# olasanni1/ETOL

Hardware: AMD Instinct MI355X
Metric: collocation-node constraint+Jacobian evals/sec, 6-state VGP N=1024 (higher is better)
Workload: dtype f64

## Files before the change

etol_amd/_lib.py:

```python
import ctypes as C
import os

import torch

_HERE = os.path.dirname(os.path.abspath(__file__))
LIB_PATH = os.path.join(_HERE, "lib", "libemi355x.so")

EMI_OK = 0
STATUS = {0: "EMI_OK", 1: "EMI_ERR_ARG", 2: "EMI_ERR_STATE", 3: "EMI_ERR_HIP",
          4: "EMI_ERR_NO_DEVICE", 5: "EMI_ERR_UNSUPPORTED", 6: "EMI_ERR_COMM"}

MODEL_POINTMASS2D, MODEL_QUADROTOR2D, MODEL_FIXEDWING12 = 0, 1, 2
MODEL_SOURCE = 100
PATH_ELLIPSE, PATH_DISC, PATH_TRACK = 0, 1, 2
PATH_REC = 8
EVAL_NODES, EVAL_DEFECT, EVAL_ALL, EVAL_NOJAC = 1, 2, 3, 4
EVAL_KEEP_INVARIANT = 8


class EmiError(RuntimeError):
    pass


class Layout(C.Structure):
    _fields_ = [("model", C.c_int), ("ns", C.c_int), ("nc", C.c_int), ("np", C.c_int),
                ("M", C.c_int), ("B", C.c_int), ("nres", C.c_int), ("nvals", C.c_int),
                ("nhess", C.c_int), ("real_bytes", C.c_int), ("px", C.c_int), ("py", C.c_int),
                ("t0", C.c_double), ("tf", C.c_double)]


class PassPlan(C.Structure):
    _fields_ = [(n, C.c_int) for n in ("one_launch", "sw", "ksplit", "ring_stages", "cpart", "cx", "mfma_workgroups", "store_mode",
                                       "block_order", "tiles16", "piece", "tail", "k_tile", "column_tiles", "k_halves")]


_P = C.c_void_p
_D = C.POINTER(C.c_double)
_I = C.POINTER(C.c_int)


def _ptr_struct(name, fields):
    return type(name, (C.Structure,), {"_fields_": [(f, _P) for f in fields], "FIELDS": tuple(fields)})


IpmPoint = _ptr_struct("IpmPoint", ("X", "U", "S", "E1", "E2"))
IpmDuals = _ptr_struct("IpmDuals", ("LamF", "Y", "ZL", "ZU", "VL", "VU", "W1", "W2"))
IpmStep = _ptr_struct("IpmStep", ("DZLam", "DS", "DY", "DE1", "DE2", "DZL", "DZU", "DVL", "DVU", "DW1", "DW2"))
IpmElim = _ptr_struct("IpmElim", ("Sigma", "SigT", "SigS", "RhatS", "Rt"))


class IpmBounds(C.Structure):
    _fields_ = [("zl", _P), ("zu", _P), ("nsets", C.c_int), ("cl", _D), ("cu", _D), ("cscale", _D)]


class IpmOptions(C.Structure):
    _fields_ = [(n, C.c_double) for n in ("tol", "mu_init", "bound_push", "bound_frac", "rho_init", "acceptable_factor")] + \
               [(n, C.c_int) for n in ("max_iter", "acceptable_iter", "max_futile_escalations", "rules", "crawl_limit")] + \
               [("crawl_frac", C.c_double)]


class IpmResult(C.Structure):
    _fields_ = [(n, C.c_int) for n in ("status", "iterations", "evaluations", "factorisations", "reflected_steps")] + \
               [(n, C.c_double) for n in ("cost", "kkt_error", "constr_viol", "emax", "mu", "rho")] + \
               [(n, C.c_int) for n in ("newton_steps", "restored_steps")]


class IpmRung(C.Structure):
    _fields_ = [("M", C.c_int), ("bd", IpmBounds), ("recs", _D), ("opt", IpmOptions), ("repair", C.c_int)]


class IpmRefine(C.Structure):
    _fields_ = [("ode_tol", C.c_double), ("first_check", C.c_int), ("ul", _D), ("uu", _D)]


class IpmRefineResult(C.Structure):
    _fields_ = [("rung", C.c_int), ("verdict", C.c_int), ("rungs_solved", C.c_int), ("err", C.c_double)]


class Start(C.Structure):
    _fields_ = [("kind", C.c_int), ("nsets", C.c_int), ("xa", _D), ("xb", _D), ("box", _D), ("bend", C.c_double), ("clearance", C.c_double),
                ("grid", C.c_int), ("repair", C.c_int)]


START_LINE, START_BEND, START_PLANNED = range(3)
REFINE_MET, REFINE_NOT_MET, REFINE_FELL_BACK, REFINE_FAILED = range(4)
IPM_RULE_RESIDUAL = 1
IPM_CONVERGED, IPM_ACCEPTABLE, IPM_MAX_ITER, IPM_LINE_SEARCH, IPM_INFEASIBLE, IPM_FACTOR, IPM_NOT_FINITE = range(7)

_PT, _DU, _ST, _EL, _BD = (C.POINTER(t) for t in (IpmPoint, IpmDuals, IpmStep, IpmElim, IpmBounds))

SYMBOLS = {
    "emi_abi_version": (C.c_int, []),
    "emi_status_string": (C.c_char_p, [C.c_int]),
    "emi_device_count": (C.c_int, [_I]),
    "emi_lgl": (C.c_int, [C.c_int, _D, _D, _D]),
    "emi_model_dims": (C.c_int, [C.c_int, _I, _I, _I]),
    "emi_edge_ellipse": (C.c_int, [C.c_double] * 4 + [_D]),
    "emi_track_centres": (C.c_int, [C.c_int, _D, _D, _D, C.c_int, _D, _D, _D]),
    "emi_create": (C.c_int, [C.c_int, C.POINTER(_P)]),
    "emi_create_f32": (C.c_int, [C.c_int, C.POINTER(_P)]),
    "emi_destroy": (C.c_int, [_P]),
    "emi_last_error": (C.c_char_p, [_P]),
    "emi_set_stream": (C.c_int, [_P, _P]),
    "emi_get_stream": (C.c_int, [_P, C.POINTER(_P)]),
    "emi_synchronize": (C.c_int, [_P]),
    "emi_set_mesh": (C.c_int, [_P, C.c_int, _D, _D, _D, C.c_double, C.c_double]),
    "emi_set_model": (C.c_int, [_P, C.c_int, _D, C.c_int, C.c_int]),
    "emi_set_model_source": (C.c_int, [_P, C.c_char_p, C.c_char_p, C.c_int, C.c_int, C.c_int, _I, C.c_int, _D, C.c_int, C.c_int]),
    "emi_check_model_source": (C.c_int, [C.c_char_p, C.c_char_p, C.c_int, C.c_int, C.c_int, C.c_int, C.c_int, C.c_char_p, C.c_size_t]),
    "emi_kkt_factor": (C.c_int, [_P, _D, _D, C.POINTER(C.c_ubyte), C.c_double, C.POINTER(C.c_int)]),
    "emi_kkt_factor_dev": (C.c_int, [_P, _P, _P, _P, C.c_double, C.POINTER(C.c_int)]),
    "emi_kkt_blocks_rows": (C.c_int, [_P, C.c_int, _I, _I, _I]),
    "emi_kkt_blocks_dev": (C.c_int, [_P, _P, _P, _P, _P, _P, C.c_double, _P, _P, C.c_int, _P, _P, _P, _P, _P]),
    "emi_kkt_blocks_host": (C.c_int, [_P, _D, _D, _D, _D, C.POINTER(C.c_ubyte), C.c_double, _D, _D, C.c_int, _I, _I, _D, _D, _D]),
    "emi_kkt_solve": (C.c_int, [_P, _D, C.c_int]),
    "emi_kkt_solve_dev": (C.c_int, [_P, _P, C.c_int]),
    "emi_ipm_reduce_dev": (C.c_int, [_P, _PT, _DU, _P, _P, _P, _BD, _P, _P, _P, _EL, _P]),
    "emi_ipm_expand_dev": (C.c_int, [_P, _PT, _DU, _P, _BD, _P, _EL, _P, _ST, _P]),
    "emi_ipm_trial_dev": (C.c_int, [_P, _PT, _ST, _P, _PT]),
    "emi_ipm_merit_dev": (C.c_int, [_P, _PT, _P, _P, _BD, _P, _P, C.c_int, _P]),
    "emi_ipm_accept_dev": (C.c_int, [_P, _PT, _PT, _DU, _ST, _BD, _P, _P, _P, _P]),
    "emi_ipm_error_dev": (C.c_int, [_P, _PT, _DU, _P, _P, _BD, _P, _P]),
    "emi_ipm_reduce_host": (C.c_int, [_P, _PT, _DU, _P, _P, _P, _BD, _P, _P, _P, _EL, _P]),
    "emi_ipm_expand_host": (C.c_int, [_P, _PT, _DU, _P, _BD, _P, _EL, _P, _ST, _P]),
    "emi_ipm_trial_host": (C.c_int, [_P, _PT, _ST, _P, _PT]),
    "emi_ipm_merit_host": (C.c_int, [_P, _PT, _P, _P, _BD, _P, _P, C.c_int, _P]),
    "emi_ipm_accept_host": (C.c_int, [_P, _PT, _PT, _DU, _ST, _BD, _P, _P, _P, _P]),
    "emi_ipm_error_host": (C.c_int, [_P, _PT, _DU, _P, _P, _BD, _P, _P]),
    "emi_ipm_start_dev": (C.c_int, [_P, C.c_int, _PT, _DU, _P, _BD, _P, C.c_double, C.c_double, _P, _P]),
    "emi_ipm_error_parts_dev": (C.c_int, [_P, _PT, _DU, _P, _P, _BD, _P, _P]),
    "emi_ipm_error_parts_host": (C.c_int, [_P, _PT, _DU, _P, _P, _BD, _P, _P]),
    "emi_ipm_keep_dev": (C.c_int, [_P, _PT, _DU, _PT, _DU, _P, C.c_int]),
    "emi_ipm_keep_host": (C.c_int, [_P, _PT, _DU, _PT, _DU, _P, C.c_int]),
    "emi_ipm_solve_shard_dev": (C.c_int, [_P, _P, _P, _BD, C.POINTER(IpmOptions), _P, _P, C.POINTER(IpmResult)]),
    "emi_ipm_solve_shard_host": (C.c_int, [_P, _P, _P, _BD, C.POINTER(IpmOptions), _P, _P, C.POINTER(IpmResult)]),
    "emi_prolong_matrix": (C.c_int, [C.c_int, _D, _D, C.c_int, _D, _D]),
    "emi_prolong_dev": (C.c_int, [_P, C.c_int, C.c_int, _P, _P, C.c_int, _P]),
    "emi_repair_guess_dev": (C.c_int, [_P, _P]),
    "emi_ipm_solve_ladder_dev": (C.c_int, [_P, C.c_int, C.POINTER(IpmRung), C.c_double, C.c_double, _P, _P, _P, _P, _P, _P, C.POINTER(IpmResult)]),
    "emi_ipm_solve_ladder_host": (C.c_int, [_P, C.c_int, C.POINTER(IpmRung), C.c_double, C.c_double, _P, _P, _P, _P, _P, _P, C.POINTER(IpmResult)]),
    "emi_ode_error_operator": (C.c_int, [C.c_int, _D, _D, _D, _D, _D]),
    "emi_interp_dev": (C.c_int, [_P, C.c_int, C.c_int, C.c_int, _P, _P, C.c_int, C.c_int, _P]),
    "emi_ode_error_dev": (C.c_int, [_P, _P, _P, _D, _D, _P, _P]),
    "emi_ode_error_host": (C.c_int, [_P, _P, _P, _D, _D, _P, _P]),
    "emi_ipm_refine_decide": (C.c_int, [C.c_int, C.c_double, C.c_double, C.c_int, C.c_int, _I]),
    "emi_prolong_rows_dev": (C.c_int, [_P, C.c_int, C.c_int, _P, _P, C.c_int, _P, _P]),
    "emi_shard_move_dev": (C.c_int, [_P, C.c_int, _P, _P, C.c_int, _I, C.POINTER(_P), _I, C.POINTER(_P), _I, C.c_int]),
    "emi_ipm_solve_refine_dev": (C.c_int, [_P, C.c_int, C.POINTER(IpmRung), C.c_double, C.c_double, C.POINTER(IpmRefine), _P, _P, C.c_int,
                                           _P, _P, _P, _P, C.POINTER(IpmResult), _D, C.POINTER(IpmRefineResult)]),
    "emi_ipm_solve_refine_host": (C.c_int, [_P, C.c_int, C.POINTER(IpmRung), C.c_double, C.c_double, C.POINTER(IpmRefine), _P, _P, C.c_int,
                                            _P, _P, _P, _P, C.POINTER(IpmResult), _D, C.POINTER(IpmRefineResult)]),
    "emi_plan_route": (C.c_int, [C.c_int, _D, _D, _D, C.c_double, C.c_int, C.c_int, _D, _D, _D, _I, _D, _I, _I]),
    "emi_start_guess_dev": (C.c_int, [_P, C.POINTER(Start), _P, _P]),
    "emi_start_guess_host": (C.c_int, [_P, C.POINTER(Start), _P, _P]),
    "emi_kkt_last_regularisation": (C.c_int, [_P, _D, _D]),
    "emi_kkt_factor_batch": (C.c_int, [C.c_int, C.POINTER(_P), C.POINTER(_D), C.POINTER(_D), C.POINTER(C.POINTER(C.c_ubyte)), _D, _I]),
    "emi_kkt_solve_batch": (C.c_int, [C.c_int, C.POINTER(_P), C.POINTER(_D)]),
    "emi_kkt_is_schur": (C.c_int, [_P]),
    "emi_kkt_solve_refined": (C.c_int, [_P, _D, C.c_double, C.c_int, _D, _I, _I, _I]),
    "emi_kkt_solve_refined_batch": (C.c_int, [C.c_int, C.POINTER(_P), C.POINTER(_D), _D, C.c_int, _D, _I, _I, _I]),
    "emi_kkt_lowrank": (C.c_int, [_P, C.c_int, C.POINTER(C.c_int), _D, _D, C.POINTER(C.c_int)]),
    "emi_kkt_factor_shard_dev": (C.c_int, [_P, _P, _P, _P, _D, C.POINTER(C.c_ubyte), _I]),
    "emi_kkt_lowrank_shard_dev": (C.c_int, [_P, C.c_int, _P, _P, _P, _P, C.POINTER(C.c_ubyte), _I]),
    "emi_kkt_solve_shard_dev": (C.c_int, [_P, _P, C.POINTER(C.c_ubyte)]),
    "emi_kkt_solve_refined_shard_dev": (C.c_int, [_P, _P, C.POINTER(C.c_ubyte), _D, C.c_int, _D, _I, _I, _I]),
    "emi_set_batch": (C.c_int, [_P, C.c_int]),
    "emi_set_path": (C.c_int, [_P, C.c_int, C.c_int, _D, C.c_int, C.c_int]),
    "emi_set_tracks": (C.c_int, [_P, C.c_int, C.c_int, _D, _D]),
    "emi_set_track_waypoints": (C.c_int, [_P, C.c_int, C.c_int, C.c_int, _I, _D, _D, _D]),
    "emi_tracks_from_waypoints_dev": (C.c_int, [_P, C.c_int, _P]),
    "emi_get_tracks": (C.c_int, [_P, _D, _D]),
    "emi_get_layout": (C.c_int, [_P, C.POINTER(Layout)]),
    "emi_jac_structure": (C.c_int, [_P, _I, _I]),
    "emi_invariant_rows": (C.c_int, [C.c_int, C.c_int, C.POINTER(C.c_ubyte), _I]),
    "emi_dev_alloc": (C.c_int, [_P, C.c_size_t, C.POINTER(_P)]),
    "emi_dev_free": (C.c_int, [_P, _P]),
    "emi_h2d": (C.c_int, [_P, _P, _P, C.c_size_t]),
    "emi_d2h": (C.c_int, [_P, _P, _P, C.c_size_t]),
    "emi_eval_dev": (C.c_int, [_P, _P, _P, _P, _P, _P, C.c_uint]),
    "emi_eval_host": (C.c_int, [_P, _D, _D, _D, _D, _D, C.c_uint]),
    "emi_hess_dev": (C.c_int, [_P, _P, _P, _P, _P, C.c_double, _P]),
    "emi_hess_host": (C.c_int, [_P, _D, _D, _D, _D, C.c_double, _D]),
    "emi_lagr_grad_dev": (C.c_int, [_P, _P, _P, _P, C.c_double, _P]),
    "emi_lagr_grad_host": (C.c_int, [_P, _D, _D, _D, C.c_double, _D]),
    "emi_kkt_certificate_dev": (C.c_int, [_P, _P, _P, _P, _P, _P, _P, C.c_double, _P, _P, C.c_int, _D, _D, _P, _P]),
    "emi_kkt_certificate_host": (C.c_int, [_P, _D, _D, _D, _D, C.c_double, _D, _D, C.c_int, _D, _D, _D, _D]),
    "emi_lagr_grad_total_dev": (C.c_int, [_P, _P, _P, _P, C.c_double, _P, _P]),
    "emi_lagr_grad_total_host": (C.c_int, [_P, _D, _D, _D, C.c_double, _D, _D]),
    "emi_kkt_certificate_total_dev": (C.c_int, [_P, _P, _P, _P, _P, _P, _P, C.c_double, _P, _P, C.c_int, _D, _D, _P, _P, _P]),
    "emi_kkt_certificate_total_host": (C.c_int, [_P, _D, _D, _D, _D, C.c_double, _D, _D, C.c_int, _D, _D, _D, _D, _D]),
    "emi_timer_start": (C.c_int, [_P]),
    "emi_timer_stop": (C.c_int, [_P, C.POINTER(C.c_float)]),
    "emi_profile_enable": (C.c_int, [_P, C.c_int]),
    "emi_profile_read": (C.c_int, [_P, C.POINTER(C.c_float), _I, C.POINTER(C.c_float), _I, C.POINTER(C.c_float), _I]),
    "emi_set_option": (C.c_int, [_P, C.c_char_p, C.c_int]),
    "emi_last_path": (C.c_int, [_P, _I]),
    "emi_plan_pass": (C.c_int, [_P, C.c_int, C.POINTER(PassPlan)]),
    "emi_last_defect_kernel": (C.c_char_p, [_P]),
    "emi_debug_pass_roles": (C.c_int, [C.c_int, C.c_int, C.c_int, C.POINTER(C.c_int), C.c_int]),
    "emi_debug_tile_order": (C.c_int, [C.c_int, C.c_int, C.c_int, C.c_int, C.c_int, C.POINTER(C.c_int), C.c_int, C.POINTER(C.c_int), C.POINTER(C.c_int), C.POINTER(C.c_int)]),
    "emi_set_delays": (C.c_int, [_P, C.c_int, C.c_int, C.c_double]),
    "emi_get_delays": (C.c_int, [_P, _I, _I, _I]),
    "emi_delay_matrix": (C.c_int, [C.c_int, C.POINTER(C.c_double), C.POINTER(C.c_double), C.c_double, C.c_double, C.c_double, C.POINTER(C.c_double)]),
    "emi_debug_tile_order2": (C.c_int, [C.c_int] * 7 + [C.POINTER(C.c_int), C.c_int, C.POINTER(C.c_int), C.POINTER(C.c_int), C.POINTER(C.c_int)]),
    "emi_comm_unique_id": (C.c_int, [_P]),
    "emi_comm_create": (C.c_int, [C.c_int, C.c_int, C.c_int, _P, C.POINTER(_P)]),
    "emi_comm_gather": (C.c_int, [_P, _P, _P, C.c_size_t, C.c_int, _P]),
    "emi_comm_destroy": (C.c_int, [_P]),
    "emi_comm_last_error": (C.c_char_p, [_P]),
}

_lib = None


def load():
    global _lib
    if _lib is not None:
        return _lib
    if not os.path.exists(LIB_PATH):
        raise EmiError(f"{LIB_PATH} is missing: run `python -c 'import __graft_entry__ as g; g.build()'` "
                       "(or `make lib`) first; there is no CPU fallback")
    lib = C.CDLL(LIB_PATH, mode=C.RTLD_GLOBAL)
    for name, (res, args) in SYMBOLS.items():
        fn = getattr(lib, name)
        fn.restype = res
        fn.argtypes = args
    _lib = lib
    return lib


def check(status, ctx=None, what=""):
    if status == EMI_OK:
        return
    lib = load()
    msg = lib.emi_status_string(status).decode()
    if ctx:
        detail = lib.emi_last_error(ctx).decode()
        if detail:
            msg += ": " + detail
    raise EmiError(f"{what or 'libemi355x'}: {STATUS.get(status, status)} ({msg})")
```

etol_amd/csrc/emi_api.hip:

```cpp
#include "emi_ctx.hpp"

using namespace emi_api;

int emi_api::fail(emi_ctx_t c, int code, const char* fmt, ...) {
    char buf[512];
    va_list ap;
    va_start(ap, fmt);
    vsnprintf(buf, sizeof buf, fmt, ap);
    va_end(ap);
    if (c) c->err = buf;
    return code;
}

int emi_api::upload_bytes(emi_ctx_t c, DevBuf& b, const void* src, size_t bytes) {
    EMI_TRY(ensure(c, b, bytes));
    if (bytes == 0) return EMI_OK;
    HIP_TRY(c, hipMemcpyAsync(b.p, src, bytes, hipMemcpyHostToDevice, c->stream));
    HIP_TRY(c, hipStreamSynchronize(c->stream));
    return EMI_OK;
}

int emi_api::upload_real(emi_ctx_t c, DevBuf& b, const double* src, size_t n) {
    if (!c->f32) return upload_bytes(c, b, src, n * 8);
    std::vector<float> tmp(n);
    for (size_t i = 0; i < n; ++i) tmp[i] = (float)src[i];
    return upload_bytes(c, b, tmp.data(), n * 4);
}

int emi_api::download_real(emi_ctx_t c, double* dst, const void* dsrc, size_t n) {
    if (!dst || n == 0) return EMI_OK;
    std::vector<float> tmp(c->f32 ? n : 0);
    HIP_TRY(c, hipMemcpyAsync(c->f32 ? (void*)tmp.data() : (void*)dst, dsrc, n * (c->f32 ? 4 : 8), hipMemcpyDeviceToHost, c->stream));
    HIP_TRY(c, hipStreamSynchronize(c->stream));
    for (size_t i = 0; i < tmp.size(); ++i) dst[i] = tmp[i];
    return EMI_OK;
}

int emi_api::ensure_vals_staging(emi_ctx_t c, size_t bytes) {
    if (c->s_VALS.bytes() < bytes) c->keep.written(c->s_VALS.p);
    return ensure(c, c->s_VALS, bytes);
}

void* emi_api::HostStager::place(const void* host, size_t bytes, bool in, bool out) {
    if (!host || status) return nullptr;
    if (slot == c->host_stage.size()) c->host_stage.emplace_back();
    DevBuf& b = c->host_stage[slot++];
    if (b.reserve(std::max<size_t>(bytes, 8)) != hipSuccess) { status = fail(c, EMI_ERR_HIP, "staging of a host-form call: out of device memory"); return nullptr; }
    if (in && bytes && hipMemcpyAsync(b.p, host, bytes, hipMemcpyHostToDevice, c->stream) != hipSuccess) {
        status = fail(c, EMI_ERR_HIP, "staging of a host-form call: copy failed");
        return nullptr;
    }
    if (out) outs.push_back({const_cast<void*>(host), b.p, bytes});
    return b.p;
}

int emi_api::HostStager::finish() {
    for (const Out& o : outs)
        if (o.bytes) HIP_TRY(c, hipMemcpyAsync(o.host, o.dev, o.bytes, hipMemcpyDeviceToHost, c->stream));
    HIP_TRY(c, hipStreamSynchronize(c->stream));
    return EMI_OK;
}

namespace {

struct OptionRow {
    const char* name;
    int emi_ctx_s::*member;
    bool (*accepts)(int);
    int (*stored)(int);
    const char* message;
};
template <int LO, int HI> bool within(int v) { return v >= LO && v <= HI; }
template <int... VS> bool one_of(int v) { return ((v == VS) || ...); }
bool any_value(int) { return true; }
bool at_least_0(int v) { return v >= 0; }
bool whole_tiles(int v) { return v >= 0 && v % 16 == 0; }
int as_given(int v) { return v; }
int as_flag(int v) { return v != 0; }
int ring_wgs(int v) { return v == 1 ? 1 : 2; }
int block_order(int v) { return v < 0 ? -1 : (v >= 100 ? v : (v != 0)); }

const OptionRow OPTIONS[] = {
    {"overlap", &emi_ctx_s::allow_fused, any_value, as_flag, nullptr},
    {"fused", &emi_ctx_s::allow_fused, any_value, as_flag, nullptr},
    {"sym_ct", &emi_ctx_s::sym_ct, within<0, 8>, as_given,
     "sym_ct must be 0..8 (0/4 = chosen from the batch, 3 = LDS-DMA ring, 5..8 = state-split ring with SW = NS/2/1/3)"},
    {"small_rows", &emi_ctx_s::small_rows, at_least_0, as_given, "small_rows must be >= 0 (0 disables the skinny defect kernel)"},
    {"sym_order", &emi_ctx_s::sym_order, any_value, as_flag, nullptr},
    {"f32_ring", &emi_ctx_s::f32_ring, any_value, as_flag, nullptr},
    {"f32_ring_wgs", &emi_ctx_s::f32_ring_wgs, any_value, ring_wgs, nullptr},
    {"f32_one_launch", &emi_ctx_s::f32_one_launch, any_value, as_flag, nullptr},
    {"slice", &emi_ctx_s::slice, whole_tiles, as_given, "slice must be 0 (never) or a multiple of 16 instances"},
    {"pass_order", &emi_ctx_s::pass_order, any_value, block_order, nullptr},
    {"sym_ablate", &emi_ctx_s::sym_ablate, any_value, as_given, nullptr},
    {"adj_fold_tile", &emi_ctx_s::adj_fold_tile, within<0, 2>, as_given, "adj_fold_tile must be 0 (by size), 1 (48 x 64) or 2 (96 x 128)"},
    {"cost_in_kernel", &emi_ctx_s::cost_in_kernel, any_value, as_flag, nullptr},
    {"sym_nst", &emi_ctx_s::sym_nst, one_of<3, 4>, as_given, "sym_nst must be 3 or 4"},
    {"sym_hs", &emi_ctx_s::sym_hs, within<0, 2>, as_given, "sym_hs must be 0 (by batch size), 1 or 2"},
    {"sym_ctc", &emi_ctx_s::sym_ctc, within<0, 2>, as_given, "sym_ctc must be 0 (by batch size), 1 or 2"},
    {"sym_bk", &emi_ctx_s::sym_bk, one_of<0, 8, 16>, as_given, "sym_bk must be 0 (by batch size), 8 or 16"},
    {"sym_cpart", &emi_ctx_s::sym_cpart, one_of<-1, 0, 1, 2, 4, 8>, as_given, "sym_cpart must be -1 (plain order), 0 (by mesh size), 1, 2, 4 or 8"},
    {"sym_gblk", &emi_ctx_s::sym_gblk, within<0, 64>, as_given, "sym_gblk must be 0 (off) .. 64 instance groups per super-block"},
    {"sym_cx", &emi_ctx_s::sym_cx, within<0, 64>, as_given, "sym_cx must be 0 (default) .. 64 column tiles per block"},
    {"sym_combine", &emi_ctx_s::sym_combine, any_value, as_flag, nullptr},
    {"sym_ksplit", &emi_ctx_s::sym_ksplit, one_of<0, 1, 2, 4, 8>, as_given, "sym_ksplit must be 0 (by batch size), 1, 2, 4 or 8"},
    {"node_store", &emi_ctx_s::node_store, within<-1, 3>, as_given,
     "node_store must be -1 (by size), 0 (plain), 1 (write-through sc1), 2 (non-temporal) or 3 (nt sc1; the one-launch pass only)"},
    {"overlap_mode", &emi_ctx_s::overlap_mode, within<0, 3>, as_given,
     "overlap_mode must be 0 (by batch size), 1 (one stream), 2 (two streams) or 3 (one launch)"},
};

}

extern "C" {

int emi_device_count(int* count) {
    if (!count) return EMI_ERR_ARG;
    int n = 0;
    if (hipGetDeviceCount(&n) != hipSuccess) n = 0;
    *count = n;
    return EMI_OK;
}

static int create_impl(int device_id, bool f32, emi_ctx_t* out) {
    if (!out) return EMI_ERR_ARG;
    *out = nullptr;
    int n = 0;
    if (hipGetDeviceCount(&n) != hipSuccess || n <= 0) return EMI_ERR_NO_DEVICE;
    if (device_id < 0 || device_id >= n) return EMI_ERR_ARG;
    hipDeviceProp_t prop;
    if (hipGetDeviceProperties(&prop, device_id) != hipSuccess) return EMI_ERR_HIP;
    if (strncmp(prop.gcnArchName, "gfx950", 6) != 0) return EMI_ERR_NO_DEVICE;
    if (hipSetDevice(device_id) != hipSuccess) return EMI_ERR_HIP;
    emi_ctx_t c = new emi_ctx_s();
    c->device = device_id;
    c->f32 = f32;
    c->own_stream = true;
    if (hipStreamCreateWithFlags(&c->stream, hipStreamNonBlocking) != hipSuccess ||
        hipEventCreateWithFlags(&c->ev_fork, hipEventDisableTiming) != hipSuccess ||
        hipEventCreateWithFlags(&c->ev_join, hipEventDisableTiming) != hipSuccess ||
        hipEventCreate(&c->t_start) != hipSuccess || hipEventCreate(&c->t_stop) != hipSuccess) {
        delete c;
        return EMI_ERR_HIP;
    }
    *out = c;
    return EMI_OK;
}

int emi_create(int device_id, emi_ctx_t* out) { return create_impl(device_id, false, out); }
int emi_create_f32(int device_id, emi_ctx_t* out) { return create_impl(device_id, true, out); }

int emi_destroy(emi_ctx_t c) {
    if (!c) return EMI_ERR_ARG;
    delete c;
    return EMI_OK;
}

const char* emi_last_error(emi_ctx_t c) { return c ? c->err.c_str() : "null context"; }

int emi_set_stream(emi_ctx_t c, void* s) {
    if (!c) return EMI_ERR_ARG;
    HIP_TRY(c, hipSetDevice(c->device));
    HIP_TRY(c, hipStreamSynchronize(c->stream));
    if (s == nullptr) {
        if (!c->own_stream) {
            HIP_TRY(c, hipStreamCreateWithFlags(&c->stream, hipStreamNonBlocking));
            c->own_stream = true;
        }
        return EMI_OK;
    }
    if (c->own_stream) { HIP_TRY(c, hipStreamDestroy(c->stream)); c->own_stream = false; }
    c->stream = (hipStream_t)s;
    return EMI_OK;
}

int emi_get_stream(emi_ctx_t c, void** s) {
    if (!c || !s) return EMI_ERR_ARG;
    *s = (void*)c->stream;
    return EMI_OK;
}

int emi_synchronize(emi_ctx_t c) {
    if (!c) return EMI_ERR_ARG;
    HIP_TRY(c, hipStreamSynchronize(c->stream));
    return EMI_OK;
}

static int upload_operator(emi_ctx_t c, int M, const double* D) {
    if (c->f32) {
        std::vector<float> Df((size_t)M * M);
        for (int i = 0; i < M; ++i) {
            double rs = 0.0;
            for (int j = 0; j < M; ++j) {
                if (j == i) continue;
                Df[(size_t)i * M + j] = (float)D[(size_t)i * M + j];
                rs += (double)Df[(size_t)i * M + j];
            }
            Df[(size_t)i * M + i] = (float)(-rs);
        }
        return upload_bytes(c, c->d_D, Df.data(), Df.size() * 4);
    }
    EMI_TRY(upload_real(c, c->d_D, D, (size_t)M * M));
    if (M % 2 != 0) return EMI_OK;
    const int N = M - 1, Hh = M / 2;
    for (int i = 0; i < M; ++i)
        for (int j = 0; j < M; ++j)
            if (D[(size_t)i * M + j] != -D[(size_t)(N - i) * M + (N - j)]) return EMI_OK;
    std::vector<double> De((size_t)Hh * Hh), Do((size_t)Hh * Hh);
    for (int i = 0; i < Hh; ++i)
        for (int j = 0; j < Hh; ++j) {
            const double p = D[(size_t)i * M + j], q = D[(size_t)i * M + (N - j)];
            De[(size_t)i * Hh + j] = 0.5 * (p + q);
            Do[(size_t)i * Hh + j] = 0.5 * (p - q);
        }
    EMI_TRY(upload_real(c, c->d_De, De.data(), De.size()));
    EMI_TRY(upload_real(c, c->d_Do, Do.data(), Do.size()));
    c->symmetric = true;
    return EMI_OK;
}

int emi_set_mesh(emi_ctx_t c, int M, const double* tau, const double* w, const double* D, double t0,
                 double tf) {
    if (!c || M < 2 || !tau || !w) return fail(c, EMI_ERR_ARG, "emi_set_mesh: bad argument");
    if (!(tf > t0)) return fail(c, EMI_ERR_ARG, "emi_set_mesh: tf must exceed t0");
    c->keep.bump();
    HIP_TRY(c, hipSetDevice(c->device));
    const double h = (tf - t0) / 2.0;
    std::vector<double> nt(M), dd(M, 0.0);
    for (int k = 0; k < M; ++k) {
        nt[k] = t0 + h * (tau[k] + 1.0);
        if (D) dd[k] = D[(size_t)k * M + k];
    }
    EMI_TRY(upload_real(c, c->d_w, w, M));
    EMI_TRY(upload_real(c, c->d_t, nt.data(), M));
    EMI_TRY(upload_real(c, c->d_Ddiag, dd.data(), M));
    c->symmetric = false;
    if (D) EMI_TRY(upload_operator(c, M, D));
    c->points_only = !D;
    c->h_tau.assign(tau, tau + M);
    c->h_w.assign(w, w + M);
    c->M = M;
    c->t0 = t0;
    c->tf = tf;
    c->adj_dirty = true;
    c->ode_dirty = true;
    c->delay_dirty = true;
    c->adjw_dirty = true;
    emi::kkt_mesh_changed(c->kkt);
    for (emi::KktWorkspace* w : c->kkt_shard) emi::kkt_mesh_changed(w);
    c->ntracks = 0;
    c->track_sets = 0;
    c->wp_nt_dirty = true;
    if (c->B > 0) EMI_TRY(ensure(c, c->d_cost_part, (size_t)c->B * emi::node_chunks(M) * (c->f32 ? 4 : 8)));
    return EMI_OK;
}

static void model_in_force(emi_ctx_t c, int model, int ns, int nc, int npath, const int* path_vars, int n_path_vars,
                           const double* params, int nparams, int maximize) {
    c->keep.bump();
    c->model = model;
    c->ns = ns;
    c->nc = nc;
    c->xh = c->uh = c->nch = 0;
    c->np_model = npath;
    c->pvars.assign(path_vars, path_vars + n_path_vars);
    c->maximize = maximize ? 1 : 0;
    memset(c->params, 0, sizeof c->params);
    for (int i = 0; i < nparams; ++i) c->params[i] = params[i];
    c->np = 0;
    c->path_sets = 0;
    c->path_has_track = false;
}

int emi_set_model(emi_ctx_t c, int model, const double* params, int nparams, int maximize) {
    if (!c) return EMI_ERR_ARG;
    int ns, nc, np_expected;
    if (emi_model_dims(model, &ns, &nc, &np_expected)) return fail(c, EMI_ERR_ARG, "unknown model %d", model);
    if (nparams != np_expected || (nparams > 0 && !params))
        return fail(c, EMI_ERR_ARG, "model %d takes %d parameters, got %d", model, np_expected, nparams);
    if (c->rtc) {
        HIP_TRY(c, hipStreamSynchronize(c->stream));
        emi::rtc_destroy(c->rtc);
        c->rtc = nullptr;
    }
    model_in_force(c, model, ns, nc, 0, nullptr, 0, params, nparams, maximize);
    return EMI_OK;
}

int emi_set_model_source(emi_ctx_t c, const char* struct_name, const char* source, int ns, int nc, int npath,
                         const int* path_vars, int n_path_vars, const double* params, int nparams, int maximize) {
    if (!c) return EMI_ERR_ARG;
    if (npath < 0 || npath > 64) return fail(c, EMI_ERR_ARG, "emi_set_model_source: npath must be in [0, 64]");
    if (npath > 0 && (!path_vars || n_path_vars < 1 || n_path_vars > ns + nc))
        return fail(c, EMI_ERR_ARG, "emi_set_model_source: %d traced rows need the list of variables they depend on", npath);
    for (int q = 0; q < (npath > 0 ? n_path_vars : 0); ++q)
        if (path_vars[q] < 0 || path_vars[q] >= ns + nc || (q > 0 && path_vars[q] <= path_vars[q - 1]))
            return fail(c, EMI_ERR_ARG, "emi_set_model_source: path_vars must be ascending node-variable indices below %d", ns + nc);
    if (nparams < 0 || nparams > EMI_MAX_PARAMS || (nparams > 0 && !params))
        return fail(c, EMI_ERR_ARG, "emi_set_model_source: at most %d parameters", EMI_MAX_PARAMS);
    HIP_TRY(c, hipSetDevice(c->device));
    HIP_TRY(c, hipStreamSynchronize(c->stream));
    emi::RtcModel* m = nullptr;
    std::string log;
    const int st = emi::rtc_build(c->f32, struct_name, source, ns, nc, npath, npath > 0 ? n_path_vars : 0, &m, &log);
    if (st) {
        c->err = log;
        return st;
    }
    emi::rtc_destroy(c->rtc);
    c->rtc = m;
    model_in_force(c, EMI_MODEL_SOURCE, ns, nc, npath, path_vars, npath > 0 ? n_path_vars : 0, params, nparams, maximize);
    return EMI_OK;
}

int emi_check_model_source(const char* struct_name, const char* source, int ns, int nc, int npath, int n_path_vars, int f32,
                           char* log, size_t log_len) {
    std::string l;
    const int st = emi::rtc_check(f32 != 0, struct_name, source, ns, nc, npath, npath > 0 ? n_path_vars : 0, &l);
    if (log && log_len) {
        strncpy(log, l.c_str(), log_len - 1);
        log[log_len - 1] = '\0';
    }
    return st;
}

int emi_set_batch(emi_ctx_t c, int B) {
    if (!c || B < 1) return fail(c, EMI_ERR_ARG, "emi_set_batch: B must be >= 1");
    if (c->M <= 0) return fail(c, EMI_ERR_STATE, "emi_set_mesh must precede emi_set_batch");
    c->keep.bump();
    HIP_TRY(c, hipSetDevice(c->device));
    const size_t rb = c->f32 ? 4 : 8;
    int st = ensure(c, c->d_cost_part, (size_t)B * emi::node_chunks(c->M) * rb);
    if (st) return st;
    c->B = B;
    return EMI_OK;
}

int emi_set_delays(emi_ctx_t c, int x_horizon, int u_horizon, double dt) {
    if (!c || x_horizon < 0 || u_horizon < 0) return fail(c, EMI_ERR_ARG, "emi_set_delays: horizons must be >= 0");
    if (c->model < 0) return fail(c, EMI_ERR_STATE, "emi_set_model / emi_set_model_source must precede emi_set_delays");
    c->keep.bump();
    const int nxd = std::max(x_horizon - 1, 0) * c->ns;
    const int rest = c->nc - nxd;
    if (nxd + u_horizon == 0) { c->xh = x_horizon; c->uh = 0; c->nch = 0; return EMI_OK; }
    if (!(dt > 0)) return fail(c, EMI_ERR_ARG, "emi_set_delays: dt must be positive");
    if (rest < 1 || rest % (1 + u_horizon) != 0)
        return fail(c, EMI_ERR_ARG, "emi_set_delays: the model has %d controls, which is not nc + %d delayed states + %d x nc delayed controls for any nc >= 1",
                    c->nc, nxd, u_horizon);
    if (c->f32) return fail(c, EMI_ERR_UNSUPPORTED, "emi_set_delays: f64 contexts only");
    c->xh = x_horizon;
    c->uh = u_horizon;
    c->nch = c->nc - rest / (1 + u_horizon);
    c->delay_dt = dt;
    c->delay_dirty = true;
    c->adjw_dirty = true;
    return EMI_OK;
}

int emi_get_delays(emi_ctx_t c, int* x_horizon, int* u_horizon, int* n_delayed) {
    if (!c) return EMI_ERR_ARG;
    if (x_horizon) *x_horizon = c->xh;
    if (u_horizon) *u_horizon = c->uh;
    if (n_delayed) *n_delayed = c->nch;
    return EMI_OK;
}

int emi_set_path(emi_ctx_t c, int np, int nsets, const double* recs, int px_state, int py_state) {
    if (!c || np < 0) return fail(c, EMI_ERR_ARG, "emi_set_path: bad argument");
    if (c->model < 0) return fail(c, EMI_ERR_STATE, "emi_set_model must precede emi_set_path");
    c->keep.bump();
    if (np > 0 && (!recs || nsets < 1)) return fail(c, EMI_ERR_ARG, "emi_set_path: null table");
    if (px_state < 0 || px_state >= c->ns || py_state < 0 || py_state >= c->ns || px_state == py_state)
        return fail(c, EMI_ERR_ARG, "emi_set_path: state indices (%d,%d) out of range", px_state, py_state);
    HIP_TRY(c, hipSetDevice(c->device));
    bool has_track = false;
    for (size_t i = 0; i < (size_t)np * nsets; ++i) {
        const int kind = (int)recs[i * EMI_PATH_REC];
        if (kind != EMI_PATH_ELLIPSE && kind != EMI_PATH_DISC && kind != EMI_PATH_TRACK)
            return fail(c, EMI_ERR_ARG, "emi_set_path: record %zu has unknown kind %d", i, kind);
        has_track = has_track || kind == EMI_PATH_TRACK;
    }
    int st = upload_real(c, c->d_path, recs, (size_t)np * nsets * EMI_PATH_REC);
    if (st) return st;
    c->path_has_track = has_track;
    c->np = np;
    c->path_sets = np > 0 ? nsets : 0;
    c->px = px_state;
    c->py = py_state;
    return EMI_OK;
}

int emi_set_tracks(emi_ctx_t c, int ntracks, int nsets, const double* xc, const double* yc) {
    if (!c || ntracks < 0) return fail(c, EMI_ERR_ARG, "emi_set_tracks: bad argument");
    if (c->M <= 0) return fail(c, EMI_ERR_STATE, "emi_set_mesh must precede emi_set_tracks");
    c->keep.bump();
    if (ntracks > 0 && (!xc || !yc || nsets < 1)) return fail(c, EMI_ERR_ARG, "emi_set_tracks: null table");
    HIP_TRY(c, hipSetDevice(c->device));
    const size_t n = (size_t)ntracks * nsets * c->M;
    int st;
    if ((st = upload_real(c, c->d_trkx, xc, n))) return st;
    if ((st = upload_real(c, c->d_trky, yc, n))) return st;
    c->ntracks = ntracks;
    c->track_sets = ntracks > 0 ? nsets : 0;
    return EMI_OK;
}

int emi_set_track_waypoints(emi_ctx_t c, int ntracks, int nsets, int ld, const int* counts, const double* t, const double* x,
                            const double* y) {
    if (!c || ntracks < 0) return fail(c, EMI_ERR_ARG, "emi_set_track_waypoints: bad argument");
    if (ntracks == 0) {
        c->wp_ntracks = c->wp_sets = c->wp_ld = 0;
        return EMI_OK;
    }
    if (!t || !x || !y || nsets < 1) return fail(c, EMI_ERR_ARG, "emi_set_track_waypoints: null table");
    if (ld < 2) return fail(c, EMI_ERR_ARG, "emi_set_track_waypoints: ld %d is below the 2 waypoints a track needs", ld);
    const size_t rows = (size_t)nsets * ntracks, n = rows * ld;
    std::vector<int> cnt(rows, ld);
    for (size_t r = 0; r < rows; ++r) {
        const int set = (int)(r / ntracks), trk = (int)(r % ntracks);
        if (counts) cnt[r] = counts[r];
        if (cnt[r] < 2 || cnt[r] > ld)
            return fail(c, EMI_ERR_ARG, "emi_set_track_waypoints: set %d, track %d has %d waypoints (2 .. ld = %d)", set, trk, cnt[r], ld);
        for (int s = 0; s + 1 < cnt[r]; ++s)
            if (!(t[r * ld + s + 1] > t[r * ld + s]))
                return fail(c, EMI_ERR_ARG, "emi_set_track_waypoints: set %d, track %d: the times of waypoints %d and %d are not ascending", set,
                            trk, s, s + 1);
    }
    HIP_TRY(c, hipSetDevice(c->device));
    HIP_TRY(c, hipStreamSynchronize(c->stream));
    HIP_TRY(c, c->d_wp.reserve(3 * n));
    HIP_TRY(c, c->d_wp_cnt.reserve(rows));
    const double* src[3] = {t, x, y};
    for (int q = 0; q < 3; ++q) HIP_TRY(c, hipMemcpyAsync(c->d_wp.p + q * n, src[q], n * sizeof(double), hipMemcpyHostToDevice, c->stream));
    HIP_TRY(c, hipMemcpyAsync(c->d_wp_cnt.p, cnt.data(), rows * sizeof(int), hipMemcpyHostToDevice, c->stream));
    HIP_TRY(c, hipStreamSynchronize(c->stream));
    c->wp_ntracks = ntracks;
    c->wp_sets = nsets;
    c->wp_ld = ld;
    return EMI_OK;
}

int emi_tracks_from_waypoints_dev(emi_ctx_t c, int n, const void* dSetMap) {
    if (!c) return EMI_ERR_ARG;
    if (c->M <= 0) return fail(c, EMI_ERR_STATE, "emi_set_mesh must precede emi_tracks_from_waypoints_dev");
    if (c->wp_ntracks <= 0) return fail(c, EMI_ERR_STATE, "emi_tracks_from_waypoints_dev: emi_set_track_waypoints has not been called");
    if (n < 0 || (!dSetMap && n != 0 && n != c->wp_sets) || (dSetMap && n == 0))
        return fail(c, EMI_ERR_ARG, "emi_tracks_from_waypoints_dev: n = %d (without a map 0 or the table's %d sets, with one >= 1)", n, c->wp_sets);
    const int sets = dSetMap ? n : c->wp_sets;
    if ((long long)sets * c->wp_ntracks > 0x7fffffffLL) return fail(c, EMI_ERR_ARG, "emi_tracks_from_waypoints_dev: %d sets of %d tracks", sets, c->wp_ntracks);
    c->keep.bump();
    HIP_TRY(c, hipSetDevice(c->device));
    const size_t total = (size_t)sets * c->wp_ntracks * c->M, rb = c->f32 ? 4 : 8, wn = (size_t)c->wp_sets * c->wp_ntracks * c->wp_ld;
    EMI_TRY(ensure(c, c->d_trkx, total * rb));
    EMI_TRY(ensure(c, c->d_trky, total * rb));
    const double* node_t = (const double*)c->d_t.p;
    if (c->f32) {
        if (c->wp_nt_dirty || c->d_wp_nt.cap < (size_t)c->M) {
            const double h = (c->tf - c->t0) / 2.0;
            std::vector<double> nt(c->M);
            for (int k = 0; k < c->M; ++k) nt[k] = c->t0 + h * (c->h_tau[k] + 1.0);
            HIP_TRY(c, hipStreamSynchronize(c->stream));
            HIP_TRY(c, c->d_wp_nt.reserve(nt.size()));
            HIP_TRY(c, hipMemcpyAsync(c->d_wp_nt.p, nt.data(), nt.size() * sizeof(double), hipMemcpyHostToDevice, c->stream));
            HIP_TRY(c, hipStreamSynchronize(c->stream));
            c->wp_nt_dirty = false;
        }
        node_t = c->d_wp_nt.p;
    }
    const emi::TrackWaypointArgs a{c->d_wp.p, c->d_wp.p + wn, c->d_wp.p + 2 * wn, node_t, c->d_wp_cnt.p, (const int*)dSetMap,
                                   c->d_trkx.p, c->d_trky.p, sets, c->wp_ntracks, c->wp_ld, c->M, 0};
    HIP_TRY(c, c->f32 ? emi::launch_track_waypoints<float>(a, c->stream) : emi::launch_track_waypoints<double>(a, c->stream));
    c->ntracks = c->wp_ntracks;
    c->track_sets = sets;
    return EMI_OK;
}

int emi_get_tracks(emi_ctx_t c, double* xc, double* yc) {
    if (!c || !xc || !yc) return fail(c, EMI_ERR_ARG, "emi_get_tracks: null argument");
    if (c->M <= 0 || c->ntracks <= 0 || c->track_sets <= 0)
        return fail(c, EMI_ERR_STATE, "emi_get_tracks: the context holds no centres (emi_set_tracks or emi_tracks_from_waypoints_dev on this mesh)");
    HIP_TRY(c, hipSetDevice(c->device));
    const size_t n = (size_t)c->track_sets * c->ntracks * c->M;
    EMI_TRY(download_real(c, xc, c->d_trkx.p, n));
    return download_real(c, yc, c->d_trky.p, n);
}

int emi_get_layout(emi_ctx_t c, emi_layout_t* o) {
    if (!c || !o) return EMI_ERR_ARG;
    o->model = c->model;
    o->ns = c->ns;
    o->nc = c->nc;
    o->np = np_total(c);
    o->M = c->M;
    o->B = c->B;
    o->nres = nres_of(c);
    o->nvals = nvals_of(c);
    o->nhess = nhess_of(c);
    o->real_bytes = c->f32 ? 4 : 8;
    o->px = c->px;
    o->py = c->py;
    o->t0 = c->t0;
    o->tf = c->tf;
    return EMI_OK;
}

int emi_jac_structure(emi_ctx_t c, int* rows, int* cols) {
    if (!c || !rows || !cols) return EMI_ERR_ARG;
    if (c->M <= 0 || c->model < 0) return fail(c, EMI_ERR_STATE, "mesh and model must be set");
    const int M = c->M, ns = c->ns, nv = c->ns + c->nc;
    size_t e = 0;
    for (int i = 0; i < ns; ++i)
        for (int v = 0; v < nv; ++v)
            for (int k = 0; k < M; ++k, ++e) { rows[e] = i * M + k; cols[e] = v * M + k; }
    for (int j = 0; j < c->np; ++j)
        for (int s = 0; s < 2; ++s)
            for (int k = 0; k < M; ++k, ++e) {
                rows[e] = ns * M + 2 * ns + j * M + k;
                cols[e] = (s == 0 ? c->px : c->py) * M + k;
            }
    for (int j = 0; j < c->np_model; ++j)
        for (size_t q = 0; q < c->pvars.size(); ++q)
            for (int k = 0; k < M; ++k, ++e) {
                rows[e] = ns * M + 2 * ns + (c->np + j) * M + k;
                cols[e] = c->pvars[q] * M + k;
            }
    for (int v = 0; v < nv; ++v)
        for (int k = 0; k < M; ++k, ++e) { rows[e] = -1; cols[e] = v * M + k; }
    return EMI_OK;
}

int emi_invariant_rows(int model, int np, unsigned char* mask, int* nvals) {
    int ns, nc;
    if (np < 0 || emi_model_dims(model, &ns, &nc, nullptr)) return EMI_ERR_ARG;
    if (nvals) *nvals = ns * (ns + nc) + 2 * np + (ns + nc);
    if (mask && !emi::invariant_rows(model, np, mask)) return EMI_ERR_ARG;
    return EMI_OK;
}

int emi_dev_alloc(emi_ctx_t c, size_t bytes, void** dptr) {
// ... 147 lines not shown
```

etol_amd/csrc/emi_api_pass.hip:

```cpp
#include "emi_ctx.hpp"

using namespace emi_api;

namespace {

bool overlapped_path(emi_ctx_t c) {
    if (c->f32 || !c->allow_fused || !c->symmetric || c->M <= 0 || c->model < 0) return false;
    if (c->model == EMI_MODEL_SOURCE) return emi::rtc_has_symdefect(c->rtc) && c->M % 128 == 0;
    return emi::fused_supported(c->model, c->M, c->sym_ct);
}

bool pass_takes_small_batches(emi_ctx_t c, int B) {
    if (!overlapped_path(c) || (c->overlap_mode != 0 && c->overlap_mode != 3) || c->M % 128 != 0) return false;
    if (c->rtc) return emi::rtc_pass_supported(c->rtc, B, c->M, 1, 1, 0);
    const emi::SymPlan p = emi::plan_symdefect(c->ns, B, c->M, 7, 1, c->sym_cpart, c->sym_gblk, c->sym_cx);
    return emi::pass_supported(c->model, c->ns, B, c->M, p);
}

int store_mode_for(emi_ctx_t c, int B) {
    if (c->node_store >= 0) return c->node_store;
    if ((size_t)B * (nvals_of(c) + nres_of(c)) * c->M * (c->f32 ? 4 : 8) > ((size_t)230 << 20)) return 2;
    const int tiles16 = ((B + 15) / 16) * (c->M / 128);
    if (tiles16 > 16 && tiles16 <= 32) return 0;
    return (!c->rtc && !c->f32) ? 1 : 0;
}

struct PassPlan {
    bool one_launch = false;
    emi::SymPlan sym;
    int tiles16 = 0;
    int store_mode = 0;
    int mfma_first = 0;
};

PassPlan plan_pass(emi_ctx_t c, int B, bool jac) {
    PassPlan p;
    p.tiles16 = ((B + 15) / 16) * (c->M / 128);
    p.store_mode = store_mode_for(c, B);
    const bool auto_mode = c->overlap_mode == 0;
    if (!((c->overlap_mode == 3 || auto_mode) && jac) || c->M % 128 != 0) return p;
    const bool auto_ct = auto_mode && (c->sym_ct == 0 || c->sym_ct == 4);
    const int gblk = (c->sym_gblk == 0 && c->sym_cpart == 0 && B > 2048 && B % 256 == 0) ? 2 : c->sym_gblk;
    const int gblk_first = (auto_ct || c->rtc) ? gblk : c->sym_gblk;
    int ct = c->sym_ct;
    const bool deep_base = auto_ct && !c->rtc && c->sym_bk == 0 && c->sym_ksplit == 0 && c->sym_nst == 3;
    const bool deep_mid = deep_base && c->ns % 2 == 0 && c->ns > 2 && p.tiles16 >= 49 && p.tiles16 < 128;
    const bool deep_small = deep_base && c->ns % 2 == 0 && c->ns > 2 && p.tiles16 >= 33 && p.tiles16 < 49;
    if (c->rtc) ct = (p.store_mode == 2 && emi::rtc_pass_sw_large(c->rtc) == 2) ? 6 : 7;
    else if (auto_ct) ct = (p.tiles16 < 128 && !deep_mid) ? 7 : 6;
    emi::SymPlan plan = emi::plan_symdefect(c->ns, B, c->M, ct, 1, c->sym_cpart, gblk_first, c->sym_cx);
    if (plan.ring1) plan = emi::plan_symdefect(c->ns, B, c->M, 5, 1, c->sym_cpart, c->sym_gblk, c->sym_cx);
    int ks_want = c->sym_ksplit;
    if (ks_want == 0 && auto_ct && !deep_mid && !deep_small) ks_want = plan.tiles * 4 <= 256 ? 4 : (plan.tiles * 2 <= 512 ? 2 : 1);
    if (ks_want > 1) {
        const int ct_now = plan.sw == c->ns ? 5 : (plan.sw == 2 ? 6 : (plan.sw == 3 ? 8 : 7));
        plan = emi::plan_symdefect(c->ns, B, c->M, ct_now, ks_want, c->sym_cpart, c->rtc ? gblk : c->sym_gblk, c->sym_cx);
    } else {
        plan.ks = 1;
    }
    plan.nst = c->rtc ? 3 : c->sym_nst;
    const bool deep_large = auto_ct && !c->rtc && c->sym_bk == 0 && c->sym_nst == 3 && c->pass_order < 0 && p.tiles16 >= 208 && p.tiles16 <= 1024;
    const bool deep_band = auto_ct && !c->rtc && c->sym_bk == 0 && c->sym_nst == 3 && c->pass_order < 0 && c->ns % 2 == 0 && c->ns > 2 &&
                           p.tiles16 >= 144 && p.tiles16 < 208;
    const int bk_want = c->sym_bk ? c->sym_bk : ((deep_mid || deep_small || deep_large || deep_band) ? 16 : 8);
    if (bk_want == 16 && !c->rtc && plan.ks == 1 && (plan.sw == 1 || plan.sw == 2) && plan.nst == 3) plan.bk = 16;
    const bool wide_large = auto_ct && c->sym_ctc == 0 && B > 2048 && B % 256 == 0 && c->sym_cpart == 0;
    const int ctc_want = c->sym_ctc ? c->sym_ctc : (wide_large ? 2 : 1);
    if (ctc_want == 2 && !c->rtc && plan.ks == 1 && plan.sw == 2 && plan.nst == 3 && c->M % 256 == 0) {
        const int bk_keep = plan.bk;
        plan = emi::plan_symdefect(c->ns, B, c->M, 6, 1, c->sym_cpart, gblk_first, (wide_large && c->sym_cx == 0) ? 1 : c->sym_cx, bk_keep, 2);
        plan.ks = 1;
        plan.nst = 3;
        plan.bk = bk_keep;
    }
    const int hs_want = c->sym_hs ? c->sym_hs : 1;
    if (hs_want == 2 && !c->rtc && plan.ks == 1 && plan.ct == 1 && (plan.sw == 1 || plan.sw == 2) && plan.nst == 3 &&
        ((c->M / 2) / plan.bk) % 4 == 0)
        plan.hs = 2;
    p.sym = plan;
    p.mfma_first = c->pass_order >= 0 ? c->pass_order
                                      : (deep_band ? 150 : (p.tiles16 < 208 ? 1 : (p.tiles16 < 384 ? 125 : (p.tiles16 < 768 ? 110 : 0))));
    p.one_launch = c->rtc ? emi::rtc_pass_supported(c->rtc, B, c->M, plan.sw, plan.ks, p.store_mode)
                          : emi::pass_supported(c->model, c->ns, B, c->M, plan);
    return p;
}

int plan_piece(emi_ctx_t c, int B) {
    const long long cap = ((0xFFFFFFFFLL / ((long long)c->ns * c->M * 8)) / 256) * 256;
    int piece = 0;
    if (c->slice > 0) { if (B > 2 * c->slice) piece = c->slice; }
    else if (B > 2048) piece = (int)std::min<long long>(cap > 0 ? cap : 256, B - B % 256);
    return piece >= B ? 0 : piece;
}

struct Launch { int first, B; bool keep = false; };
struct PassIO { const void *X, *U; void *RES, *VALS, *COST; };

PassIO io_at(emi_ctx_t c, const PassIO& io, int first) {
    const size_t row = (size_t)first * c->M * (c->f32 ? 4 : 8);
    return PassIO{(const char*)io.X + row * c->ns, (const char*)io.U + row * c->nc, (char*)io.RES + row * nres_of(c),
                  io.VALS ? (char*)io.VALS + row * nvals_of(c) : nullptr, (char*)io.COST + (size_t)first * (c->f32 ? 4 : 8)};
}

template <typename T>
void fill_node_args(emi_ctx_t c, Launch L, emi::NodeArgs<T>& a, const PassIO& io) {
    a.X = (const T*)io.X;
    a.U = (const T*)io.U;
    a.RES = (T*)io.RES;
    a.VALS = (T*)io.VALS;
    a.cost_part = (T*)c->d_cost_part.p + (size_t)L.first * emi::node_chunks(c->M);
    a.cost = (T*)io.COST;
    a.cost_ticket = nullptr;
    a.w = (const T*)c->d_w.p;
    a.node_t = (const T*)c->d_t.p;
    a.Ddiag = (const T*)c->d_Ddiag.p;
    a.path = (const T*)c->d_path.p + (c->path_sets > 1 ? (size_t)L.first * c->np * EMI_PATH_REC : 0);
    a.track_x = (const T*)c->d_trkx.p + (c->track_sets > 1 ? (size_t)L.first * c->ntracks * c->M : 0);
    a.track_y = (const T*)c->d_trky.p + (c->track_sets > 1 ? (size_t)L.first * c->ntracks * c->M : 0);
    a.M = c->M;
    a.B = L.B;
    a.np = np_total(c);
    a.nres = nres_of(c);
    a.nvals = nvals_of(c);
    a.path_sets = c->path_sets;
    a.track_sets = c->track_sets;
    a.ntracks = c->ntracks;
    a.px = c->px;
    a.py = c->py;
    a.store_mode = store_mode_for(c, L.B);
    a.keep = L.keep ? 1 : 0;
    a.h = (T)((c->tf - c->t0) / 2.0);
    a.sgn = c->maximize ? T(-1) : T(1);
    for (int i = 0; i < EMI_MAX_PARAMS; ++i) a.P.p[i] = (T)c->params[i];
}

void delay_matrix(const std::vector<double>& tau, const std::vector<double>& w, double t0, double tf, double delay, double* W) {
    const int M = (int)tau.size();
    std::vector<double> lam(M);
    for (int j = 0; j < M; ++j) lam[j] = ((j & 1) ? -1.0 : 1.0) * std::sqrt(w[j]);
    const double hh = (tf - t0) / 2.0;
    for (int k = 0; k < M; ++k) {
        double ts = t0 + hh * (tau[k] + 1.0) - delay;
        if (ts < t0) ts = t0;
        const double x = (ts - t0) / hh - 1.0;
        double* row = W + (size_t)k * M;
        int hit = -1;
        for (int j = 0; j < M; ++j)
            if (x == tau[j]) hit = j;
        if (ts <= t0) hit = 0;
        if (hit >= 0) {
            for (int j = 0; j < M; ++j) row[j] = j == hit ? 1.0 : 0.0;
            continue;
        }
        double den = 0.0;
        for (int j = 0; j < M; ++j) {
            row[j] = lam[j] / (x - tau[j]);
            den += row[j];
        }
        for (int j = 0; j < M; ++j) row[j] /= den;
    }
}

int extend_controls(emi_ctx_t c, const void* dX, const void* dU_free, const void** dU_ext) {
    if (c->f32) return fail(c, EMI_ERR_UNSUPPORTED, "delayed values: f64 contexts only");
    if (c->points_only) return fail(c, EMI_ERR_STATE, "delayed values need a collocation mesh (this context holds a points-only mesh)");
    const int M = c->M, ncf = c->nc - c->nch;
    HIP_TRY(c, hipSetDevice(c->device));
    if (!c->attr_set) {
        HIP_TRY(c, emi::defect_f64_set_attr());
        c->attr_set = true;
    }
    int st;
    if ((st = ensure_delay_matrices(c))) return st;
    const size_t row = (size_t)M * 8;
    if ((st = ensure(c, c->d_uext, (size_t)c->B * c->nc * row))) return st;
    HIP_TRY(c, hipMemsetAsync(c->d_uext.p, 0, (size_t)c->B * c->nc * row, c->stream));
    HIP_TRY(c, hipMemcpy2DAsync(c->d_uext.p, (size_t)c->nc * row, dU_free, (size_t)ncf * row, (size_t)ncf * row, c->B, hipMemcpyDeviceToDevice, c->stream));
    double* base = (double*)c->d_uext.p + (size_t)ncf * M;
    for (int i = 1; i < c->xh; ++i) {
        emi::DefectArgs a{(const double*)dX, (const double*)c->d_W.p + (size_t)(i - 1) * M * M, base + (size_t)(i - 1) * c->ns * M,
                          c->B * c->ns, M, c->ns, c->nc};
        HIP_TRY(c, emi::launch_defect_f64(a, c->stream));
    }
    base += (size_t)std::max(c->xh - 1, 0) * c->ns * M;
    for (int i = 1; i <= c->uh; ++i) {
        emi::DefectArgs a{(const double*)dU_free, (const double*)c->d_W.p + (size_t)(i - 1) * M * M, base + (size_t)(i - 1) * ncf * M,
                          c->B * ncf, M, ncf, c->nc};
        HIP_TRY(c, emi::launch_defect_f64(a, c->stream));
    }
    *dU_ext = c->d_uext.p;
    return EMI_OK;
}

enum class Form {
    PassF64,
    TwoKernelF64,
    PassF32,
    TwoStreamF32,
    Sequential,
};
struct FormChoice {
    Form form = Form::Sequential;
    bool small = false;
    PassPlan plan;
    bool overlapped() const { return form == Form::PassF64 || form == Form::TwoKernelF64; }
};

FormChoice choose_form(emi_ctx_t c, Launch L, unsigned flags) {
    const bool nodes = flags & EMI_EVAL_NODES, defect = flags & EMI_EVAL_DEFECT, jac = !(flags & EMI_EVAL_NOJAC);
    FormChoice ch;
    ch.small = defect && !c->f32 && L.B > 0 && L.B * c->ns <= c->small_rows && emi::defect_small_supported(L.B * c->ns) &&
               !(nodes && jac && pass_takes_small_batches(c, L.B));
    if (nodes && defect && !ch.small && overlapped_path(c)) {
        ch.plan = plan_pass(c, L.B, jac);
        ch.form = ch.plan.one_launch ? Form::PassF64 : Form::TwoKernelF64;
    } else if (c->f32 && nodes && defect && jac && !c->rtc && c->allow_fused) {
        if ((c->overlap_mode == 3 || (c->overlap_mode == 0 && c->f32_one_launch)) && emi::pass_f32_supported(c->model, L.B * c->ns, c->M, L.B))
            ch.form = Form::PassF32;
        else if (c->overlap_mode == 2 && emi::defect_f32_mfma_supported(c->M))
            ch.form = Form::TwoStreamF32;
    }
    return ch;
}

int next_prof_record(emi_ctx_t c, ProfEvents** out) {
    if (c->prof_used == c->prof.size()) c->prof.emplace_back();
    ProfEvents& pe = c->prof[c->prof_used];
    for (hipEvent_t& e : pe.ev)
        if (!e) HIP_TRY(c, hipEventCreate(&e));
    ++c->prof_used;
    *out = &pe;
    return EMI_OK;
}

constexpr unsigned AT1 = 1u << 1, AT2 = 1u << 2, AT3 = 1u << 3, AT_ANY = AT1 | AT2 | AT3;
int prof_mark(emi_ctx_t c, ProfEvents* pe, ProfMark which, unsigned levels, hipStream_t s) {
    if (pe && pe->level > 0 && ((levels >> pe->level) & 1u)) HIP_TRY(c, hipEventRecord(pe->ev[which], s));
    return EMI_OK;
}

const char* const NAME_PASS_F32 = "emi_pass_f32_kernel (MFMA + node roles, one launch)";
const char* const NAME_RING1_F64 = "emi_symdefect_ring_f64_kernel";
const char* name_defect_f32(emi_ctx_t c, bool mfma) {
    return !mfma ? "emi_defect_f32_kernel" : (c->f32_ring ? "emi_defect_f32_ring_kernel" : "emi_defect_f32_mfma_kernel");
}
const char* name_defect_f64(bool small) { return small ? "emi_defect_small_f64_kernel" : "emi_defect_f64_kernel"; }
std::string name_pass_f64(const emi::SymPlan& plan) {
    return "emi_pass_f64_kernel<SW=" + std::to_string(plan.sw) + "> (MFMA + node roles, one launch" +
           (plan.ks > 1 ? ", " + std::to_string(plan.ks) + " K slices per tile" : "") + ")" +
           (plan.bk == 16 ? " [K tiles of 16]" : "") + (plan.ct == 2 ? " [128-column tiles]" : "") + (plan.hs == 2 ? " [K range in two halves per workgroup]" : "");
}
std::string name_symdefect(emi_ctx_t c, const emi::SymPlan& plan, bool in_kernel_combine) {
    if (plan.ring1) return c->sym_ct == 1 || c->sym_ct == 2 ? "emi_symdefect_f64_kernel" : NAME_RING1_F64;
    return "emi_symdefect_ring2_f64_kernel<SW=" + std::to_string(plan.sw) + ">" +
           (plan.ks > 1 ? " x" + std::to_string(plan.ks) + (in_kernel_combine ? " K slices (in-kernel combine)" : " K slices + emi_symdefect_combine_kernel") : "");
}

emi::SymDefectArgs sym_defect_args(emi_ctx_t c, Launch L, const PassIO& io) {
    emi::SymDefectArgs sa;
    sa.X = (const double*)io.X;
    sa.U = (const double*)io.U;
    sa.RES = (double*)io.RES;
    sa.node_t = (const double*)c->d_t.p;
    sa.De = (const double*)c->d_De.p;
    sa.Do = (const double*)c->d_Do.p;
    sa.M = c->M;
    sa.B = L.B;
    sa.nres = nres_of(c);
    sa.h = (c->tf - c->t0) / 2.0;
    sa.order = c->sym_order;
    sa.ablate = c->sym_ablate;
    sa.ksplit = 1;
    sa.slab = nullptr;
    sa.tile_ticket = nullptr;
    sa.cpart = sa.cx = 0;
    sa.mfma_first = 0;
    for (int i = 0; i < EMI_MAX_PARAMS; ++i) sa.P.p[i] = c->params[i];
    return sa;
}

emi::DefectArgsF32 defect_args_f32(emi_ctx_t c, Launch L, const PassIO& io) {
    return emi::DefectArgsF32{(const float*)io.X, (const float*)c->d_D.p, (float*)io.RES, L.B * c->ns, c->M, c->ns, nres_of(c)};
}

int form_pass_f64(emi_ctx_t c, Launch L, const PassIO& io, const PassPlan& pp, ProfEvents* pe) {
    const emi::SymPlan& plan = pp.sym;
    emi::SymDefectArgs sa = sym_defect_args(c, L, io);
    emi::NodeArgs<double> na;
    fill_node_args(c, L, na, io);
    sa.mfma_first = pp.mfma_first;
    sa.cpart = plan.cpart;
    sa.cx = plan.cx;
    if (plan.ks > 1) {
        EMI_TRY(ensure(c, c->d_slab, plan.slab_bytes));
        EMI_TRY(ensure_zeroed(c, c->d_tile_ticket, (size_t)plan.tiles * 4, c->stream));
        sa.ksplit = plan.ks;
        sa.slab = (double*)c->d_slab.p;
        sa.tile_ticket = (unsigned*)c->d_tile_ticket.p;
    }
    EMI_TRY(ensure_zeroed(c, c->d_ticket, (size_t)L.B * 4, c->stream));
    na.cost_ticket = (unsigned*)c->d_ticket.p;
    EMI_TRY(prof_mark(c, pe, K0, AT_ANY, c->stream));
    if (c->rtc) HIP_TRY(c, emi::rtc_launch_pass(c->rtc, sa, na, plan.sw, c->stream));
    else HIP_TRY(c, emi::launch_pass(c->model, sa, na, c->stream, plan));
    EMI_TRY(prof_mark(c, pe, K1, AT_ANY, c->stream));
    if (pe) pe->level = -1;
    c->last_defect_kernel = name_pass_f64(plan);
    return EMI_OK;
}

int launch_symdefect_f64(emi_ctx_t c, Launch L, emi::SymDefectArgs& sa, hipStream_t s) {
    if (c->rtc) {
        HIP_TRY(c, emi::rtc_launch_symdefect(c->rtc, sa, s));
        c->last_defect_kernel = NAME_RING1_F64;
        return EMI_OK;
    }
    const emi::SymPlan plan = emi::plan_symdefect(c->ns, L.B, c->M, c->sym_ct, c->sym_ksplit, c->sym_cpart, c->sym_gblk, c->sym_cx);
    if (plan.slab_bytes) EMI_TRY(ensure(c, c->d_slab, plan.slab_bytes));
    sa.ksplit = plan.ring1 ? 1 : plan.ks;
    sa.slab = (double*)c->d_slab.p;
    sa.cpart = plan.cpart;
    sa.cx = plan.cx;
    if (sa.ksplit > 1 && c->sym_combine) {
        EMI_TRY(ensure_zeroed(c, c->d_tile_ticket, (size_t)plan.tiles * 4, s));
        sa.tile_ticket = (unsigned*)c->d_tile_ticket.p;
    }
    const unsigned bit = 1u << c->sym_ct;
    HIP_TRY(c, emi::launch_symdefect(c->model, sa, s, !(c->fused_attr_mask & bit), c->sym_ct, plan));
    c->fused_attr_mask |= bit;
    c->last_defect_kernel = name_symdefect(c, plan, sa.tile_ticket != nullptr);
    return EMI_OK;
}

int form_two_kernel_f64(emi_ctx_t c, Launch L, const PassIO& io, bool jac, ProfEvents* pe) {
    emi::SymDefectArgs sa = sym_defect_args(c, L, io);
    emi::NodeArgs<double> na;
    fill_node_args(c, L, na, io);
    const bool two = c->overlap_mode != 1;
    const bool split = two && c->cu_split > 0;
    if (two && !split) EMI_TRY(need_stream2(c));
    hipStream_t s1 = split ? c->s_mfma : c->stream;
    hipStream_t s2 = split ? c->s_node : (two ? c->stream2 : c->stream);
    if (two) {
        HIP_TRY(c, hipEventRecord(c->ev_fork, c->stream));
        HIP_TRY(c, hipStreamWaitEvent(s2, c->ev_fork, 0));
        if (split) HIP_TRY(c, hipStreamWaitEvent(s1, c->ev_fork, 0));
    }
    EMI_TRY(prof_mark(c, pe, K0, AT1 | AT2, s1));
    EMI_TRY(launch_symdefect_f64(c, L, sa, s1));
    EMI_TRY(prof_mark(c, pe, K1, AT1 | AT2, s1));
    if (c->cost_in_kernel) {
        EMI_TRY(ensure_zeroed(c, c->d_ticket, (size_t)L.B * 4, s2));
        na.cost_ticket = (unsigned*)c->d_ticket.p;
    }
    EMI_TRY(prof_mark(c, pe, K2, AT1 | AT3, s2));
    if (c->rtc && jac && na.store_mode == 2 && c->M % 2 == 0) HIP_TRY(c, emi::rtc_launch_nodes_nt(c->rtc, na, s2));
    else if (c->rtc) HIP_TRY(c, emi::rtc_launch_nodes<double>(c->rtc, na, jac, false, s2));
    else HIP_TRY(c, emi::launch_nodes<double>(c->model, na, jac, false, s2));
    EMI_TRY(prof_mark(c, pe, K3, AT1 | AT3, s2));
    if (!c->cost_in_kernel) HIP_TRY(c, emi::launch_cost_finish<double>(na.cost_part, na.cost, L.B, emi::node_chunks(c->M), na.sgn * na.h, s2));
    if (two) {
        HIP_TRY(c, hipEventRecord(c->ev_join, s2));
        HIP_TRY(c, hipStreamWaitEvent(c->stream, c->ev_join, 0));
        if (split) {
            HIP_TRY(c, hipEventRecord(c->ev_join2, s1));
            HIP_TRY(c, hipStreamWaitEvent(c->stream, c->ev_join2, 0));
        }
    }
    EMI_TRY(prof_mark(c, pe, E1, AT1, c->stream));
    EMI_TRY(prof_mark(c, pe, E2, AT1, c->stream));
    return EMI_OK;
}

int form_pass_f32(emi_ctx_t c, Launch L, const PassIO& io, ProfEvents* pe) {
    emi::NodeArgs<float> na;
    fill_node_args(c, L, na, io);
    const size_t rowb = (size_t)c->M * 4;
    HIP_TRY(c, hipMemset2DAsync(io.RES, (size_t)nres_of(c) * rowb, 0, (size_t)c->ns * rowb, L.B, c->stream));
    EMI_TRY(ensure_zeroed(c, c->d_ticket, (size_t)L.B * 4, c->stream));
    na.cost_ticket = (unsigned*)c->d_ticket.p;
    EMI_TRY(prof_mark(c, pe, K0, AT_ANY, c->stream));
    HIP_TRY(c, emi::launch_pass_f32(c->model, defect_args_f32(c, L, io), na, c->pass_order >= 0 ? c->pass_order : 0, c->stream));
    EMI_TRY(prof_mark(c, pe, K1, AT_ANY, c->stream));
    if (pe) { pe->level = -1; pe->fused = true; }
    c->last_defect_kernel = NAME_PASS_F32;
    return EMI_OK;
}

int form_two_stream_f32(emi_ctx_t c, Launch L, const PassIO& io, ProfEvents* pe) {
    emi::NodeArgs<float> pre, full;
    PassIO values_only = io;
    values_only.VALS = nullptr;
    fill_node_args(c, L, pre, values_only);
    fill_node_args(c, L, full, io);
    EMI_TRY(ensure(c, c->d_cost_part2, (size_t)L.B * emi::node_chunks(c->M) * 4));
    EMI_TRY(need_stream2(c));
    pre.cost_part = (float*)c->d_cost_part2.p;
    pre.np = 0;
    const bool fork_late = c->f32_ring_wgs == 1;
    if (!fork_late) {
        HIP_TRY(c, hipEventRecord(c->ev_fork, c->stream));
        HIP_TRY(c, hipStreamWaitEvent(c->stream2, c->ev_fork, 0));
    }
    HIP_TRY(c, emi::launch_nodes<float>(c->model, pre, false, true, c->stream));
    if (fork_late) {
        HIP_TRY(c, hipEventRecord(c->ev_fork, c->stream));
        HIP_TRY(c, hipStreamWaitEvent(c->stream2, c->ev_fork, 0));
    }
    EMI_TRY(prof_mark(c, pe, K0, AT1 | AT2, c->stream));
    HIP_TRY(c, emi::launch_defect_f32_mfma(defect_args_f32(c, L, io), c->stream, c->f32_ring, c->f32_ring_wgs));
    EMI_TRY(prof_mark(c, pe, K1, AT1 | AT2, c->stream));
    c->last_defect_kernel = name_defect_f32(c, true);
    EMI_TRY(prof_mark(c, pe, K2, AT1 | AT3, c->stream2));
    HIP_TRY(c, emi::launch_nodes<float>(c->model, full, true, false, c->stream2));
    EMI_TRY(prof_mark(c, pe, K3, AT1 | AT3, c->stream2));
    HIP_TRY(c, emi::launch_cost_finish<float>(full.cost_part, full.cost, L.B, emi::node_chunks(c->M), full.sgn * full.h, c->stream2));
    HIP_TRY(c, hipEventRecord(c->ev_join, c->stream2));
    HIP_TRY(c, hipStreamWaitEvent(c->stream, c->ev_join, 0));
    if (pe) pe->fused = true;
    EMI_TRY(prof_mark(c, pe, E1, AT1, c->stream));
    EMI_TRY(prof_mark(c, pe, E2, AT1, c->stream));
    return EMI_OK;
}

template <typename T>
int launch_nodes_alone(emi_ctx_t c, Launch L, const PassIO& io, bool jac) {
    emi::NodeArgs<T> a;
    fill_node_args(c, L, a, io);
    if (c->rtc) HIP_TRY(c, emi::rtc_launch_nodes<T>(c->rtc, a, jac, true, c->stream));
    else HIP_TRY(c, emi::launch_nodes<T>(c->model, a, jac, true, c->stream));
    HIP_TRY(c, emi::launch_cost_finish<T>(a.cost_part, a.cost, L.B, emi::node_chunks(c->M), a.sgn * a.h, c->stream));
    return EMI_OK;
}

int form_sequential(emi_ctx_t c, Launch L, const PassIO& io, unsigned flags, bool small, ProfEvents* pe) {
    const bool jac = !(flags & EMI_EVAL_NOJAC);
    if (flags & EMI_EVAL_NODES) EMI_TRY(c->f32 ? launch_nodes_alone<float>(c, L, io, jac) : launch_nodes_alone<double>(c, L, io, jac));
    EMI_TRY(prof_mark(c, pe, E1, AT_ANY, c->stream));
    if ((flags & EMI_EVAL_DEFECT) && c->f32) {
        const bool mfma = emi::defect_f32_mfma_supported(c->M) && c->allow_fused;
        if (mfma) HIP_TRY(c, emi::launch_defect_f32_mfma(defect_args_f32(c, L, io), c->stream, c->f32_ring, c->f32_ring_wgs));
        else HIP_TRY(c, emi::launch_defect_f32(defect_args_f32(c, L, io), c->stream));
        c->last_defect_kernel = name_defect_f32(c, mfma);
    } else if (flags & EMI_EVAL_DEFECT) {
        emi::DefectArgs a{(const double*)io.X, (const double*)c->d_D.p, (double*)io.RES, L.B * c->ns, c->M, c->ns, nres_of(c)};
        if (small) HIP_TRY(c, emi::launch_defect_small_f64(a, c->stream));
        else HIP_TRY(c, emi::launch_defect_f64(a, c->stream));
        c->last_defect_kernel = name_defect_f64(small);
    }
    EMI_TRY(prof_mark(c, pe, E2, AT1 | AT2, c->stream));
    return EMI_OK;
}

int eval_launch(emi_ctx_t c, Launch L, const PassIO& io, unsigned flags) {
    const bool nodes = flags & EMI_EVAL_NODES, defect = flags & EMI_EVAL_DEFECT;
    const bool jac = !(flags & EMI_EVAL_NOJAC);
    if (!nodes && !defect) return fail(c, EMI_ERR_ARG, "emi_eval: empty flags");
    if (defect && c->points_only) return fail(c, EMI_ERR_STATE, "emi_eval: the mesh has no differentiation matrix (points-only mesh): EMI_EVAL_NODES only");
    if (!io.X || !io.RES || (nodes && (!io.U || !io.COST || (jac && !io.VALS))))
        return fail(c, EMI_ERR_ARG, "emi_eval: null device pointer");
    HIP_TRY(c, hipSetDevice(c->device));
    if (!c->attr_set) {
        HIP_TRY(c, emi::defect_f64_set_attr());
        c->attr_set = true;
    }
    const FormChoice ch = choose_form(c, L, flags);
    ProfEvents* pe = nullptr;
    if (c->profile) {
        EMI_TRY(next_prof_record(c, &pe));
        pe->has_node = nodes;
        pe->has_defect = defect;
        pe->fused = ch.overlapped();
        pe->level = c->profile;
        EMI_TRY(prof_mark(c, pe, E0, pe->fused ? AT1 : AT1 | AT3, c->stream));
    }
    switch (ch.form) {
        case Form::PassF64: return form_pass_f64(c, L, io, ch.plan, pe);
        case Form::TwoKernelF64: return form_two_kernel_f64(c, L, io, jac, pe);
        case Form::PassF32: return form_pass_f32(c, L, io, pe);
        case Form::TwoStreamF32: return form_two_stream_f32(c, L, io, pe);
        case Form::Sequential: break;
    }
    return form_sequential(c, L, io, flags, ch.small, pe);
}

}

int emi_api::ensure_delay_matrices(emi_ctx_t c) {
    if (!c->delay_dirty) return EMI_OK;
    const int M = c->M, nd = std::max(c->xh - 1, c->uh);
    std::vector<double> W((size_t)nd * M * M);
    for (int d = 0; d < nd; ++d) delay_matrix(c->h_tau, c->h_w, c->t0, c->tf, (d + 1) * c->delay_dt, W.data() + (size_t)d * M * M);
    EMI_TRY(upload_real(c, c->d_W, W.data(), W.size()));
    c->delay_dirty = false;
    return EMI_OK;
}

int emi_api::need_stream2(emi_ctx_t c) {
    if (c->stream2) return EMI_OK;
    if (hipStreamCreateWithFlags(&c->stream2, hipStreamNonBlocking) != hipSuccess) {
        c->stream2 = nullptr;
        return fail(c, EMI_ERR_HIP, "cannot create the second stream of the two-stream pass");
    }
    return EMI_OK;
}

extern "C" {

int emi_delay_matrix(int M, const double* tau, const double* w, double t0, double tf, double delay, double* W) {
    if (M < 2 || !tau || !w || !W || !(tf > t0) || delay < 0) return EMI_ERR_ARG;
    delay_matrix(std::vector<double>(tau, tau + M), std::vector<double>(w, w + M), t0, tf, delay, W);
    return EMI_OK;
}

int emi_eval_dev(emi_ctx_t c, const void* dX, const void* dU, void* dRES, void* dVALS, void* dCOST,
                 unsigned flags) {
    int st = ready(c);
    if (st) return st;
    if (c->nch > 0 && dX && dU && (st = extend_controls(c, dX, dU, &dU))) return st;
    int piece = 0;
    if (!c->profile && !c->f32 && (flags & EMI_EVAL_ALL) == EMI_EVAL_ALL && overlapped_path(c) && dX && dU && dRES && dCOST &&
        (dVALS || (flags & EMI_EVAL_NOJAC)))
        piece = plan_piece(c, c->B);
    const PassIO io{dX, dU, dRES, dVALS, dCOST};
    const emi::KeepRecord::Pass kp = c->keep.begin_pass((flags & EMI_EVAL_NODES) && !(flags & EMI_EVAL_NOJAC),
                                                        flags & EMI_EVAL_KEEP_INVARIANT, dVALS);
    flags &= ~(unsigned)EMI_EVAL_KEEP_INVARIANT;
    if (piece <= 0) st = eval_launch(c, Launch{0, c->B, kp.keep}, io, flags);
    for (int first = 0; piece > 0 && first < c->B && st == EMI_OK; first += piece)
        st = eval_launch(c, Launch{first, std::min(piece, c->B - first), kp.keep}, io_at(c, io, first), flags);
    c->keep.end_pass(kp, dVALS, st == EMI_OK);
    return st;
}

int emi_eval_host(emi_ctx_t c, const double* X, const double* U, double* RES, double* VALS,
                  double* COST, unsigned flags) {
    int st = ready(c);
    if (st) return st;
    if (!X || !U) return fail(c, EMI_ERR_ARG, "emi_eval_host: null input");
    const size_t rb = c->f32 ? 4 : 8;
    const size_t nX = (size_t)c->B * c->ns * c->M, nU = (size_t)c->B * (c->nc - c->nch) * c->M;
    const size_t nR = (size_t)c->B * nres_of(c) * c->M, nV = (size_t)c->B * nvals_of(c) * c->M;
    if ((st = upload_real(c, c->s_X, X, nX))) return st;
    if ((st = upload_real(c, c->s_U, U, nU))) return st;
    if ((st = ensure(c, c->s_RES, nR * rb))) return st;
    if ((st = ensure_vals_staging(c, nV * rb))) return st;
    if ((st = ensure(c, c->s_COST, (size_t)c->B * rb))) return st;
    if (!(flags & EMI_EVAL_NODES)) {
        if (!RES) return fail(c, EMI_ERR_ARG, "emi_eval_host: defect-only needs RES in/out");
        if ((st = upload_real(c, c->s_RES, RES, nR))) return st;
    }
    if ((st = emi_eval_dev(c, c->s_X.p, c->s_U.p, c->s_RES.p, c->s_VALS.p, c->s_COST.p, flags | EMI_EVAL_KEEP_INVARIANT))) return st;
    if ((st = download_real(c, RES, c->s_RES.p, nR))) return st;
    if (!(flags & EMI_EVAL_NOJAC) && (flags & EMI_EVAL_NODES))
        if ((st = download_real(c, VALS, c->s_VALS.p, nV))) return st;
    if (flags & EMI_EVAL_NODES)
        if ((st = download_real(c, COST, c->s_COST.p, c->B))) return st;
    HIP_TRY(c, hipStreamSynchronize(c->stream));
    return EMI_OK;
}

int emi_hess_dev(emi_ctx_t c, const void* dX, const void* dU, const void* dLamF, const void* dLamC,
                 double sigma, void* dH) {
    int st = ready(c);
    if (st) return st;
    if (!dX || !dU || !dLamF || !dH || (np_total(c) > 0 && !dLamC))
        return fail(c, EMI_ERR_ARG, "emi_hess: null device pointer");
    HIP_TRY(c, hipSetDevice(c->device));
    if (c->nch > 0 && (st = extend_controls(c, dX, dU, &dU))) return st;
    auto fill = [&](auto& a) {
        using T = typename std::remove_reference<decltype(a.h)>::type;
        a.X = (const T*)dX; a.U = (const T*)dU; a.lamF = (const T*)dLamF; a.lamC = (const T*)dLamC;
        a.H = (T*)dH; a.w = (const T*)c->d_w.p; a.node_t = (const T*)c->d_t.p;
        a.path = (const T*)c->d_path.p;
        a.M = c->M; a.B = c->B; a.np = np_total(c); a.path_sets = c->path_sets; a.px = c->px; a.py = c->py;
        a.h = (T)((c->tf - c->t0) / 2.0); a.sgn = c->maximize ? T(-1) : T(1); a.sigma = (T)sigma;
        for (int i = 0; i < EMI_MAX_PARAMS; ++i) a.P.p[i] = (T)c->params[i];
    };
    if (c->f32) {
        emi::HessArgs<float> a;
        fill(a);
        if (c->rtc) HIP_TRY(c, emi::rtc_launch_hess<float>(c->rtc, a, c->stream));
        else HIP_TRY(c, emi::launch_hess<float>(c->model, a, c->stream));
    } else {
        emi::HessArgs<double> a;
        fill(a);
        if (c->rtc) HIP_TRY(c, emi::rtc_launch_hess<double>(c->rtc, a, c->stream));
        else HIP_TRY(c, emi::launch_hess<double>(c->model, a, c->stream));
    }
    return EMI_OK;
}

int emi_hess_host(emi_ctx_t c, const double* X, const double* U, const double* LamF,
                  const double* LamC, double sigma, double* H) {
    int st = ready(c);
    if (st) return st;
    if (!X || !U || !LamF || !H || (np_total(c) > 0 && !LamC)) return fail(c, EMI_ERR_ARG, "emi_hess_host: null pointer");
    const size_t rb = c->f32 ? 4 : 8;
    const size_t nX = (size_t)c->B * c->ns * c->M, nU = (size_t)c->B * (c->nc - c->nch) * c->M;
    const size_t nC = (size_t)c->B * np_total(c) * c->M, nH = (size_t)c->B * nhess_of(c) * c->M;
    if ((st = upload_real(c, c->s_X, X, nX))) return st;
    if ((st = upload_real(c, c->s_U, U, nU))) return st;
    if ((st = upload_real(c, c->s_LF, LamF, nX))) return st;
    if (nC && (st = upload_real(c, c->s_LC, LamC, nC))) return st;
    if ((st = ensure(c, c->s_H, nH * rb))) return st;
    if ((st = emi_hess_dev(c, c->s_X.p, c->s_U.p, c->s_LF.p, c->s_LC.p, sigma, c->s_H.p))) return st;
    return download_real(c, H, c->s_H.p, nH);
}

int emi_plan_pass(emi_ctx_t c, int B, emi_pass_plan_t* out) {
    if (!c || !out || B < 1) return EMI_ERR_ARG;
    if (c->M <= 0 || c->model < 0) return fail(c, EMI_ERR_STATE, "emi_plan_pass: mesh and model must be set");
    memset(out, 0, sizeof *out);
    const int piece = (!c->f32 && overlapped_path(c)) ? plan_piece(c, B) : 0;
    const int first = piece > 0 ? piece : B;
    out->piece = piece;
    out->tail = piece > 0 ? B % piece : 0;
    if (!c->f32 && overlapped_path(c)) {
        const PassPlan p = plan_pass(c, first, true);
        out->one_launch = p.one_launch ? 1 : 0;
        out->sw = p.sym.sw;
        out->ksplit = p.sym.ks;
        out->ring_stages = p.sym.nst;
        out->k_tile = p.sym.bk;
        out->column_tiles = p.sym.ct;
        out->k_halves = p.sym.hs;
        out->cpart = p.sym.cpart;
        out->cx = p.sym.cx;
        out->mfma_workgroups = p.sym.tiles * p.sym.ks;
        out->store_mode = p.store_mode;
        out->block_order = p.mfma_first;
        out->tiles16 = p.tiles16;
    }
    return EMI_OK;
}

int emi_last_path(emi_ctx_t c, int* fused) {
    if (!c || !fused) return EMI_ERR_ARG;
    *fused = choose_form(c, Launch{0, c->B}, EMI_EVAL_ALL).overlapped() ? 1 : 0;
    return EMI_OK;
}

int emi_debug_pass_roles(int nm, int nn, int order, int* out_role, int out_cap) {
    if (nm < 0 || nn < 0 || nm + nn < 1 || !out_role || out_cap < nm + nn) return EMI_ERR_ARG;
    for (int j = 0; j < nm + nn; ++j) {
        const emi::PassRole r = emi::pass_role_of(j, nm, nn, order);
        out_role[j] = r.mfma ? r.index : -1 - r.index;
    }
    return EMI_OK;
}

int emi_debug_tile_order(int ns, int B, int M, int sym_ct, int sym_cpart, int* out_tile, int out_cap, int* ntiles_total, int* cpart,
                         int* cx) {
    return emi_debug_tile_order2(ns, B, M, sym_ct, sym_cpart, 0, 0, out_tile, out_cap, ntiles_total, cpart, cx);
}

int emi_debug_tile_order2(int ns, int B, int M, int sym_ct, int sym_cpart, int sym_gblk, int sym_cx, int* out_tile, int out_cap,
                          int* ntiles_total, int* cpart, int* cx) {
    if (ns < 1 || B < 1 || M < 128 || M % 128 != 0 || !ntiles_total) return EMI_ERR_ARG;
    const emi::SymPlan p = emi::plan_symdefect(ns, B, M, sym_ct, 1, sym_cpart, sym_gblk, sym_cx);
    if (p.ring1 || p.sw < 1) return EMI_ERR_UNSUPPORTED;
    const int ntiles = (M / 2) / 64, ngrp = ((B + 15) / 16) * (ns / p.sw), total = ntiles * ngrp;
    *ntiles_total = total;
    if (cpart) *cpart = p.cpart;
    if (cx) *cx = p.cx;
    for (int t = 0; t < total && t < out_cap && out_tile; ++t) {
        const emi::RingTile rt = emi::ring_tile_of(t, ntiles, ngrp, p.cpart, p.cx, ns / p.sw);
        out_tile[t] = rt.ntile + ntiles * rt.grp;
    }
    return EMI_OK;
}

const char* emi_last_defect_kernel(emi_ctx_t c) {
    if (!c) return "";
    return c->last_defect_kernel.c_str();
}

}
```

etol_amd/csrc/emi_args.hpp:

```cpp
#pragma once
#ifdef __HIPCC_RTC__
#define EMI_PATH_ELLIPSE 0
#define EMI_PATH_DISC 1
#define EMI_PATH_TRACK 2
#define EMI_PATH_REC 8
#else
#include <hip/hip_runtime.h>
#include <stddef.h>
#include "emi355x.h"
#endif

#define EMI_NODE_THREADS 256

#ifdef EMI_TICKET_ACQ_REL
#define EMI_TICKET_ORDER __ATOMIC_ACQ_REL
#else
#define EMI_TICKET_ORDER __ATOMIC_RELAXED
#endif
#ifdef EMI_NO_M0_NOP
#define EMI_M0_NOP ""
#else
#define EMI_M0_NOP "s_nop 0\n\t"
#endif

#define DEF_TM 96
#define DEF_TN 128
#define DEF_BK 16

#define FUSED_TI 16
#define FUSED_BK 16

#include "emi_models.hpp"

namespace emi {

template <typename T> struct NodeArgs {
    const T* X;
    const T* U;
    T* RES;
    T* VALS;
    T* cost_part;
    T* cost;
    unsigned* cost_ticket;
    const T* w;
    const T* node_t;
    const T* Ddiag;
    const T* path;
    const T* track_x;
    const T* track_y;
    int M, B, np, nres, nvals;
    int path_sets, track_sets, ntracks;
    int px, py;
    int store_mode;
    int keep;
    T h, sgn;
    ModelParams<T> P;
};

template <typename T> struct HessArgs {
    const T* X;
    const T* U;
    const T* lamF;
    const T* lamC;
    T* H;
    const T* w;
    const T* node_t;
    const T* path;
    int M, B, np, path_sets, px, py;
    T h, sgn, sigma;
    ModelParams<T> P;
};

template <typename T> struct OdeResidArgs {
    const T* Zs;
    const T* Zc;
    const T* tq;
    const T* scale;
    const T* ul;
    const T* uu;
    T* eta;
    int M, B, lds, ldc;
    T h;
    ModelParams<T> P;
};

struct SymDefectArgs {
    const double* X;
    const double* U;
    double* RES;
    const double* node_t;
    const double* De;
    const double* Do;
    int M, B, nres;
    int order;
    int ablate;
    int ksplit;
    double* slab;
    unsigned* tile_ticket;
    int mfma_first;
    int cpart, cx;
    double h;
    ModelParams<double> P;
};

struct DefectArgs {
    const double* X;
    const double* D;
    double* RES;
    int R, M, ns, nres;
};
struct DefectArgsF32 {
    const float* X;
    const float* D;
    float* RES;
    int R, M, ns, nres;
};
struct RingTile { int ntile, grp; };
#if defined(__HIPCC__)
__host__ __device__
#endif
inline RingTile ring_tile_of(int tl, int ntiles, int ngrp, int cpart, int cx, int nsg = 1) {
    RingTile t;
    if (cpart > 0) {
        const int per_xcd = ngrp * ntiles / 8;
        const int x = tl / per_xcd, m = tl - x * per_xcd;
        const int pc = x % cpart, pg = x / cpart;
        const int ncol = ntiles / cpart, ng = ngrp / (8 / cpart);
        const int cb = m / (ng * cx), r = m - cb * ng * cx;
        t.grp = pg * ng + r / cx;
        t.ntile = pc * ncol + cb * cx + r % cx;
    } else if (cpart < 0) {
        const int G = -cpart, per_xcd = ngrp * ntiles / 8;
        const int x = tl / per_xcd, m = tl - x * per_xcd;
        const int per_sb = G * nsg * ntiles, sb = m / per_sb, r = m - sb * per_sb;
        const int per_cb = G * nsg * cx, cb = r / per_cb, r2 = r - cb * per_cb;
        const int g = r2 / (nsg * cx), r3 = r2 - g * (nsg * cx);
        const int mt = x * (ngrp / nsg / 8) + sb * G + g;
        t.grp = mt * nsg + r3 / cx;
        t.ntile = cb * cx + r3 % cx;
    } else {
        t.ntile = tl % ntiles;
        t.grp = tl / ntiles;
    }
    return t;
}
struct PassRole { int mfma, index; };
#if defined(__HIPCC__)
__host__ __device__
#endif
inline PassRole pass_role_of(int j, int nm, int nn, int order) {
    const long long t = (long long)nm + nn;
    long long m0, m1;
    const long long d = order >= 100 ? order : 100;
    if (order == 1 || d * nm > 100 * t) {
        m0 = j < nm ? j : nm;
        m1 = j < nm ? j + 1 : nm;
    } else {
        m0 = ((long long)j * nm * d) / (100 * t);
        m1 = ((long long)(j + 1) * nm * d) / (100 * t);
        if (m0 > nm) m0 = nm;
        if (m1 > nm) m1 = nm;
    }
    PassRole r;
    r.mfma = m1 > m0;
    r.index = (int)(r.mfma ? m0 : j - m0);
    return r;
}
struct PassArgs {
    SymDefectArgs s;
    NodeArgs<double> n;
    int nm8, nn8;
    int nm, nn;
    int nbx;
};

}
```

etol_amd/csrc/emi_ctx.hpp:

```cpp
#pragma once
#include <hip/hip_runtime.h>

#include <algorithm>
#include <cstdarg>
#include <cstdio>
#include <cstring>
#include <string>
#include <vector>

#include "emi355x.h"
#include "emi_device_array.hpp"
#include "emi_keep_record.hpp"
#include "emi_kernels.hpp"

namespace emi_api {

using DevBuf = emi::DeviceArray<unsigned char>;

enum ProfMark { E0, E1, E2, K0, K1, K2, K3, PROF_MARKS };
struct ProfEvents {
    hipEvent_t ev[PROF_MARKS] = {};
    bool has_node = false, has_defect = false, fused = false;
    int level = 0;
};

}
using emi_api::DevBuf, emi_api::ProfEvents;

struct emi_ctx_s {
    int device = 0;
    bool f32 = false;
    hipStream_t stream = nullptr;
    bool own_stream = false;
    hipStream_t stream2 = nullptr;
    hipEvent_t ev_fork = nullptr, ev_join = nullptr, ev_join2 = nullptr;
    int cu_split = 0;
    hipStream_t s_mfma = nullptr, s_node = nullptr;
    std::string err;
    std::string last_defect_kernel;

    int M = 0;
    double t0 = 0, tf = 0;
    DevBuf d_w, d_t, d_Ddiag, d_D, d_De, d_Do;
    bool symmetric = false;
    bool points_only = false;
    int allow_fused = 1;
    int sym_ct = 0;
    int sym_order = 1;
    int sym_ablate = 0;
    int small_rows = 24;
    int overlap_mode = 0;
    int node_store = -1;
    unsigned fused_attr_mask = 0;
    std::vector<double> h_tau, h_w;
    int model = -1, ns = 0, nc = 0, maximize = 0;
    double params[EMI_MAX_PARAMS] = {0};
    emi::KktWorkspace* kkt = nullptr;
    std::vector<emi::KktWorkspace*> kkt_shard;
    int kkt_method = 1;
    emi::RtcModel* rtc = nullptr;
    int B = 0;
    int np = 0, path_sets = 0, px = 0, py = 1;
    int np_model = 0;
    std::vector<int> pvars;
    DevBuf d_path;
    int ntracks = 0, track_sets = 0;
    DevBuf d_trkx, d_trky;
    int wp_ntracks = 0, wp_sets = 0, wp_ld = 0;
    emi::DeviceArray<double> d_wp;
    emi::DeviceArray<int> d_wp_cnt;
    emi::DeviceArray<double> d_wp_nt;
    bool wp_nt_dirty = true;
    DevBuf d_cost_part;
    DevBuf d_slab;
    DevBuf d_tile_ticket;
    DevBuf d_cost_part2;
    DevBuf d_ticket;
    int cost_in_kernel = 1;
    int sym_nst = 3;
    int sym_hs = 0;
    int sym_ctc = 0;
    int sym_bk = 0;
    int xh = 0, uh = 0, nch = 0;
    double delay_dt = 0.0;
    bool delay_dirty = true;
    DevBuf d_W;
    bool adjw_dirty = true;
    DevBuf d_adjWT;
    DevBuf d_adj_Gx;
    int adj_fold_tile = 0;
    DevBuf d_uext;
    int f32_ring_wgs = 2;
    int f32_ring = 1;
    int f32_one_launch = 0;
    int slice = 0;
    int sym_ksplit = 0;
    int sym_cpart = 0;
    int sym_gblk = 0, sym_cx = 0;
    int pass_order = -1;
    int sym_combine = 1;
    emi::KeepRecord keep;
    DevBuf s_X, s_U, s_RES, s_VALS, s_COST, s_LF, s_LC, s_H;
    std::vector<DevBuf> host_stage;
    DevBuf d_adjDT;
    bool adj_dirty = true;
    DevBuf d_adj_pvars;
    std::vector<int> adj_pvars;
    DevBuf d_adj_c;
    DevBuf d_adj_G;
    DevBuf d_adj_op;
    DevBuf s_G, s_cert, s_zl, s_zu, s_Gdel;
    bool ode_dirty = true;
    emi::DeviceArray<double> d_ode_op;
    emi::DeviceArray<double> d_ode_tq;
    emi::DeviceArray<double> d_ode_ub;
    emi::DeviceArray<double> d_ode_ws;
    bool blk_rows_set = false;
    std::vector<int> blk_row_ptr, blk_var, blk_entry;
    std::vector<int> blk_key;
    emi::DeviceArray<int> blk_term_ptr, blk_term_row, blk_term_ea, blk_term_eb, blk_flag, blk_list, blk_nflag, blk_cnt;
    emi::DeviceArray<double> blk_tdelta, blk_tvec, blk_tworst;
    int blk_generic = 0;
    std::vector<int> ipm_key;
    emi::DeviceArray<int> ipm_lists;
    int ipm_npairs = 0;
    std::vector<double> ipm_crow_h;
    emi::DeviceArray<double> ipm_crow, ipm_part;
    emi::IpmSolveWs* ipm_solve = nullptr;
    emi::IpmLadderWs* ipm_ladder = nullptr;
    emi::StartGuessWs* start_guess = nullptr;
    bool path_has_track = false;
    hipEvent_t t_start = nullptr, t_stop = nullptr;
    int profile = 0;
    std::vector<ProfEvents> prof;
    size_t prof_used = 0;
    bool attr_set = false;

    ~emi_ctx_s() {
        (void)hipSetDevice(device);
        if (stream) (void)hipStreamSynchronize(stream);
        for (ProfEvents& pe : prof)
            for (hipEvent_t e : pe.ev)
                if (e) (void)hipEventDestroy(e);
        for (hipStream_t s : {stream2, s_mfma, s_node})
            if (s) { (void)hipStreamSynchronize(s); (void)hipStreamDestroy(s); }
        for (hipEvent_t e : {ev_join2, ev_fork, ev_join, t_start, t_stop})
            if (e) (void)hipEventDestroy(e);
        if (own_stream && stream) (void)hipStreamDestroy(stream);
        emi::rtc_destroy(rtc);
        emi::kkt_destroy(kkt);
        for (emi::KktWorkspace* w : kkt_shard) emi::kkt_destroy(w);
        emi::ipm_solve_destroy(ipm_solve);
        emi::ipm_ladder_destroy(ipm_ladder);
        emi::start_guess_destroy(start_guess);
    }
};

#define HIP_TRY(c, call)                                                                                                                  \
    do {                                                                                                                                  \
        hipError_t e_ = (call);                                                                                                           \
        if (e_ != hipSuccess) return emi_api::fail((c), EMI_ERR_HIP, "%s failed: %s (%s:%d)", #call, hipGetErrorString(e_), __FILE__, __LINE__); \
    } while (0)
#define HIP_TRY_AS(c, who, call)                                                                                        \
    do {                                                                                                                \
        const hipError_t e_ = (call);                                                                                   \
        if (e_ != hipSuccess) return emi_api::fail((c), EMI_ERR_HIP, "%s: %s failed: %s", who, #call, hipGetErrorString(e_)); \
    } while (0)

#define EMI_TRY(call)              \
    do {                           \
        const int st_ = (call);    \
        if (st_) return st_;       \
    } while (0)

namespace emi_api {

int fail(emi_ctx_t c, int code, const char* fmt, ...);
inline int ensure(emi_ctx_t c, DevBuf& b, size_t bytes) {
    HIP_TRY(c, b.reserve(bytes));
    return EMI_OK;
}
inline int ensure_zeroed(emi_ctx_t c, DevBuf& b, size_t bytes, hipStream_t s) {
    if (b.bytes() >= bytes) return EMI_OK;
    EMI_TRY(ensure(c, b, bytes));
    HIP_TRY(c, hipMemsetAsync(b.p, 0, bytes, s));
    return EMI_OK;
}
int upload_bytes(emi_ctx_t c, DevBuf& b, const void* src, size_t bytes);
int upload_real(emi_ctx_t c, DevBuf& b, const double* src, size_t n);
int download_real(emi_ctx_t c, double* dst, const void* dsrc, size_t n);
int ensure_vals_staging(emi_ctx_t c, size_t bytes);

inline int np_total(emi_ctx_t c) { return c->np + c->np_model; }
inline int nvals_of(emi_ctx_t c) { return c->ns * (c->ns + c->nc) + 2 * c->np + c->np_model * (int)c->pvars.size() + (c->ns + c->nc); }
inline int nres_of(emi_ctx_t c) { return c->ns + np_total(c); }
inline int nhess_of(emi_ctx_t c) { const int nv = c->ns + c->nc; return nv * (nv + 1) / 2; }
inline int ready(emi_ctx_t c) {
    if (!c) return EMI_ERR_ARG;
    if (c->M <= 0) return fail(c, EMI_ERR_STATE, "emi_set_mesh has not been called");
    if (c->model < 0) return fail(c, EMI_ERR_STATE, "emi_set_model has not been called");
    if (c->B <= 0) return fail(c, EMI_ERR_STATE, "emi_set_batch has not been called");
    if (c->np > 0 && c->path_sets != 1 && c->path_sets != c->B)
        return fail(c, EMI_ERR_STATE, "path table has %d sets, batch is %d", c->path_sets, c->B);
    if (c->ntracks > 0 && c->track_sets != 1 && c->track_sets != c->B)
        return fail(c, EMI_ERR_STATE, "track table has %d sets, batch is %d", c->track_sets, c->B);
    return EMI_OK;
}

struct HostStager {
    emi_ctx_t c;
    size_t slot = 0;
    int status = EMI_OK;
    struct Out { void* host; void* dev; size_t bytes; };
    std::vector<Out> outs;
    explicit HostStager(emi_ctx_t c_) : c(c_) {}
    void* place(const void* host, size_t bytes, bool in, bool out);
    int finish();
};
#define HOST_STAGED_TRY(s, call)                                                          \
    if ((s).status) { (void)hipStreamSynchronize((s).c->stream); return (s).status; }     \
    if (const int st_ = (call)) { (void)hipStreamSynchronize((s).c->stream); return st_; }

int ensure_delay_matrices(emi_ctx_t c);
int need_stream2(emi_ctx_t c);
int path_row_list(emi_ctx_t c, const char* what, std::vector<int>& ptr, std::vector<int>& var, std::vector<int>& ent);
int shard_check(emi_ctx_t c, const char* what);
int ctx_ipm_launch(emi_ctx_t c, int what, const emi_ipm_bounds_t* bd, const void* dPar, emi::IpmArgs& a);

}
```

etol_amd/csrc/emi_kernels.hpp:

```cpp
#pragma once
#include <hip/hip_runtime.h>
#include <stddef.h>

#include <string>

#include "emi355x.h"
#include "emi_args.hpp"

static_assert(EMI_PATH_ELLIPSE == 0 && EMI_PATH_DISC == 1 && EMI_PATH_TRACK == 2 && EMI_PATH_REC == 8,
              "emi_args.hpp and emi355x.h disagree");

namespace emi {

int node_chunks(int M);
bool invariant_rows(int model, int np, unsigned char* mask);
template <typename T>
hipError_t launch_nodes(int model, const NodeArgs<T>& a, bool jac, bool defect_rows, hipStream_t s);
template <typename T> hipError_t launch_hess(int model, const HessArgs<T>& a, hipStream_t s);
hipError_t launch_defect_f64(const DefectArgs& a, hipStream_t s);
bool defect_small_supported(int R);
hipError_t launch_defect_small_f64(const DefectArgs& a, hipStream_t s);
hipError_t launch_defect_f32(const DefectArgsF32& a, hipStream_t s);
bool defect_f32_mfma_supported(int M);
hipError_t launch_defect_f32_mfma(const DefectArgsF32& a, hipStream_t s, int ring = 0, int wgs_per_cu = 2);
bool pass_f32_supported(int model, int R, int M, int B);
hipError_t launch_pass_f32(int model, const DefectArgsF32& d, const NodeArgs<float>& n, int order, hipStream_t s);
hipError_t defect_f64_set_attr();
template <typename T>
hipError_t launch_cost_finish(const T* part, T* cost, int B, int nchunks, T scale, hipStream_t s);
bool fused_supported(int model, int M, int ct);
struct SymPlan {
    bool ring1 = false;
    int sw = 0;
    int ks = 1;
    int nst = 3;
    int bk = 8;
    int hs = 1;
    int ct = 1;
    size_t slab_bytes = 0;
    int cpart = 0, cx = 0;
    int tiles = 0;
};
SymPlan plan_symdefect(int ns, int B, int M, int ct, int ksplit_opt, int cpart_opt = 0, int gblk_opt = 0, int cx_opt = 0, int bk_opt = 8, int ct_cols = 1);
hipError_t launch_symdefect(int model, const SymDefectArgs& a, hipStream_t s, bool set_attr, int ct, const SymPlan& plan);
bool pass_supported(int model, int ns, int B, int M, const SymPlan& plan);
hipError_t launch_pass(int model, const SymDefectArgs& sa, const NodeArgs<double>& na, hipStream_t s, const SymPlan& plan);

struct AdjointArgs {
    const double* VALS;
    const double* lamF;
    const double* lamC;
    const double* DT;
    const int* pvars;
    double* G;
    int B, M, ldt, ns, nc, np_table, np_traced, pw, px, py, nvals;
    int add_op;
    double sigma;
};
struct CertArgs {
    const double *X, *U, *RES, *VALS, *lamF, *lamC, *G;
    const double *zl, *zu;
    const double *cl, *cu;
    double* cert;
    int B, M, ns, nc, np, nres, nvals, nsets;
    int ncg;
    double sigma;
};
struct AdjointOpArgs {
    const double* A;
    const double* Bop;
    const double* add;
    double* out;
    int R, rpi, M, ldt, nseg, ldb;
    int a_inst, a_row0, a_seg, out_inst, out_row0, add_inst, add_row0;
};
hipError_t launch_adjoint_transpose(const double* dSrc, double* dDst, int M, int ldt, int ld_dst, int nseg, bool keep_diag, hipStream_t s);
bool adjoint_side_by_side(int B, int ns, int M);
hipError_t launch_adjoint_op(const AdjointArgs& a, hipStream_t s);
hipError_t launch_adjoint_product(const AdjointOpArgs& a, int tile, hipStream_t s);
hipError_t launch_adjoint_nodes(const AdjointArgs& a, hipStream_t s);
hipError_t launch_adjoint_add(const double* dGop, double* dG, int B, int ns, int nv, int M, hipStream_t s);
hipError_t launch_kkt_certificate(const CertArgs& a, hipStream_t s);

struct InterpOpArgs {
    const double* V;
    const double* OP;
    double* out;
    int R, K, N, ldk, ldo;
};
hipError_t launch_interp_op(const InterpOpArgs& a, hipStream_t s);
hipError_t launch_ode_copy_D(const double* D, double* dst, int M, int ldk, hipStream_t s);
hipError_t launch_ode_resid(int model, const OdeResidArgs<double>& a, hipStream_t s);
struct RtcModel;
hipError_t rtc_launch_ode_resid(RtcModel* m, const OdeResidArgs<double>& a, hipStream_t s);
struct OdeFinishArgs {
    const double* X;
    const double* Zs;
    const double* eta;
    double* err;
    int B, M, ns, lds, dcol;
    double h;
};
hipError_t launch_ode_finish(const OdeFinishArgs& a, hipStream_t s);

struct BlocksArgs {
    const double *H, *VALS, *Sigma, *SigT;
    const unsigned char* fixed;
    double dw_shift;
    double *Qexact, *Q;
    int max_mods;
    int* count;
    int* node;
    double *delta, *vec, *worst;
    int B, M, nv, np, nvals;
    int generic;
    const int *term_ptr, *term_row, *term_ea, *term_eb;
    int *flag, *list, *nflag, *cnt;
    double *tdelta, *tvec, *tworst;
};
hipError_t launch_kkt_blocks(const BlocksArgs& a, hipStream_t s);

struct IpmArgs {
    int B, M, ns, nc, np, nvals, nsets, reset;
    double *X, *U, *S, *E1, *E2;
    double *tX, *tU, *tS, *tE1, *tE2;
    double *LF, *Y, *ZL, *ZU, *VL, *VU, *W1, *W2;
    double *DZ, *DS, *DY, *DE1, *DE2, *DZL, *DZU, *DVL, *DVU, *DW1, *DW2;
    double *Sigma, *SigT, *SigS, *RhatS, *Rt, *Rhs;
    const double *RES, *VALS, *G, *COST, *DefRes, *RowRes, *rs;
    const double *zl, *zu;
    const double* crow;
    const double *par, *apr, *adu;
    const unsigned char* mask;
    const int *vptr, *vrow, *vent;
    const int *rptr, *rvar, *rent;
    double *part, *out;
    unsigned char* fixedb;
    double* LamC;
    double push, frac;
};
enum { IPM_REDUCE, IPM_EXPAND, IPM_TRIAL, IPM_MERIT, IPM_ACCEPT, IPM_ERROR, IPM_ERROR_PARTS, IPM_START_PUSH, IPM_START_ROWS, IPM_RESET_W, IPM_LAMC };
constexpr int IPM_MAX_PARTIALS = 9;
int ipm_chunks(int M);
hipError_t launch_ipm(int what, const IpmArgs& a, hipStream_t s);

struct RtcModel;
int rtc_check(bool f32, const char* struct_name, const char* source, int ns, int nc, int npath, int pw, std::string* log);
int rtc_build(bool f32, const char* struct_name, const char* source, int ns, int nc, int npath, int pw, RtcModel** out, std::string* log);
void rtc_destroy(RtcModel* m);
bool rtc_has_symdefect(const RtcModel* m);
template <typename T>
hipError_t rtc_launch_nodes(RtcModel* m, const NodeArgs<T>& a, bool jac, bool defect_rows, hipStream_t s);
template <typename T> hipError_t rtc_launch_hess(RtcModel* m, const HessArgs<T>& a, hipStream_t s);
hipError_t rtc_launch_symdefect(RtcModel* m, const SymDefectArgs& a, hipStream_t s);
int rtc_pass_sw_large(const RtcModel* m);
bool rtc_pass_supported(const RtcModel* m, int B, int M, int sw, int ks, int store_mode);
hipError_t rtc_launch_pass(RtcModel* m, const SymDefectArgs& sa, const NodeArgs<double>& na, int sw, hipStream_t s);
hipError_t rtc_launch_nodes_nt(RtcModel* m, const NodeArgs<double>& a, hipStream_t s);

struct KktWorkspace;
int kkt_factor(KktWorkspace** w, hipStream_t stream, const double* dD, int M, int ns, int nv, const double* Qblk,
               const double* Jblk, const unsigned char* fixed, double dc, int method, int* info, std::string* err,
               bool blocks_on_device = false);
int kkt_solve(KktWorkspace* w, hipStream_t stream, int nz, double* rhs, int nrhs, std::string* err,
              bool rhs_on_device = false);
bool kkt_set_option(const char* name, int value);
int kkt_lowrank(KktWorkspace* w, hipStream_t stream, int nz, int r, const int* node, const double* vec, const double* delta,
                int* exact, std::string* err);
void kkt_destroy(KktWorkspace* w);
void kkt_last_regularisation(const KktWorkspace* w, double* dc, double* dw);
void kkt_mesh_changed(KktWorkspace* w);
bool kkt_is_schur(const KktWorkspace* w);
struct KktShardSrc {
    const double* Q;
    const double* VALS;
    const unsigned char* fixed;
    size_t vals_stride;
    const int* inst;
};
int kkt_factor_batch(int n, KktWorkspace** const* pws, hipStream_t stream, const double* const* dD, int M, int ns, int nv,
                     const double* const* Qblk, const double* const* Jblk, const unsigned char* const* fixed, const double* dc, int* info,
                     std::string* err, const KktShardSrc* src = nullptr);
int kkt_solve_batch(int n, KktWorkspace* const* ws, hipStream_t stream, int nz, double* const* rhs, std::string* err,
                    bool rhs_on_device = false);
int kkt_solve_refined_batch(int n, KktWorkspace* const* ws, hipStream_t stream, double* const* rhs, const double* dc_nominal, int max_steps,
                            double* rel, int* nsolve, int* reverted, int* status, std::string* err, bool rhs_on_device = false);
int kkt_holds(const KktWorkspace* w, int M, int ns, int nv);
int kkt_lowrank_shard(int n, KktWorkspace* const* ws, hipStream_t stream, int max_mods, const int* inst, const int* count, const int* dNode,
                      const double* dDelta, const double* dVec, int* exact, std::string* err);
void kkt_forget_ladder(KktWorkspace* w);

struct IpmSolveWs;
void ipm_solve_destroy(IpmSolveWs* w);
int ipm_solve_shard(emi_ctx_t c, void* dX, void* dU, const emi_ipm_bounds_t* bd, const emi_ipm_options_t& opt, void* dLamF, void* dLamC,
                    emi_ipm_result_t* results);

struct IpmKeepArgs {
    double* live[13];
    double* kept[13];
    const unsigned char* mask;
    int B, M, ns, nc, np, restore;
};
hipError_t launch_ipm_keep(const IpmKeepArgs& a, hipStream_t s);

hipError_t launch_prolong_rows(const double* PT, const double* Vc, const int* map, int group, double* Vf, int Mc, int Mf, int R, hipStream_t s);
struct RepairArgs {
    double* X;
    const double *recs, *trkx, *trky;
    int B, ns, M, np, path_sets, px, py, ntracks, track_sets;
};
hipError_t launch_repair_guess(const RepairArgs& a, hipStream_t s);
struct TrackWaypointArgs {
    const double *t, *x, *y, *node_t;
    const int *cnt, *map;
    void *xc, *yc;
    int n, ntracks, ld, M, first;
};
template <typename T> hipError_t launch_track_waypoints(TrackWaypointArgs a, hipStream_t s);
struct IpmLadderWs;
void ipm_ladder_destroy(IpmLadderWs* w);
struct StartArgs {
    double* X;
    int* level;
    const double *recs, *par, *tau, *sine;
    double *cost, *dist, *extra;
    int* cells;
    unsigned char* bits;
    int B, ns, M, np, path_sets, px, py, nsets, kind, N, has_box;
    double bend, clearance;
};
struct StartGuessWs;
void start_guess_destroy(StartGuessWs* w);
int start_guess(emi_ctx_t c, const emi_start_t& st, void* dX, void* dLevel);
int ipm_solve_ladder(emi_ctx_t c, int nrungs, const emi_ipm_rung_t* rungs, double t0, double tf, const void* dX0, const void* dU0, void* dX,
                     void* dU, void* dLamF, void* dLamC, emi_ipm_result_t* results);
constexpr int SHARD_MOVE_ARRAYS = 4;
struct ShardMoveArgs {
    const double* src[SHARD_MOVE_ARRAYS];
    double* dst[SHARD_MOVE_ARRAYS];
    int rows[SHARD_MOVE_ARRAYS], sld[SHARD_MOVE_ARRAYS], dld[SHARD_MOVE_ARRAYS];
    const int *sidx, *didx;
    int n, narrays, len, first;
};
hipError_t launch_shard_move(ShardMoveArgs a, hipStream_t s);
int ipm_solve_refine(emi_ctx_t c, int nrungs, const emi_ipm_rung_t* rungs, double t0, double tf, const emi_ipm_refine_t& rf, const void* dX0,
                     const void* dU0, int ldm, void* dX, void* dU, void* dLamF, void* dLamC, emi_ipm_result_t* results, double* err,
                     emi_ipm_refine_result_t* out);

}
```

etol_amd/csrc/emi_symdefect.hip:

```cpp
#include <hip/hip_runtime.h>

#include <algorithm>
#include <type_traits>

#include "emi_kernels.hpp"
#include "emi_models.hpp"
#include "emi_symdefect_kernels.hpp"

namespace emi {

template <class Model>
static hipError_t launch_symdefect_ring_model(const SymDefectArgs& a, hipStream_t s, bool set_attr) {
    constexpr int NS = Model::NS;
    const int mtiles = (a.B + FUSED_TI - 1) / FUSED_TI, ntiles = (a.M / 2) / 64;
    const size_t lds = (size_t)3 * (2 * NS * FUSED_TI + 2 * 64) * 16 * sizeof(double);
    if (set_attr) {
        hipError_t e = hipFuncSetAttribute((const void*)emi_symdefect_ring_f64_kernel<Model>,
                                           hipFuncAttributeMaxDynamicSharedMemorySize, (int)lds);
        if (e != hipSuccess) return e;
    }
    dim3 grid(mtiles * ntiles), block(256);
    hipLaunchKernelGGL((emi_symdefect_ring_f64_kernel<Model>), grid, block, lds, s, a);
    return hipGetLastError();
}

template <class Model, int CT>
static hipError_t launch_symdefect_model(const SymDefectArgs& a, hipStream_t s, bool set_attr) {
    constexpr int NS = Model::NS, TN = 64 * CT;
    const int mtiles = (a.B + FUSED_TI - 1) / FUSED_TI, ntiles = (a.M / 2) / TN;
    const size_t lds = (size_t)2 * (2 * NS * FUSED_TI + 2 * TN) * (FUSED_BK + 2) * sizeof(double);
    if (set_attr) {
        hipError_t e = hipFuncSetAttribute((const void*)emi_symdefect_f64_kernel<Model, CT>,
                                           hipFuncAttributeMaxDynamicSharedMemorySize, (int)lds);
        if (e != hipSuccess) return e;
    }
    dim3 grid(mtiles * ntiles), block(256);
    hipLaunchKernelGGL((emi_symdefect_f64_kernel<Model, CT>), grid, block, lds, s, a);
    return hipGetLastError();
}

template <class Model, int SW>
static hipError_t launch_ring2_model(const SymDefectArgs& a, hipStream_t s) {
    constexpr int NS = Model::NS;
    const int mtiles = (a.B + FUSED_TI - 1) / FUSED_TI, ntiles = (a.M / 2) / 64;
    const size_t lds = (size_t)3 * ((2 * SW * FUSED_TI + 2 * 64 + 63) / 64 * 64) * 8 * sizeof(double);
    static bool attr_done = false;
    if (!attr_done) {
        hipError_t e = hipFuncSetAttribute((const void*)emi_symdefect_ring2_f64_kernel<Model, SW>,
                                           hipFuncAttributeMaxDynamicSharedMemorySize, (int)lds);
        if (e != hipSuccess) return e;
        attr_done = true;
    }
    const int tiles = mtiles * ntiles * (NS / SW), ks = a.ksplit > 1 ? a.ksplit : 1;
    hipLaunchKernelGGL((emi_symdefect_ring2_f64_kernel<Model, SW>), dim3(tiles * ks), dim3(256), lds, s, a);
    if (ks > 1 && a.tile_ticket == nullptr) hipLaunchKernelGGL((emi_symdefect_combine_kernel<Model, SW>), dim3(tiles), dim3(256), 0, s, a);
    return hipGetLastError();
}

SymPlan plan_symdefect(int ns, int B, int M, int ct, int ksplit_opt, int cpart_opt, int gblk_opt, int cx_opt, int bk_opt, int ct_cols) {
    SymPlan p;
    p.bk = bk_opt == 16 ? 16 : 8;
    const int tiles = ((B + FUSED_TI - 1) / FUSED_TI) * ((M / 2) / 64);
    const int nkt = (M / 2) / p.bk;
    if (ct == 0 || ct == 4) {
        if (tiles >= 448) p.sw = (ns % 2 == 0 && ns > 2) ? 2 : ns;
        else if (tiles >= 320) p.sw = ns;
        else if (tiles >= 192) { p.ring1 = true; return p; }
        else p.sw = (tiles <= 96 || ns % 2 != 0 || ns <= 2) ? 1 : 2;
    } else if (ct >= 5 && ct <= 8) {
        p.sw = ct == 5 ? ns : (ct == 6 ? 2 : (ct == 8 ? 3 : 1));
        if (ns % p.sw != 0) p.sw = 1;
    } else {
        p.ring1 = true;
        return p;
    }
    if (ksplit_opt > 0) p.ks = ksplit_opt;
    while (p.ks > 1 && (nkt % p.ks != 0 || nkt / p.ks < 2 || (nkt / p.ks) % 2 != 0)) p.ks >>= 1;
    p.ct = (ct_cols == 2 && p.sw == 2 && p.ks == 1 && M % 256 == 0) ? 2 : 1;
    const int TNp = 64 * p.ct;
    p.tiles = (tiles / p.ct) * (ns / p.sw);
    {
        const int ntiles = (M / 2) / TNp, ngrp = ((B + FUSED_TI - 1) / FUSED_TI) * (ns / p.sw);
        const int target_cols = std::max(1, 4096 / M / p.ct);
        auto valid = [&](int cp) { return cp >= 1 && cp <= 8 && ntiles % cp == 0 && ngrp % (8 / cp) == 0 && (ngrp * ntiles) % 8 == 0; };
        int cp = 0;
        if (cpart_opt > 0) cp = valid(cpart_opt) ? cpart_opt : 0;
        else if (cpart_opt == 0 && tiles >= 192)
            for (int c = 1; c <= 8 && !cp; c *= 2)
                if (valid(c) && (ntiles / c <= target_cols || c == 8 || !valid(2 * c))) cp = c;
        const int mtiles = (B + FUSED_TI - 1) / FUSED_TI;
        if (gblk_opt > 0 && mtiles % (8 * gblk_opt) == 0 && (ngrp * ntiles) % 8 == 0) {
            int cxg = cx_opt > 0 ? cx_opt : 2;
            while (cxg > 1 && ntiles % cxg != 0) --cxg;
            p.cpart = -gblk_opt;
            p.cx = cxg;
        } else if (cp > 0) {
            p.cpart = cp;
            p.cx = 1;
            for (int d = 1; d <= std::min(ntiles / cp, target_cols); ++d)
                if ((ntiles / cp) % d == 0) p.cx = d;
            if (cp == 1 && p.cx == ntiles) p.cpart = p.cx = 0;
        }
    }
    if (p.ks > 1) p.slab_bytes = (size_t)p.tiles * p.ks * (2 * p.sw * 4) * 256 * sizeof(double);
    return p;
}

template <class Model>
static hipError_t launch_ring2_planned(const SymDefectArgs& a, hipStream_t s, const SymPlan& p) {
    constexpr int NS = Model::NS;
    if (p.sw == NS) return launch_ring2_model<Model, NS>(a, s);
    if constexpr (NS > 2 && NS % 2 == 0) {
        if (p.sw == 2) return launch_ring2_model<Model, 2>(a, s);
    }
    if constexpr (NS > 3 && NS % 3 == 0) {
        if (p.sw == 3) return launch_ring2_model<Model, 3>(a, s);
    }
    return launch_ring2_model<Model, 1>(a, s);
}

template <class Model, int SW, int NST, int BK = 8, int CT = 1, int HS = 1>
static hipError_t launch_pass_model(const SymDefectArgs& sa, const NodeArgs<double>& na, hipStream_t s) {
    constexpr int NS = Model::NS;
    PassArgs a;
    a.s = sa;
    a.n = na;
    const int mtiles = (sa.B + FUSED_TI - 1) / FUSED_TI, ntiles = (sa.M / 2) / (64 * CT);
    const int nm = mtiles * ntiles * (NS / SW) * (sa.ksplit > 1 ? sa.ksplit : 1);
    a.nbx = (na.M + 2 * EMI_NODE_THREADS - 1) / (2 * EMI_NODE_THREADS);
    const int nn = a.nbx * na.B;
    a.nm = nm;
    a.nn = nn;
    a.nm8 = (nm + 7) / 8;
    a.nn8 = ((nn + HS - 1) / HS + 7) / 8;
    const size_t lds = (size_t)HS * NST * ((2 * SW * FUSED_TI + 2 * 64 * CT + 63) / 64 * 64) * BK * sizeof(double);
    const int st = (na.store_mode >= 0 && na.store_mode <= 3) ? na.store_mode : 0;
    constexpr bool HAS_KEEP = NST == 3 && HS == 1;
    const bool keep = HAS_KEEP && na.keep;
    auto pick = [&](auto keep_c) {
        constexpr bool K = decltype(keep_c)::value;
        return st == 2 ? emi_pass_f64_kernel<Model, SW, 2, 2, NST, BK, CT, HS, K>
             : (st == 1 ? emi_pass_f64_kernel<Model, SW, 2, 1, NST, BK, CT, HS, K>
                        : (st == 3 ? emi_pass_f64_kernel<Model, SW, 2, 3, NST, BK, CT, HS, K> : emi_pass_f64_kernel<Model, SW, 2, 0, NST, BK, CT, HS, K>));
    };
    auto kern = pick(std::false_type{});
    if constexpr (HAS_KEEP) {
        if (keep) kern = pick(std::true_type{});
    }
    static bool attr_done[2][4] = {};
    if (!attr_done[keep][st]) {
        hipError_t e = hipFuncSetAttribute((const void*)kern, hipFuncAttributeMaxDynamicSharedMemorySize, (int)lds);
        if (e != hipSuccess) return e;
        attr_done[keep][st] = true;
    }
    hipLaunchKernelGGL(kern, dim3(8 * (a.nm8 + a.nn8)), dim3(256 * HS), lds, s, a);
    return hipGetLastError();
}

template <class Model>
static hipError_t launch_pass_planned(const SymDefectArgs& sa, const NodeArgs<double>& na, hipStream_t s, const SymPlan& p) {
    constexpr int NS = Model::NS;
    if (p.sw == NS) return launch_pass_model<Model, NS, 3>(sa, na, s);
    if constexpr (NS > 2 && NS % 2 == 0) {
        if (p.sw == 2 && p.hs == 2 && p.ct == 1) return p.bk == 16 ? launch_pass_model<Model, 2, 3, 16, 1, 2>(sa, na, s) : launch_pass_model<Model, 2, 3, 8, 1, 2>(sa, na, s);
        if (p.sw == 2 && p.ct == 2) return p.bk == 16 ? launch_pass_model<Model, 2, 3, 16, 2>(sa, na, s) : launch_pass_model<Model, 2, 3, 8, 2>(sa, na, s);
        if (p.sw == 2 && p.bk == 16) return launch_pass_model<Model, 2, 3, 16>(sa, na, s);
        if (p.sw == 2) return p.nst > 3 ? launch_pass_model<Model, 2, 4>(sa, na, s) : launch_pass_model<Model, 2, 3>(sa, na, s);
    }
    if constexpr (NS > 3 && NS % 3 == 0) {
        if (p.sw == 3) return launch_pass_model<Model, 3, 3>(sa, na, s);
    }
    if (p.hs == 2) return p.bk == 16 ? launch_pass_model<Model, 1, 3, 16, 1, 2>(sa, na, s) : launch_pass_model<Model, 1, 3, 8, 1, 2>(sa, na, s);
    if (p.bk == 16) return launch_pass_model<Model, 1, 3, 16>(sa, na, s);
    return p.nst > 3 ? launch_pass_model<Model, 1, 4>(sa, na, s) : launch_pass_model<Model, 1, 3>(sa, na, s);
}

bool pass_supported(int model, int ns, int B, int M, const SymPlan& p) {
    if (p.ring1 || p.sw < 1 || (model != EMI_MODEL_POINTMASS2D && model != EMI_MODEL_QUADROTOR2D)) return false;
    if (M % 128 != 0 || ns % p.sw != 0) return false;
    return B >= 1;
}

hipError_t launch_pass(int model, const SymDefectArgs& sa, const NodeArgs<double>& na, hipStream_t s, const SymPlan& p) {
    if (model == EMI_MODEL_POINTMASS2D) return launch_pass_planned<PointMass2D<double>>(sa, na, s, p);
    if (model == EMI_MODEL_QUADROTOR2D) return launch_pass_planned<Quadrotor2D<double>>(sa, na, s, p);
    return hipErrorInvalidValue;
}

bool fused_supported(int model, int M, int ct) {
    if (ct == 0 || (ct >= 4 && ct <= 8))
        return (model == EMI_MODEL_POINTMASS2D || model == EMI_MODEL_QUADROTOR2D) && M >= 128 && M % 128 == 0;
    const int w = ct == 2 ? 2 : 1;
    return (model == EMI_MODEL_POINTMASS2D || model == EMI_MODEL_QUADROTOR2D) && ct >= 1 && ct <= 3 &&
           M >= 128 * w && M % (128 * w) == 0;
}

hipError_t launch_symdefect(int model, const SymDefectArgs& a, hipStream_t s, bool set_attr, int ct, const SymPlan& plan) {
    if (!plan.ring1) {
        if (model == EMI_MODEL_POINTMASS2D) return launch_ring2_planned<PointMass2D<double>>(a, s, plan);
        if (model == EMI_MODEL_QUADROTOR2D) return launch_ring2_planned<Quadrotor2D<double>>(a, s, plan);
        return hipErrorInvalidValue;
    }
    if (ct == 0 || ct >= 4) {
        ct = 3;
        set_attr = true;
    }
    if (ct == 3) {
        if (model == EMI_MODEL_POINTMASS2D) return launch_symdefect_ring_model<PointMass2D<double>>(a, s, set_attr);
        if (model == EMI_MODEL_QUADROTOR2D) return launch_symdefect_ring_model<Quadrotor2D<double>>(a, s, set_attr);
        return hipErrorInvalidValue;
    }
    if (model == EMI_MODEL_POINTMASS2D)
        return ct == 1 ? launch_symdefect_model<PointMass2D<double>, 1>(a, s, set_attr)
                       : launch_symdefect_model<PointMass2D<double>, 2>(a, s, set_attr);
    if (model == EMI_MODEL_QUADROTOR2D)
        return ct == 1 ? launch_symdefect_model<Quadrotor2D<double>, 1>(a, s, set_attr)
                       : launch_symdefect_model<Quadrotor2D<double>, 2>(a, s, set_attr);
    return hipErrorInvalidValue;
}

}
```

etol_amd/csrc/emi_symdefect_kernels.hpp:

```cpp
#pragma once
#include "emi_args.hpp"
#include "emi_node_kernels.hpp"

namespace emi {

typedef double d4 __attribute__((ext_vector_type(4)));

template <class Model, int CT>
__global__ __launch_bounds__(256, CT == 1 ? 2 : 1) void emi_symdefect_f64_kernel(SymDefectArgs a) {
    constexpr int NS = Model::NS, NC = Model::NC, NV = Model::NV;
    constexpr int TI = FUSED_TI, TM = NS * TI, TN = 64 * CT, BK = FUSED_BK, LDK = BK + 2;
    constexpr int A_PASS = TM * (BK / 2) / 256;
    constexpr int B_PASS = TN * (BK / 2) / 256;
    static_assert(TM * (BK / 2) % 256 == 0 && TN * (BK / 2) % 256 == 0, "staging shape");
    static_assert(TN % 64 == 0 && TI == 16, "wave layout below assumes 16 instances x 64*CT columns");
    constexpr int STAGE = (2 * TM + 2 * TN) * LDK;

    extern __shared__ __attribute__((aligned(16))) double smem[];

    const int M = a.M, Hh = M >> 1, B = a.B;
    const int mtiles = (B + TI - 1) / TI;
    int bid = blockIdx.x;
    {
        const int nwg = gridDim.x, xcd = bid & 7, q = nwg >> 3, rr = nwg & 7;
        bid = (xcd < rr ? xcd * (q + 1) : rr * (q + 1) + (xcd - rr) * q) + (bid >> 3);
    }
    const int ntiles_ = gridDim.x / mtiles;
    const int ntile = a.order ? bid % ntiles_ : bid / mtiles;
    const int mtile = a.order ? bid / ntiles_ : bid - ntile * mtiles;
    const int inst0 = mtile * TI, i0 = ntile * TN;

    const int tid = threadIdx.x, lane = tid & 63, wid = tid >> 6;
    const int r16 = lane & 15, kq = lane >> 4;

    d4 acc_a[NS][CT], acc_b[NS][CT];
#pragma unroll
    for (int s = 0; s < NS; ++s)
#pragma unroll
        for (int c = 0; c < CT; ++c) {
            acc_a[s][c] = d4{0.0, 0.0, 0.0, 0.0};
            acc_b[s][c] = d4{0.0, 0.0, 0.0, 0.0};
        }

    double2 pe[A_PASS], po[A_PASS], pde[B_PASS], pdo[B_PASS];
    auto gload = [&](int k0) {
#pragma unroll
        for (int p = 0; p < A_PASS; ++p) {
            const int idx = tid + 256 * p, row = idx >> 3, c2 = idx & 7;
            const int inst = inst0 + (row & 15), st = row >> 4;
            double2 v = make_double2(0.0, 0.0), m = v;
            if (inst < B) {
                const double* xr = a.X + ((size_t)inst * NS + st) * M;
                const int j = k0 + 2 * c2;
                v = *reinterpret_cast<const double2*>(xr + j);
                m = *reinterpret_cast<const double2*>(xr + (M - 2 - j));
            }
            pe[p] = make_double2(v.x + m.y, v.y + m.x);
            po[p] = make_double2(v.x - m.y, v.y - m.x);
        }
#pragma unroll
        for (int p = 0; p < B_PASS; ++p) {
            const int idx = tid + 256 * p, row = idx >> 3, c2 = idx & 7;
            const size_t off = (size_t)(i0 + row) * Hh + k0 + 2 * c2;
            const double2 te = *reinterpret_cast<const double2*>(a.De + off);
            const double2 to = *reinterpret_cast<const double2*>(a.Do + off);
            pde[p] = make_double2(te.x, te.y);
            pdo[p] = make_double2(to.x, to.y);
        }
    };
    auto lstore = [&](int buf) {
        double* Es = smem + (size_t)buf * STAGE;
        double* Os = Es + TM * LDK;
        double* Des = Os + TM * LDK;
        double* Dos = Des + TN * LDK;
#pragma unroll
        for (int p = 0; p < A_PASS; ++p) {
            const int idx = tid + 256 * p, row = idx >> 3, c2 = idx & 7;
            *reinterpret_cast<double2*>(Es + row * LDK + 2 * c2) = pe[p];
            *reinterpret_cast<double2*>(Os + row * LDK + 2 * c2) = po[p];
        }
#pragma unroll
        for (int p = 0; p < B_PASS; ++p) {
            const int idx = tid + 256 * p, row = idx >> 3, c2 = idx & 7;
            *reinterpret_cast<double2*>(Des + row * LDK + 2 * c2) = pde[p];
            *reinterpret_cast<double2*>(Dos + row * LDK + 2 * c2) = pdo[p];
        }
    };

    const int nkt = Hh / BK;
    gload(0);
    lstore(0);
    __syncthreads();
    int cur = 0;
    for (int kt = 0; kt < nkt; ++kt) {
        if (kt + 1 < nkt) gload((kt + 1) * BK);
        const double* Es = smem + (size_t)cur * STAGE;
        const double* Os = Es + TM * LDK;
        const double* Db = Os + TM * LDK + (wid * (16 * CT) + r16) * LDK + kq;
        const double* Ob = Db + TN * LDK;
#pragma unroll 2
        for (int ks = 0; ks < BK / 4; ++ks) {
            double bfe[CT], bfo[CT];
#pragma unroll
            for (int c = 0; c < CT; ++c) {
                bfe[c] = Db[c * 16 * LDK + ks * 4];
                bfo[c] = Ob[c * 16 * LDK + ks * 4];
            }
#pragma unroll
            for (int s = 0; s < NS; ++s) {
                const double afe = Es[(s * 16 + r16) * LDK + ks * 4 + kq];
                const double afo = Os[(s * 16 + r16) * LDK + ks * 4 + kq];
#pragma unroll
                for (int c = 0; c < CT; ++c) {
                    acc_a[s][c] = __builtin_amdgcn_mfma_f64_16x16x4f64(afe, bfe[c], acc_a[s][c], 0, 0, 0);
                    acc_b[s][c] = __builtin_amdgcn_mfma_f64_16x16x4f64(afo, bfo[c], acc_b[s][c], 0, 0, 0);
                }
            }
        }
        if (kt + 1 < nkt) {
            lstore(cur ^ 1);
            __syncthreads();
            cur ^= 1;
        }
    }

#pragma unroll
    for (int c = 0; c < CT; ++c) {
        const int col = wid * (16 * CT) + c * 16 + r16;
        const int node_f = i0 + col, node_m = M - 1 - node_f;
#pragma unroll
        for (int i = 0; i < 4; ++i) {
            const int inst = inst0 + kq + 4 * i;
            if (inst >= B) continue;
            const double* __restrict__ Xb = a.X + (size_t)inst * NS * M;
            const double* __restrict__ Ub = a.U + (size_t)inst * NC * M;
            double* __restrict__ Rb = a.RES + (size_t)inst * a.nres * M;
#pragma unroll
            for (int side = 0; side < 2; ++side) {
                const int node = side == 0 ? node_f : node_m;
                double z[NV], f[NS];
#pragma unroll
                for (int v = 0; v < NS; ++v) z[v] = Xb[(size_t)v * M + node];
#pragma unroll
                for (int v = 0; v < NC; ++v) z[NS + v] = Ub[(size_t)v * M + node];
                Model::f(a.P, z, a.node_t[node], f);
#pragma unroll
                for (int s = 0; s < NS; ++s) {
                    const double dx = side == 0 ? acc_a[s][c][i] + acc_b[s][c][i] : acc_b[s][c][i] - acc_a[s][c][i];
                    Rb[(size_t)s * M + node] = dx - a.h * f[s];
                }
            }
        }
    }
}

typedef __attribute__((address_space(3))) void* emi_lds_ptr_t;
typedef const __attribute__((address_space(1))) void* emi_glb_ptr_t;

template <class Model>
__global__ __launch_bounds__(256, 2) void emi_symdefect_ring_f64_kernel(SymDefectArgs a) {
    constexpr int NS = Model::NS, NC = Model::NC, NV = Model::NV;
    constexpr int TI = FUSED_TI, TM = NS * TI, TN = 64, BK = 16, NST = 3;
    constexpr int STAGE = (2 * TM + 2 * TN) * BK;
    constexpr int NINSTR = (2 * TM + 2 * TN) * 8 / 64;
    constexpr int L = NINSTR / 4;
    static_assert(NINSTR % 4 == 0, "stage does not split evenly over 4 waves");

    extern __shared__ __attribute__((aligned(16))) double smem[];

    const int M = a.M, Hh = M >> 1, B = a.B;
    const int mtiles = (B + TI - 1) / TI;
    int bid = blockIdx.x;
    {
        const int nwg = gridDim.x, xcd = bid & 7, q = nwg >> 3, rr = nwg & 7;
        bid = (xcd < rr ? xcd * (q + 1) : rr * (q + 1) + (xcd - rr) * q) + (bid >> 3);
    }
    const int ntiles_ = gridDim.x / mtiles;
    const int ntile = a.order ? bid % ntiles_ : bid / mtiles;
    const int mtile = a.order ? bid / ntiles_ : bid - ntile * mtiles;
    const int inst0 = mtile * TI, i0 = ntile * TN;

    const int tid = threadIdx.x, lane = tid & 63;
    const int wid = __builtin_amdgcn_readfirstlane(tid >> 6);
    const int r16 = lane & 15, kq = lane >> 4;

    const double* src[L];
    int kdir[L];
#pragma unroll
    for (int t = 0; t < L; ++t) {
        const int q = (wid + 4 * t) * 64 + lane;
        int row, p;
        if (q < 2 * TM * 8) {
            const bool mir = q >= TM * 8;
            const int qr = mir ? q - TM * 8 : q;
            row = qr >> 3; p = qr & 7;
            const int c = p ^ ((row >> 1) & 7);
            int inst = inst0 + (row & 15);
            inst = inst < B ? inst : B - 1;
            const double* xr = a.X + ((size_t)inst * NS + (row >> 4)) * M;
            src[t] = mir ? xr + (M - BK) + 2 * c : xr + 2 * c;
            kdir[t] = mir ? -1 : 1;
        } else {
            const bool od = q >= (2 * TM + TN) * 8;
            const int qr = q - (2 * TM + (od ? TN : 0)) * 8;
            row = qr >> 3; p = qr & 7;
            const int c = p ^ ((row >> 1) & 7);
            src[t] = (od ? a.Do : a.De) + (size_t)(i0 + row) * Hh + 2 * c;
            kdir[t] = 1;
        }
    }
    const unsigned lds0 = (unsigned)(unsigned long)(emi_lds_ptr_t)smem;
    auto issue = [&](int stage, int kt) {
#pragma unroll
        for (int t = 0; t < L; ++t) {
            const unsigned dst = lds0 + (unsigned)stage * (unsigned)(STAGE * 8) + (unsigned)(wid + 4 * t) * 1024u;
            const double* g = src[t] + (ptrdiff_t)kdir[t] * kt * BK;
            asm volatile("s_mov_b32 m0, %1\n\t" EMI_M0_NOP "global_load_lds_dwordx4 %0, off" ::"v"(g), "s"(dst) : "memory", "m0");
        }
    };

    d4 acc_a[NS], acc_b[NS];
#pragma unroll
    for (int s = 0; s < NS; ++s) {
        acc_a[s] = d4{0.0, 0.0, 0.0, 0.0};
        acc_b[s] = d4{0.0, 0.0, 0.0, 0.0};
    }

    const int nkt = Hh / BK;
    issue(0, 0);
    if (nkt > 1) issue(1, 1);
    for (int kt = 0; kt < nkt; ++kt) {
        if (kt + 1 < nkt) asm volatile("s_waitcnt vmcnt(%0)" ::"n"(L) : "memory");
        else              asm volatile("s_waitcnt vmcnt(0)" ::: "memory");
        asm volatile("s_barrier" ::: "memory");
        if (kt + 2 < nkt && !(a.ablate & 2)) issue((kt + 2) % NST, kt + 2);
        if (a.ablate & 1) continue;
        const double* XF = smem + (size_t)(kt % NST) * STAGE;
        const double* XM = XF + TM * BK;
        const double* DE = XM + TM * BK;
        const double* DO = DE + TN * BK;
        const int rb = wid * 16 + r16, swb = (rb >> 1) & 7;
        double xf_c[NS], xm_c[NS], be_c, bo_c;
        auto frag = [&](int ks, double (&xf)[NS], double (&xm)[NS], double& be, double& bo) {
            const int kk = ks * 4 + kq, km = BK - 1 - kk;
            const int pb = ((kk >> 1) ^ swb) * 2 + (kk & 1);
            be = DE[rb * BK + pb];
            bo = DO[rb * BK + pb];
#pragma unroll
            for (int s = 0; s < NS; ++s) {
                const int r = s * 16 + r16, sw = (r >> 1) & 7;
                xf[s] = XF[r * BK + ((kk >> 1) ^ sw) * 2 + (kk & 1)];
                xm[s] = XM[r * BK + ((km >> 1) ^ sw) * 2 + (km & 1)];
            }
        };
        frag(0, xf_c, xm_c, be_c, bo_c);
#pragma unroll
        for (int ks = 0; ks < BK / 4; ++ks) {
            double xf_n[NS], xm_n[NS], be_n = 0.0, bo_n = 0.0;
            if (ks + 1 < BK / 4) frag(ks + 1, xf_n, xm_n, be_n, bo_n);
#pragma unroll
            for (int s = 0; s < NS; ++s) {
                acc_a[s] = __builtin_amdgcn_mfma_f64_16x16x4f64(xf_c[s] + xm_c[s], be_c, acc_a[s], 0, 0, 0);
                acc_b[s] = __builtin_amdgcn_mfma_f64_16x16x4f64(xf_c[s] - xm_c[s], bo_c, acc_b[s], 0, 0, 0);
            }
            if (ks + 1 < BK / 4) {
#pragma unroll
                for (int s = 0; s < NS; ++s) { xf_c[s] = xf_n[s]; xm_c[s] = xm_n[s]; }
                be_c = be_n;
                bo_c = bo_n;
            }
        }
    }

    const int col = wid * 16 + r16;
    const int node_f = i0 + col, node_m = M - 1 - node_f;
#pragma unroll
    for (int i = 0; i < 4; ++i) {
        const int inst = inst0 + kq + 4 * i;
        if (inst >= B || (a.ablate & 4)) continue;
        const double* __restrict__ Xb = a.X + (size_t)inst * NS * M;
        const double* __restrict__ Ub = a.U + (size_t)inst * NC * M;
        double* __restrict__ Rb = a.RES + (size_t)inst * a.nres * M;
#pragma unroll
        for (int side = 0; side < 2; ++side) {
            const int node = side == 0 ? node_f : node_m;
            double z[NV], f[NS];
#pragma unroll
            for (int v = 0; v < NS; ++v) z[v] = Xb[(size_t)v * M + node];
#pragma unroll
            for (int v = 0; v < NC; ++v) z[NS + v] = Ub[(size_t)v * M + node];
            Model::f(a.P, z, a.node_t[node], f);
#pragma unroll
            for (int s = 0; s < NS; ++s) {
                const double dx = side == 0 ? acc_a[s][i] + acc_b[s][i] : acc_b[s][i] - acc_a[s][i];
                Rb[(size_t)s * M + node] = dx - a.h * f[s];
            }
        }
    }
}

EMI_DEV constexpr int ring_swz(int r) { return (0 - (r >> 2)) & 3; }
#ifndef EMI_EPILOGUE_PREFETCH
#define EMI_EPILOGUE_PREFETCH 0
#endif
template <int BK> EMI_DEV constexpr int ring_swz_k(int r) { return BK == 8 ? ring_swz(r) : ((r >> 1) & 7); }

template <class Model>
EMI_DEV void ring_epilogue_load(const SymDefectArgs& a, double (&z)[2][Model::NV], int inst, int node_f) {
    constexpr int NS = Model::NS, NC = Model::NC;
    const int M = a.M, node_m = M - 1 - node_f;
    inst = inst < a.B ? inst : a.B - 1;
    const double* __restrict__ Xb = a.X + (size_t)inst * NS * M;
    const double* __restrict__ Ub = a.U + (size_t)inst * NC * M;
#pragma unroll
    for (int side = 0; side < 2; ++side) {
        const int node = side == 0 ? node_f : node_m;
#pragma unroll
        for (int v = 0; v < NS; ++v) z[side][v] = Xb[(size_t)v * M + node];
#pragma unroll
        for (int v = 0; v < NC; ++v) z[side][NS + v] = Ub[(size_t)v * M + node];
    }
}
template <class Model, int SW, int S0, bool PRE>
EMI_DEV void ring_epilogue_s0(const SymDefectArgs& a, const d4 (&acc_a)[SW], const d4 (&acc_b)[SW], int inst0, int i0,
                              int wid, int r16, int kq, const double (&zpre)[2][Model::NV]) {
    constexpr int NS = Model::NS, NC = Model::NC, NV = Model::NV;
    const int M = a.M, B = a.B;
    const int col = wid * 16 + r16;
    const int node_f = i0 + col, node_m = M - 1 - node_f;
    const double t_f = a.node_t[node_f], t_m = a.node_t[node_m];
    if constexpr (SW == 1) {
        if (a.ablate & 4) return;
        double zz[4][2][NV];
#pragma unroll
        for (int i = 0; i < 4; ++i) {
            int inst = inst0 + kq + 4 * i;
            inst = inst < B ? inst : B - 1;
            const double* __restrict__ Xb = a.X + (size_t)inst * NS * M;
            const double* __restrict__ Ub = a.U + (size_t)inst * NC * M;
#pragma unroll
            for (int side = 0; side < 2; ++side) {
                const int node = side == 0 ? node_f : node_m;
#pragma unroll
                for (int v = 0; v < NS; ++v) zz[i][side][v] = Xb[(size_t)v * M + node];
#pragma unroll
                for (int v = 0; v < NC; ++v) zz[i][side][NS + v] = Ub[(size_t)v * M + node];
            }
        }
#pragma unroll
        for (int i = 0; i < 4; ++i) {
            const int inst = inst0 + kq + 4 * i;
            if (inst >= B) continue;
            double* __restrict__ Rb = a.RES + (size_t)inst * a.nres * M;
#pragma unroll
            for (int side = 0; side < 2; ++side) {
                double f[NS];
                Model::f(a.P, zz[i][side], side == 0 ? t_f : t_m, f);
                const double dx = side == 0 ? acc_a[0][i] + acc_b[0][i] : acc_b[0][i] - acc_a[0][i];
                Rb[(size_t)S0 * M + (side == 0 ? node_f : node_m)] = dx - a.h * f[S0];
            }
        }
        return;
    }
    if (a.ablate & 4) return;
    auto load_z = [&](double (&z)[2][NV], int i) {
        int inst = inst0 + kq + 4 * i;
        inst = inst < B ? inst : B - 1;
        const double* __restrict__ Xb = a.X + (size_t)inst * NS * M;
        const double* __restrict__ Ub = a.U + (size_t)inst * NC * M;
#pragma unroll
        for (int side = 0; side < 2; ++side) {
            const int node = side == 0 ? node_f : node_m;
#pragma unroll
            for (int v = 0; v < NS; ++v) z[side][v] = Xb[(size_t)v * M + node];
#pragma unroll
            for (int v = 0; v < NC; ++v) z[side][NS + v] = Ub[(size_t)v * M + node];
        }
    };
    double zc[2][NV], zn[2][NV];
    if constexpr (PRE) {
#pragma unroll
        for (int side = 0; side < 2; ++side)
#pragma unroll
            for (int v = 0; v < NV; ++v) zc[side][v] = zpre[side][v];
    } else {
        load_z(zc, 0);
    }
#pragma unroll
    for (int i = 0; i < 4; ++i) {
        if (i < 3) load_z(zn, i + 1);
        const int inst = inst0 + kq + 4 * i;
        if (inst < B) {
            double* __restrict__ Rb = a.RES + (size_t)inst * a.nres * M;
            double hf[2][SW];
#pragma unroll
            for (int side = 0; side < 2; ++side) {
                double f[NS];
                Model::f(a.P, zc[side], side == 0 ? t_f : t_m, f);
#pragma unroll
                for (int s = 0; s < SW; ++s) hf[side][s] = a.h * f[S0 + s];
            }
#pragma unroll
            for (int side = 0; side < 2; ++side) {
                const int node = side == 0 ? node_f : node_m;
#pragma unroll
                for (int s = 0; s < SW; ++s) {
                    const double dx = side == 0 ? acc_a[s][i] + acc_b[s][i] : acc_b[s][i] - acc_a[s][i];
                    Rb[(size_t)(S0 + s) * M + node] = dx - hf[side][s];
                }
            }
        }
        if (i < 3) {
#pragma unroll
            for (int side = 0; side < 2; ++side)
#pragma unroll
                for (int v = 0; v < NV; ++v) zc[side][v] = zn[side][v];
        }
    }
}
template <class Model, int SW, bool PRE, int SG = 0>
EMI_DEV void ring_epilogue_pre(const SymDefectArgs& a, const d4 (&acc_a)[SW], const d4 (&acc_b)[SW], int inst0, int i0,
                               int s0, int wid, int r16, int kq, const double (&zpre)[2][Model::NV]) {
    if constexpr (SG * SW < Model::NS) {
        if (s0 == SG * SW) ring_epilogue_s0<Model, SW, SG * SW, PRE>(a, acc_a, acc_b, inst0, i0, wid, r16, kq, zpre);
        else ring_epilogue_pre<Model, SW, PRE, SG + 1>(a, acc_a, acc_b, inst0, i0, s0, wid, r16, kq, zpre);
    }
}
template <class Model, int SW>
EMI_DEV void ring_epilogue(const SymDefectArgs& a, const d4 (&acc_a)[SW], const d4 (&acc_b)[SW], int inst0, int i0,
                           int s0, int wid, int r16, int kq) {
    const double none[2][Model::NV] = {};
    ring_epilogue_pre<Model, SW, false>(a, acc_a, acc_b, inst0, i0, s0, wid, r16, kq, none);
}

template <class Model, int SW, int NST = 3, int BK = 8, int CT = 1, int HS = 1>
EMI_DEV void emi_ring2_body(const SymDefectArgs& a, const int bid ) {
    constexpr int NS = Model::NS;
    constexpr int TI = FUSED_TI, TM = SW * TI, TN = 64 * CT, CH = BK / 2, NSG = NS / SW;
    static_assert(CT == 1 || CT == 2, "one or two column sub-tiles per wave");
    constexpr int KH = BK / 8;
    constexpr int RPI = 64 / CH;
    static_assert(BK == 8 || BK == 16, "K tiles of 8 or 16");
    constexpr int LOOK = NST - 1;
    constexpr int ROWS = 2 * TM + 2 * TN;
    constexpr int ROWS_PAD = (ROWS + 63) / 64 * 64;
    constexpr int STAGE = ROWS_PAD * BK;
    constexpr int L = ROWS_PAD * CH / 256;
    static_assert(NS % SW == 0, "states split evenly over workgroups");

    extern __shared__ __attribute__((aligned(16))) double smem_all[];
    static_assert(HS == 1 || HS == 2, "the K range whole or in two halves");
    const int half = HS > 1 ? __builtin_amdgcn_readfirstlane((int)(threadIdx.x >> 8)) : 0;
    double* const smem = smem_all + (size_t)half * NST * STAGE;

    const int M = a.M, Hh = M >> 1, B = a.B;
    const int ntiles = Hh / TN;
    const int KS = (HS == 1 && a.ksplit > 1) ? a.ksplit : 1;
    const int kslice = bid % KS;
    const RingTile rt = ring_tile_of(bid / KS, ntiles, (B + TI - 1) / TI * NSG, a.cpart, a.cx, NSG);
    const int ntile = rt.ntile, grp = rt.grp;
    const int tile = grp * ntiles + ntile;
    const int sg = grp % NSG, mtile = grp / NSG;
    const int inst0 = mtile * TI, i0 = ntile * TN, s0 = sg * SW;

    const int tid = threadIdx.x & 255, lane = tid & 63;
    const int wid = __builtin_amdgcn_readfirstlane(tid >> 6);
    const int r16 = lane & 15, kq = lane >> 4;

    unsigned voff[L];
    unsigned long long gbase[L];
    int gstep[L];
#pragma unroll
    for (int t = 0; t < L; ++t) {
        const int row0 = (wid + 4 * t) * RPI;
        const int row = row0 + lane / CH, p = lane % CH;
        if (row0 < 2 * TM) {
            const bool mir = row0 >= TM;
            const int rr = row - (mir ? TM : 0);
            const int c = p ^ ring_swz_k<BK>(rr);
            int inst = inst0 + (rr & 15);
            inst = inst < B ? inst : B - 1;
            if (a.ablate & 8) inst &= 15;
            voff[t] = (unsigned)((((size_t)inst * NS + s0 + (rr >> 4)) * M + 2 * c) * sizeof(double));
            gbase[t] = (unsigned long long)(a.X + (mir ? M - BK : 0));
            gstep[t] = mir ? -(int)(BK * sizeof(double)) : (int)(BK * sizeof(double));
        } else if (row0 < ROWS) {
            const bool od = row0 >= 2 * TM + TN;
            const int rr = row - 2 * TM - (od ? TN : 0);
            const int c = p ^ ring_swz_k<BK>(rr);
            voff[t] = (unsigned)(((size_t)((a.ablate & 64) ? rr : i0 + rr) * Hh + 2 * c) * sizeof(double));
            gbase[t] = (unsigned long long)(od ? a.Do : a.De);
            gstep[t] = (int)(BK * sizeof(double));
        } else {
            voff[t] = (unsigned)(2 * p * sizeof(double));
            gbase[t] = (unsigned long long)a.De;
            gstep[t] = 0;
        }
    }
    const unsigned lds0 = (unsigned)(unsigned long)(emi_lds_ptr_t)smem;
    const int nkt = (Hh / BK) / KS / HS, kt0 = (kslice * HS + half) * nkt;
    unsigned long long gnext[L];
#pragma unroll
    for (int t = 0; t < L; ++t) gnext[t] = gbase[t] + (long long)gstep[t] * kt0;
    unsigned st_dma = 0, st_rd = 0;
    int nd = 0;
    auto issue_one = [&](int t) {
        const unsigned dst = lds0 + st_dma + (unsigned)(wid + 4 * t) * 1024u;
        asm volatile("s_mov_b32 m0, %2\n\t" EMI_M0_NOP "global_load_lds_dwordx4 %0, %1" ::"v"(voff[t]), "s"(gnext[t]), "s"(dst) : "memory", "m0");
        gnext[t] += (long long)gstep[t];
        if (t == L - 1) {
            st_dma = st_dma == (unsigned)((NST - 1) * STAGE * 8) ? 0u : st_dma + (unsigned)(STAGE * 8);
            ++nd;
        }
    };
    auto issue = [&]() {
#pragma unroll
        for (int t = 0; t < L; ++t) issue_one(t);
    };

    d4 acc_a[SW][CT], acc_b[SW][CT];
#pragma unroll
    for (int s = 0; s < SW; ++s)
#pragma unroll
        for (int c = 0; c < CT; ++c) {
            acc_a[s][c] = d4{0.0, 0.0, 0.0, 0.0};
            acc_b[s][c] = d4{0.0, 0.0, 0.0, 0.0};
        }

    constexpr bool EPI_PRE = EMI_EPILOGUE_PREFETCH && SW >= 2 && SW <= 3 && HS == 1 && CT == 1;
    double zpre[2][Model::NV] = {};
    if constexpr (EPI_PRE) ring_epilogue_load<Model>(a, zpre, inst0 + kq, i0 + wid * 16 + r16);

#pragma unroll
    for (int t = 0; t < LOOK; ++t)
        if (t < nkt) issue();
    int off_b[CT][KH], off_f[SW][KH], off_m[SW][KH];
#pragma unroll
    for (int c = 0; c < CT; ++c) {
        const int rb = c * 64 + wid * 16 + r16;
#pragma unroll
        for (int h = 0; h < KH; ++h) off_b[c][h] = rb * BK + (((kq + 4 * h) ^ ring_swz_k<BK>(rb)) << 1);
    }
#pragma unroll
    for (int s = 0; s < SW; ++s) {
        const int r = s * 16 + r16;
#pragma unroll
        for (int h = 0; h < KH; ++h) {
            off_f[s][h] = r * BK + (((kq + 4 * h) ^ ring_swz_k<BK>(r)) << 1);
            off_m[s][h] = (TM + r) * BK + (((CH - 1 - kq - 4 * h) ^ ring_swz_k<BK>(r)) << 1);
        }
    }
    struct Frag {
        double2 be[CT][KH], bo[CT][KH], sp[SW][KH], dm[SW][KH];
    };
    double2 txf[SW][KH], txm[SW][KH];
    constexpr int NRH = 2 * CT + 2 * SW;
    constexpr int NR = NRH * KH, NM = 4 * SW * CT * KH;
    auto read_one = [&](Frag& f, const double* S, int r) {
        const int h = r / NRH, q = r % NRH;
        if (q < 2 * CT) {
            if (q & 1) f.bo[q >> 1][h] = *reinterpret_cast<const double2*>(S + (2 * TM + TN) * BK + off_b[q >> 1][h]);
            else f.be[q >> 1][h] = *reinterpret_cast<const double2*>(S + 2 * TM * BK + off_b[q >> 1][h]);
        } else if (q & 1) txm[(q - 2 * CT) >> 1][h] = *reinterpret_cast<const double2*>(S + off_m[(q - 2 * CT) >> 1][h]);
        else txf[(q - 2 * CT) >> 1][h] = *reinterpret_cast<const double2*>(S + off_f[(q - 2 * CT) >> 1][h]);
    };
    auto sums_one = [&](Frag& f, int s) {
#pragma unroll
        for (int h = 0; h < KH; ++h) {
            f.sp[s][h] = double2{txf[s][h].x + txm[s][h].y, txf[s][h].y + txm[s][h].x};
            f.dm[s][h] = double2{txf[s][h].x - txm[s][h].y, txf[s][h].y - txm[s][h].x};
        }
    };
    auto rd_stage = [&]() -> const double* {
        const double* S = smem + (st_rd >> 3);
        st_rd = st_rd == (unsigned)((NST - 1) * STAGE * 8) ? 0u : st_rd + (unsigned)(STAGE * 8);
        return S;
    };
    auto read_frag = [&](Frag& f) {
        const double* S = rd_stage();
#pragma unroll
        for (int r = 0; r < NR; ++r) read_one(f, S, r);
#pragma unroll
        for (int s = 0; s < SW; ++s) sums_one(f, s);
    };
    auto mfma_one = [&](const Frag& f, int i) {
        const int per = 2 * SW * CT, q = i % per, j = i / per, h = j >> 1;
        const int s = q / (2 * CT), c = (q >> 1) % CT;
        const bool second = j & 1, odd = q & 1;
        if (!odd) acc_a[s][c] = __builtin_amdgcn_mfma_f64_16x16x4f64(second ? f.sp[s][h].y : f.sp[s][h].x, second ? f.be[c][h].y : f.be[c][h].x, acc_a[s][c], 0, 0, 0);
        else      acc_b[s][c] = __builtin_amdgcn_mfma_f64_16x16x4f64(second ? f.dm[s][h].y : f.dm[s][h].x, second ? f.bo[c][h].y : f.bo[c][h].x, acc_b[s][c], 0, 0, 0);
    };
    auto multiply = [&](const Frag& f) {
#pragma unroll
        for (int i = 0; i < NM; ++i) mfma_one(f, i);
    };
    if constexpr (SW <= 3) {
        constexpr int RPG = (NR + (NM - L) - 1) / (NM - L);
        constexpr int GR = (NR + RPG - 1) / RPG;
        static_assert(NM > L && GR + L <= NM, "a gap for every DMA instruction after the reads");
        auto step = [&](const Frag& cur, Frag& nxt, int kt) {
            if (kt + LOOK < nkt) asm volatile("s_waitcnt vmcnt(%0)" ::"n"(L * (LOOK - 1)) : "memory");
            else                 asm volatile("s_waitcnt vmcnt(0)" ::: "memory");
            __builtin_amdgcn_s_waitcnt(0xC07F);
            asm volatile("s_barrier" ::: "memory");
            const bool more = nd < nkt;
            const double* S = rd_stage();
#pragma unroll
            for (int i = 0; i < NM; ++i) {
                mfma_one(cur, i);
                if (i < GR) {
#pragma unroll
                    for (int r = i * RPG; r < (i + 1) * RPG && r < NR; ++r) read_one(nxt, S, r);
                } else if (i < GR + L) {
                    if (more) issue_one(i - GR);
                }
                if (i >= NM - SW) sums_one(nxt, i - (NM - SW));
                __builtin_amdgcn_sched_barrier(0);
            }
        };
        Frag f0, f1;
        if (nkt > LOOK - 1) asm volatile("s_waitcnt vmcnt(%0)" ::"n"(L * (LOOK - 1)) : "memory");
        else                asm volatile("s_waitcnt vmcnt(0)" ::: "memory");
        asm volatile("s_barrier" ::: "memory");
        if (LOOK < nkt) issue();
        __builtin_amdgcn_s_waitcnt(0xC07F);
        read_frag(f0);
        int kt = 0;
        for (; kt + 2 < nkt; kt += 2) {
            step(f0, f1, kt);
            step(f1, f0, kt + 1);
        }
        step(f0, f1, kt);
        multiply(f1);
    } else {
        for (int kt = 0; kt < nkt; ++kt) {
            if (kt + LOOK - 1 < nkt) asm volatile("s_waitcnt vmcnt(%0)" ::"n"(L * (LOOK - 1)) : "memory");
            else                     asm volatile("s_waitcnt vmcnt(0)" ::: "memory");
            asm volatile("s_barrier" ::: "memory");
            if (kt + LOOK < nkt) issue();
            Frag f;
            read_frag(f);
            multiply(f);
        }
    }

    if (CT == 1 && KS > 1) {
        double* sl = a.slab + ((size_t)tile * KS + kslice) * (2 * SW * 4) * 256 + tid;
        if (a.tile_ticket == nullptr) {
#pragma unroll
            for (int s = 0; s < SW; ++s)
#pragma unroll
                for (int i = 0; i < 4; ++i) {
                    sl[(size_t)((2 * s) * 4 + i) * 256] = acc_a[s][0][i];
                    sl[(size_t)((2 * s + 1) * 4 + i) * 256] = acc_b[s][0][i];
                }
            return;
        }
#pragma unroll
        for (int s = 0; s < SW; ++s)
#pragma unroll
            for (int i = 0; i < 4; ++i) {
                __hip_atomic_store(sl + (size_t)((2 * s) * 4 + i) * 256, acc_a[s][0][i], __ATOMIC_RELAXED, __HIP_MEMORY_SCOPE_AGENT);
                __hip_atomic_store(sl + (size_t)((2 * s + 1) * 4 + i) * 256, acc_b[s][0][i], __ATOMIC_RELAXED, __HIP_MEMORY_SCOPE_AGENT);
            }
        asm volatile("s_waitcnt vmcnt(0)" ::: "memory");
        __syncthreads();
        unsigned* flag = reinterpret_cast<unsigned*>(smem);
        if (tid == 0) *flag = __hip_atomic_fetch_add(a.tile_ticket + tile, 1u, EMI_TICKET_ORDER, __HIP_MEMORY_SCOPE_AGENT);
        __syncthreads();
        if (*flag != (unsigned)KS - 1u) return;
#pragma unroll
        for (int s = 0; s < SW; ++s) {
            acc_a[s][0] = d4{0.0, 0.0, 0.0, 0.0};
            acc_b[s][0] = d4{0.0, 0.0, 0.0, 0.0};
        }
        for (int k = 0; k < KS; ++k) {
            const double* sk = a.slab + ((size_t)tile * KS + k) * (2 * SW * 4) * 256 + tid;
#pragma unroll
            for (int s = 0; s < SW; ++s)
#pragma unroll
                for (int i = 0; i < 4; ++i) {
                    acc_a[s][0][i] += __hip_atomic_load(sk + (size_t)((2 * s) * 4 + i) * 256, __ATOMIC_RELAXED, __HIP_MEMORY_SCOPE_AGENT);
                    acc_b[s][0][i] += __hip_atomic_load(sk + (size_t)((2 * s + 1) * 4 + i) * 256, __ATOMIC_RELAXED, __HIP_MEMORY_SCOPE_AGENT);
                }
        }
        if (tid == 0) __hip_atomic_store(a.tile_ticket + tile, 0u, __ATOMIC_RELAXED, __HIP_MEMORY_SCOPE_AGENT);
    }
    __builtin_amdgcn_s_setprio(0);
    if constexpr (HS == 2) {
        asm volatile("s_waitcnt lgkmcnt(0)" ::: "memory");
        __syncthreads();
        double* cb = smem_all + tid;
        if (half == 1) {
#pragma unroll
            for (int s2 = 0; s2 < SW; ++s2)
#pragma unroll
                for (int c = 0; c < CT; ++c)
#pragma unroll
                    for (int i = 0; i < 4; ++i) {
                        cb[(size_t)(((2 * s2) * CT + c) * 4 + i) * 256] = acc_a[s2][c][i];
                        cb[(size_t)(((2 * s2 + 1) * CT + c) * 4 + i) * 256] = acc_b[s2][c][i];
                    }
        }
        __syncthreads();
        if (half == 1) return;
#pragma unroll
        for (int s2 = 0; s2 < SW; ++s2)
#pragma unroll
            for (int c = 0; c < CT; ++c)
#pragma unroll
                for (int i = 0; i < 4; ++i) {
                    acc_a[s2][c][i] += cb[(size_t)(((2 * s2) * CT + c) * 4 + i) * 256];
                    acc_b[s2][c][i] += cb[(size_t)(((2 * s2 + 1) * CT + c) * 4 + i) * 256];
                }
    }
#pragma unroll
    for (int c = 0; c < CT; ++c) {
        d4 ea[SW], eb[SW];
#pragma unroll
        for (int s2 = 0; s2 < SW; ++s2) { ea[s2] = acc_a[s2][c]; eb[s2] = acc_b[s2][c]; }
        if (c == 0) ring_epilogue_pre<Model, SW, EPI_PRE>(a, ea, eb, inst0, i0, s0, wid, r16, kq, zpre);
        else ring_epilogue<Model, SW>(a, ea, eb, inst0, i0 + 64 * c, s0, wid, r16, kq);
    }
}

template <class Model, int SW>
__global__ __launch_bounds__(256, 2) void emi_symdefect_ring2_f64_kernel(SymDefectArgs a) {
    int bid = blockIdx.x;
    {
        const int nwg = gridDim.x, xcd = bid & 7, q = nwg >> 3, rr = nwg & 7;
        bid = (xcd < rr ? xcd * (q + 1) : rr * (q + 1) + (xcd - rr) * q) + (bid >> 3);
    }
    emi_ring2_body<Model, SW>(a, bid);
}

template <class Model, int SW>
__global__ __launch_bounds__(256) void emi_symdefect_combine_kernel(SymDefectArgs a) {
    constexpr int NS = Model::NS, TI = FUSED_TI, TN = 64, NSG = NS / SW;
    const int ntiles = (a.M >> 1) / TN, KS = a.ksplit;
    const int tile = blockIdx.x;
    const int ntile = tile % ntiles, grp = tile / ntiles;
    const int sg = grp % NSG, mtile = grp / NSG;
    const int tid = threadIdx.x, lane = tid & 63, wid = tid >> 6;
    d4 acc_a[SW], acc_b[SW];
#pragma unroll
    for (int s = 0; s < SW; ++s) {
        acc_a[s] = d4{0.0, 0.0, 0.0, 0.0};
        acc_b[s] = d4{0.0, 0.0, 0.0, 0.0};
    }
    for (int k = 0; k < KS; ++k) {
        const double* sl = a.slab + ((size_t)tile * KS + k) * (2 * SW * 4) * 256 + tid;
#pragma unroll
        for (int s = 0; s < SW; ++s)
#pragma unroll
            for (int i = 0; i < 4; ++i) {
                acc_a[s][i] += sl[(size_t)((2 * s) * 4 + i) * 256];
                acc_b[s][i] += sl[(size_t)((2 * s + 1) * 4 + i) * 256];
            }
    }
    ring_epilogue<Model, SW>(a, acc_a, acc_b, mtile * TI, ntile * TN, sg * SW, wid, lane & 15, lane >> 4);
}


#define EMI_STR2(x) #x
#define EMI_STR(x) EMI_STR2(x)
#ifndef EMI_PASS_WAVES_PER_EU
#define EMI_PASS_WAVES_PER_EU 0
#endif
#if EMI_PASS_WAVES_PER_EU > 0
#define EMI_PASS_OCC __attribute__((amdgpu_waves_per_eu(EMI_PASS_WAVES_PER_EU, EMI_PASS_WAVES_PER_EU)))
#elif EMI_PASS_WAVES_PER_EU < 0
#define EMI_PASS_OCC
#else
#define EMI_PASS_OCC __attribute__((amdgpu_waves_per_eu(SW > 3 ? 1 : 2, 2)))
#endif
template <class Model, int SW, int VEC, int ST, int NST = 3, int BK = 8, int CT = 1, int HS = 1, bool KEEP = false>
__global__ __launch_bounds__(256 * HS) EMI_PASS_OCC void emi_pass_f64_kernel(PassArgs a) {
#ifdef EMI_ENTRY_PAD_NOPS
    asm volatile(".rept " EMI_STR(EMI_ENTRY_PAD_NOPS) "\n\ts_nop 0\n\t.endr" ::: "memory");
#endif
    const int g = blockIdx.x, xcd = g & 7, j = g >> 3;
    const PassRole role = pass_role_of(j, a.nm8, a.nn8, a.s.mfma_first);
    if (a.s.ablate & (role.mfma ? 16 : 32)) return;
    if (role.mfma) {
        const int tid = xcd * a.nm8 + role.index;
        if (tid >= a.nm) return;
        __builtin_amdgcn_s_setprio(3);
        emi_ring2_body<Model, SW, NST, BK, CT, HS>(a.s, tid);
    } else {
        const int nid = (xcd * a.nn8 + role.index) * HS + (HS > 1 ? (int)(threadIdx.x >> 8) : 0);
        if (nid >= a.nn) return;
        emi_nodes_body<double, Model, VEC, true, false, ST, false, KEEP>(a.n, nid % a.nbx, nid / a.nbx, a.nbx);
    }
}

}
```

include/emi355x.h:

```cpp
#ifndef EMI355X_H_
#define EMI355X_H_

#include <stddef.h>

#ifdef __cplusplus
extern "C" {
#endif

#define EMI_ABI_VERSION 2

typedef struct emi_ctx_s* emi_ctx_t;

enum {
    EMI_OK = 0,
    EMI_ERR_ARG = 1,
    EMI_ERR_STATE = 2,
    EMI_ERR_HIP = 3,
    EMI_ERR_NO_DEVICE = 4,
    EMI_ERR_UNSUPPORTED = 5,
    EMI_ERR_COMM = 6
};

enum {
    EMI_MODEL_POINTMASS2D = 0,
    EMI_MODEL_QUADROTOR2D = 1,
    EMI_MODEL_FIXEDWING12 = 2,
    EMI_MODEL_SOURCE = 100
};

enum {
    EMI_PATH_ELLIPSE = 0,
    EMI_PATH_DISC = 1,
    EMI_PATH_TRACK = 2
};
#define EMI_PATH_REC 8

enum {
    EMI_EVAL_NODES = 1u,
    EMI_EVAL_DEFECT = 2u,
    EMI_EVAL_ALL = 3u,
    EMI_EVAL_NOJAC = 4u,
    EMI_EVAL_KEEP_INVARIANT = 8u
};

typedef struct {
    int model, ns, nc, np, M, B;
    int nres;
    int nvals;
    int nhess;
    int real_bytes;
    int px, py;
    double t0, tf;
} emi_layout_t;

int emi_abi_version(void);
const char* emi_status_string(int status);
int emi_device_count(int* count);

int emi_lgl(int M, double* tau, double* w, double* D);
int emi_model_dims(int model, int* ns, int* nc, int* nparams);
int emi_edge_ellipse(double xa, double ya, double xb, double yb, double* rec8);
int emi_track_centres(int nway, const double* t, const double* x, const double* y,
                      int M, const double* node_t, double* xc, double* yc);

int emi_create(int device_id, emi_ctx_t* out);
int emi_create_f32(int device_id, emi_ctx_t* out);
int emi_destroy(emi_ctx_t ctx);
const char* emi_last_error(emi_ctx_t ctx);
int emi_set_stream(emi_ctx_t ctx, void* hip_stream);
int emi_get_stream(emi_ctx_t ctx, void** hip_stream);
int emi_synchronize(emi_ctx_t ctx);

int emi_set_mesh(emi_ctx_t ctx, int M, const double* tau, const double* w,
                 const double* D, double t0, double tf);
int emi_set_model(emi_ctx_t ctx, int model, const double* params, int nparams,
                  int maximize);
int emi_set_model_source(emi_ctx_t ctx, const char* struct_name, const char* source,
                         int ns, int nc, int npath, const int* path_vars, int n_path_vars,
                         const double* params, int nparams, int maximize);
int emi_check_model_source(const char* struct_name, const char* source, int ns,
                           int nc, int npath, int n_path_vars, int f32, char* log, size_t log_len);
int emi_set_batch(emi_ctx_t ctx, int B);
int emi_set_delays(emi_ctx_t ctx, int x_horizon, int u_horizon, double dt);
int emi_get_delays(emi_ctx_t ctx, int* x_horizon, int* u_horizon, int* n_delayed);
int emi_delay_matrix(int M, const double* tau, const double* w, double t0, double tf, double delay, double* W);
int emi_set_path(emi_ctx_t ctx, int np, int nsets, const double* recs,
                 int px_state, int py_state);
int emi_set_tracks(emi_ctx_t ctx, int ntracks, int nsets, const double* xc,
                   const double* yc);
int emi_set_track_waypoints(emi_ctx_t ctx, int ntracks, int nsets, int ld, const int* counts, const double* t, const double* x,
                            const double* y);
int emi_tracks_from_waypoints_dev(emi_ctx_t ctx, int n, const void* dSetMap);
int emi_get_tracks(emi_ctx_t ctx, double* xc, double* yc);
int emi_get_layout(emi_ctx_t ctx, emi_layout_t* out);

int emi_kkt_factor(emi_ctx_t ctx, const double* Qblk, const double* Jblk,
                   const unsigned char* fixed, double dc, int* info);
int emi_kkt_lowrank(emi_ctx_t ctx, int r, const int* node, const double* vec,
                    const double* delta, int* exact);
int emi_kkt_factor_batch(int n, const emi_ctx_t* ctxs, const double* const* Qblk,
                         const double* const* Jblk, const unsigned char* const* fixed,
                         const double* dc, int* info);
int emi_kkt_solve_batch(int n, const emi_ctx_t* ctxs, double* const* rhs);
int emi_kkt_is_schur(emi_ctx_t ctx);
int emi_kkt_solve_refined(emi_ctx_t ctx, double* rhs, double dc_nominal, int max_steps,
                          double* rel, int* nsolve, int* reverted, int* status);
int emi_kkt_solve_refined_batch(int n, const emi_ctx_t* ctxs, double* const* rhs,
                                const double* dc_nominal, int max_steps, double* rel,
                                int* nsolve, int* reverted, int* status);
int emi_kkt_last_regularisation(emi_ctx_t ctx, double* dc, double* dw);
int emi_kkt_factor_dev(emi_ctx_t ctx, const void* dQblk, const void* dJblk, const void* dFixed, double dc, int* info);

int emi_kkt_blocks_rows(emi_ctx_t ctx, int np, const int* row_ptr, const int* var, const int* entry);
int emi_kkt_blocks_dev(emi_ctx_t ctx, const void* dH, const void* dVALS, const void* dSigma, const void* dSigT,
                       const void* dFixed, double dw_shift, void* dQexact, void* dQ, int max_mods, void* dCount, void* dNode,
                       void* dDelta, void* dVec, void* dWorst);
int emi_kkt_blocks_host(emi_ctx_t ctx, const double* H, const double* VALS, const double* Sigma, const double* SigT,
                        const unsigned char* fixed, double dw_shift, double* Qexact, double* Q, int max_mods, int* count,
                        int* node, double* delta, double* vec, double* worst);
int emi_kkt_solve(emi_ctx_t ctx, double* rhs, int nrhs);
int emi_kkt_solve_dev(emi_ctx_t ctx, void* dRhs, int nrhs);

typedef struct emi_ipm_point { void *X, *U, *S, *E1, *E2; } emi_ipm_point_t;
typedef struct emi_ipm_duals { void *LamF, *Y, *ZL, *ZU, *VL, *VU, *W1, *W2; } emi_ipm_duals_t;
typedef struct emi_ipm_step { void *DZLam, *DS, *DY, *DE1, *DE2, *DZL, *DZU, *DVL, *DVU, *DW1, *DW2; } emi_ipm_step_t;
typedef struct emi_ipm_elim { void *Sigma, *SigT, *SigS, *RhatS, *Rt; } emi_ipm_elim_t;
typedef struct emi_ipm_bounds { const void *zl, *zu; int nsets; const double *cl, *cu, *cscale; } emi_ipm_bounds_t;
int emi_ipm_reduce_dev(emi_ctx_t ctx, const emi_ipm_point_t* pt, const emi_ipm_duals_t* du, const void* dRES, const void* dVALS,
                       const void* dG, const emi_ipm_bounds_t* bd, const void* dPar, const void* dDefRes, const void* dRowRes,
                       const emi_ipm_elim_t* out, void* dRhs);
int emi_ipm_expand_dev(emi_ctx_t ctx, const emi_ipm_point_t* pt, const emi_ipm_duals_t* du, const void* dVALS,
                       const emi_ipm_bounds_t* bd, const void* dPar, const emi_ipm_elim_t* el, const void* dRs,
                       const emi_ipm_step_t* st, void* dScal);
int emi_ipm_trial_dev(emi_ctx_t ctx, const emi_ipm_point_t* pt, const emi_ipm_step_t* st, const void* dAlpha,
                      const emi_ipm_point_t* trial);
int emi_ipm_merit_dev(emi_ctx_t ctx, const emi_ipm_point_t* pt, const void* dRES, const void* dCOST, const emi_ipm_bounds_t* bd,
                      const void* dPar, const void* dRs, int reset, void* dOut);
int emi_ipm_accept_dev(emi_ctx_t ctx, const emi_ipm_point_t* pt, const emi_ipm_point_t* trial, const emi_ipm_duals_t* du,
                       const emi_ipm_step_t* st, const emi_ipm_bounds_t* bd, const void* dPar, const void* dApr, const void* dAdu,
                       const void* dMask);
int emi_ipm_error_dev(emi_ctx_t ctx, const emi_ipm_point_t* pt, const emi_ipm_duals_t* du, const void* dRES, const void* dG,
                      const emi_ipm_bounds_t* bd, const void* dPar, void* dOut);
int emi_ipm_reduce_host(emi_ctx_t ctx, const emi_ipm_point_t* pt, const emi_ipm_duals_t* du, const double* RES, const double* VALS,
                        const double* G, const emi_ipm_bounds_t* bd, const double* par, const double* DefRes, const double* RowRes,
                        const emi_ipm_elim_t* out, double* Rhs);
int emi_ipm_expand_host(emi_ctx_t ctx, const emi_ipm_point_t* pt, const emi_ipm_duals_t* du, const double* VALS,
                        const emi_ipm_bounds_t* bd, const double* par, const emi_ipm_elim_t* el, const double* rs,
                        const emi_ipm_step_t* st, double* scal);
int emi_ipm_trial_host(emi_ctx_t ctx, const emi_ipm_point_t* pt, const emi_ipm_step_t* st, const double* alpha,
                       const emi_ipm_point_t* trial);
int emi_ipm_merit_host(emi_ctx_t ctx, const emi_ipm_point_t* pt, const double* RES, const double* COST, const emi_ipm_bounds_t* bd,
                       const double* par, const double* rs, int reset, double* out);
int emi_ipm_accept_host(emi_ctx_t ctx, const emi_ipm_point_t* pt, const emi_ipm_point_t* trial, const emi_ipm_duals_t* du,
                        const emi_ipm_step_t* st, const emi_ipm_bounds_t* bd, const double* par, const double* a_pr,
                        const double* a_du, const unsigned char* mask);
int emi_ipm_error_host(emi_ctx_t ctx, const emi_ipm_point_t* pt, const emi_ipm_duals_t* du, const double* RES, const double* G,
                       const emi_ipm_bounds_t* bd, const double* par, double* out);

int emi_kkt_factor_shard_dev(emi_ctx_t ctx, const void* dQ, const void* dVALS, const void* dFixed, const double* dc,
                             const unsigned char* mask, int* info);
int emi_kkt_lowrank_shard_dev(emi_ctx_t ctx, int max_mods, const void* dCount, const void* dNode, const void* dDelta,
                              const void* dVec, const unsigned char* mask, int* exact);
int emi_kkt_solve_shard_dev(emi_ctx_t ctx, void* dRhs, const unsigned char* mask);
int emi_kkt_solve_refined_shard_dev(emi_ctx_t ctx, void* dRhs, const unsigned char* mask, const double* dc_nominal, int max_steps,
                                    double* rel, int* nsolve, int* reverted, int* status);

enum { EMI_IPM_CONVERGED = 0, EMI_IPM_ACCEPTABLE = 1, EMI_IPM_MAX_ITER = 2, EMI_IPM_LINE_SEARCH = 3, EMI_IPM_INFEASIBLE = 4,
       EMI_IPM_FACTOR = 5 , EMI_IPM_NOT_FINITE = 6 };
enum { EMI_IPM_RULE_RESIDUAL = 1  };
typedef struct emi_ipm_options {
  double tol, mu_init, bound_push, bound_frac, rho_init, acceptable_factor;
  int max_iter, acceptable_iter, max_futile_escalations;
  int rules;
  int crawl_limit;
  double crawl_frac;
} emi_ipm_options_t;
typedef struct emi_ipm_result {
  int status, iterations, evaluations, factorisations, reflected_steps;
  double cost, kkt_error, constr_viol, emax, mu, rho;
  int newton_steps, restored_steps;
} emi_ipm_result_t;
int emi_ipm_solve_shard_dev(emi_ctx_t ctx, void* dX, void* dU, const emi_ipm_bounds_t* bd, const emi_ipm_options_t* opt,
                            void* dLamF, void* dLamC, emi_ipm_result_t* results);
int emi_ipm_solve_shard_host(emi_ctx_t ctx, double* X, double* U, const emi_ipm_bounds_t* bd, const emi_ipm_options_t* opt,
                             double* LamF, double* LamC, emi_ipm_result_t* results);
typedef struct emi_ipm_rung {
  int M;
  emi_ipm_bounds_t bd;
  const double* recs;
  emi_ipm_options_t opt;
  int repair;
} emi_ipm_rung_t;
int emi_prolong_matrix(int Mc, const double* tau_c, const double* w_c, int Mf, const double* tau_f, double* P);
int emi_prolong_dev(emi_ctx_t ctx, int Mc, int Mf, const void* dPT, const void* dVc, int R, void* dVf);
int emi_repair_guess_dev(emi_ctx_t ctx, void* dX);
int emi_ipm_solve_ladder_dev(emi_ctx_t ctx, int nrungs, const emi_ipm_rung_t* rungs, double t0, double tf, const void* dX0,
                             const void* dU0, void* dX, void* dU, void* dLamF, void* dLamC, emi_ipm_result_t* results);
int emi_ipm_solve_ladder_host(emi_ctx_t ctx, int nrungs, const emi_ipm_rung_t* rungs, double t0, double tf, const double* X0,
                              const double* U0, double* X, double* U, double* LamF, double* LamC, emi_ipm_result_t* results);
int emi_ode_error_operator(int M, const double* tau, const double* w, double* E, double* Ed, double* tq);
int emi_interp_dev(emi_ctx_t ctx, int K, int N, int ldk, const void* dOP, const void* dV, int R, int ldo, void* dOut);
int emi_ode_error_dev(emi_ctx_t ctx, const void* dX, const void* dU, const double* ul, const double* uu, void* dEta, void* dErr);
int emi_ode_error_host(emi_ctx_t ctx, const double* X, const double* U, const double* ul, const double* uu, double* Eta, double* Err);
enum { EMI_REFINE_MET = 0, EMI_REFINE_NOT_MET = 1, EMI_REFINE_FELL_BACK = 2, EMI_REFINE_FAILED = 3 };
typedef struct emi_ipm_refine {
  double ode_tol;
  int first_check;
  const double *ul, *uu;
} emi_ipm_refine_t;
typedef struct emi_ipm_refine_result { int rung, verdict, rungs_solved; double err; } emi_ipm_refine_result_t;
int emi_ipm_refine_decide(int status, double err, double ode_tol, int has_good, int is_last, int* verdict);
int emi_prolong_rows_dev(emi_ctx_t ctx, int Mc, int Mf, const void* dPT, const void* dVc, int R, const void* dRowMap, void* dVf);
int emi_shard_move_dev(emi_ctx_t ctx, int n, const void* dSrcIdx, const void* dDstIdx, int narrays, const int* rows,
                       const void* const* src, const int* src_ld, void* const* dst, const int* dst_ld, int len);
int emi_ipm_solve_refine_dev(emi_ctx_t ctx, int nrungs, const emi_ipm_rung_t* rungs, double t0, double tf, const emi_ipm_refine_t* rf,
                             const void* dX0, const void* dU0, int ldm, void* dX, void* dU, void* dLamF, void* dLamC,
                             emi_ipm_result_t* results, double* err, emi_ipm_refine_result_t* out);
int emi_ipm_solve_refine_host(emi_ctx_t ctx, int nrungs, const emi_ipm_rung_t* rungs, double t0, double tf, const emi_ipm_refine_t* rf,
                              const double* X0, const double* U0, int ldm, double* X, double* U, double* LamF, double* LamC,
                              emi_ipm_result_t* results, double* err, emi_ipm_refine_result_t* out);
enum { EMI_START_LINE = 0, EMI_START_BEND = 1, EMI_START_PLANNED = 2 };
typedef struct emi_start {
  int kind;
  int nsets;
  const double* xa;
  const double* xb;
  const double* box;
  double bend;
  double clearance;
  int grid;
  int repair;
} emi_start_t;
int emi_plan_route(int np, const double* recs, const double ends[4], const double box[4], double clearance, int grid, int M,
                   const double* tau, double* xs, double* ys, int* level, double* cost, int* cells, int* ncells);
int emi_start_guess_dev(emi_ctx_t ctx, const emi_start_t* st, void* dX, void* dLevel);
int emi_start_guess_host(emi_ctx_t ctx, const emi_start_t* st, double* X, int* level);
int emi_ipm_start_dev(emi_ctx_t ctx, int phase, const emi_ipm_point_t* pt, const emi_ipm_duals_t* du, const void* dRES,
                      const emi_ipm_bounds_t* bd, const void* dPar, double bound_push, double bound_frac, void* dFixed,
                      const void* dMask);
int emi_ipm_error_parts_dev(emi_ctx_t ctx, const emi_ipm_point_t* pt, const emi_ipm_duals_t* du, const void* dRES, const void* dG,
                            const emi_ipm_bounds_t* bd, const void* dPar, void* dOut);
int emi_ipm_error_parts_host(emi_ctx_t ctx, const emi_ipm_point_t* pt, const emi_ipm_duals_t* du, const double* RES, const double* G,
                             const emi_ipm_bounds_t* bd, const double* par, double* out);
int emi_ipm_keep_dev(emi_ctx_t ctx, const emi_ipm_point_t* pt, const emi_ipm_duals_t* du, const emi_ipm_point_t* kept_pt,
                     const emi_ipm_duals_t* kept_du, const void* dMask, int restore);
int emi_ipm_keep_host(emi_ctx_t ctx, const emi_ipm_point_t* pt, const emi_ipm_duals_t* du, const emi_ipm_point_t* kept_pt,
                      const emi_ipm_duals_t* kept_du, const unsigned char* mask, int restore);

typedef struct emi_pass_plan {
  int one_launch;
  int sw;
  int ksplit;
  int ring_stages;
  int cpart, cx;
  int mfma_workgroups;
  int store_mode;
  int block_order;
  int tiles16;
  int piece, tail;
  int k_tile;
  int column_tiles;
  int k_halves;
} emi_pass_plan_t;
int emi_plan_pass(emi_ctx_t ctx, int B, emi_pass_plan_t* out);

int emi_jac_structure(emi_ctx_t ctx, int* rows, int* cols);
int emi_invariant_rows(int model, int np, unsigned char* mask, int* nvals);

int emi_dev_alloc(emi_ctx_t ctx, size_t bytes, void** dptr);
int emi_dev_free(emi_ctx_t ctx, void* dptr);
int emi_h2d(emi_ctx_t ctx, void* dst, const void* src, size_t bytes);
int emi_d2h(emi_ctx_t ctx, void* dst, const void* src, size_t bytes);

int emi_eval_dev(emi_ctx_t ctx, const void* dX, const void* dU, void* dRES,
                 void* dVALS, void* dCOST, unsigned flags);
int emi_eval_host(emi_ctx_t ctx, const double* X, const double* U, double* RES,
                  double* VALS, double* COST, unsigned flags);

int emi_hess_dev(emi_ctx_t ctx, const void* dX, const void* dU,
                 const void* dLamF, const void* dLamC, double sigma, void* dH);
int emi_hess_host(emi_ctx_t ctx, const double* X, const double* U,
                  const double* LamF, const double* LamC, double sigma,
                  double* H);

int emi_lagr_grad_dev(emi_ctx_t ctx, const void* dVALS, const void* dLamF, const void* dLamC, double sigma, void* dG);
int emi_lagr_grad_host(emi_ctx_t ctx, const double* VALS, const double* LamF, const double* LamC, double sigma, double* G);
int emi_kkt_certificate_dev(emi_ctx_t ctx, const void* dX, const void* dU, const void* dRES, const void* dVALS,
                            const void* dLamF, const void* dLamC, double sigma, const void* dZl, const void* dZu, int nsets,
                            const double* cl, const double* cu, void* dCert, void* dG);
int emi_kkt_certificate_host(emi_ctx_t ctx, const double* X, const double* U, const double* LamF, const double* LamC,
                             double sigma, const double* zl, const double* zu, int nsets, const double* cl, const double* cu,
                             double* cert, double* G);
int emi_lagr_grad_total_dev(emi_ctx_t ctx, const void* dVALS, const void* dLamF, const void* dLamC, double sigma, void* dG,
                            void* dGdel);
int emi_lagr_grad_total_host(emi_ctx_t ctx, const double* VALS, const double* LamF, const double* LamC, double sigma, double* G,
                             double* Gdel);
int emi_kkt_certificate_total_dev(emi_ctx_t ctx, const void* dX, const void* dU, const void* dRES, const void* dVALS,
                                  const void* dLamF, const void* dLamC, double sigma, const void* dZl, const void* dZu, int nsets,
                                  const double* cl, const double* cu, void* dCert, void* dG, void* dGdel);
int emi_kkt_certificate_total_host(emi_ctx_t ctx, const double* X, const double* U, const double* LamF, const double* LamC,
                                   double sigma, const double* zl, const double* zu, int nsets, const double* cl, const double* cu,
                                   double* cert, double* G, double* Gdel);

int emi_timer_start(emi_ctx_t ctx);
int emi_timer_stop(emi_ctx_t ctx, float* elapsed_ms);
int emi_profile_enable(emi_ctx_t ctx, int level);
int emi_profile_read(emi_ctx_t ctx, float* node_ms, int* node_launches,
                     float* defect_ms, int* defect_launches,
                     float* fused_ms, int* fused_launches);

int emi_set_option(emi_ctx_t ctx, const char* name, int value);
int emi_last_path(emi_ctx_t ctx, int* fused);
int emi_debug_tile_order(int ns, int B, int M, int sym_ct, int sym_cpart, int* out_tile, int out_cap, int* ntiles_total,
                         int* cpart, int* cx);
int emi_debug_tile_order2(int ns, int B, int M, int sym_ct, int sym_cpart, int sym_gblk, int sym_cx, int* out_tile, int out_cap,
                          int* ntiles_total, int* cpart, int* cx);
int emi_debug_pass_roles(int nm, int nn, int order, int* out_role, int out_cap);
const char* emi_last_defect_kernel(emi_ctx_t ctx);

#define EMI_COMM_ID_BYTES 128
typedef struct emi_comm_s* emi_comm_t;
int emi_comm_unique_id(void* id );
int emi_comm_create(int device_id, int world, int rank, const void* id, emi_comm_t* out);
int emi_comm_gather(emi_comm_t comm, const void* dsend, void* drecv, size_t bytes, int root, void* hip_stream);
int emi_comm_destroy(emi_comm_t comm);
const char* emi_comm_last_error(emi_comm_t comm);

#ifdef __cplusplus
}
#endif
#endif
```

Baseline: 5.610 billion.

## Load De/Do operator fragments straight from L2 in the fused pass kernel

Precomputes the even/odd operator halves in the exact per-lane MFMA fragment order on the host and uploads them. A new DOP variant of the ring body fetches these B fragments with direct global loads interleaved among the MFMAs, so they no longer pass through the LDS operand ring. This shrinks the LDS stages and removes the LDS reads for the operator. In exchange it adds global load traffic and inline-asm waitcnt handling. The variant is selected automatically only for large deep batches with BK=16 and SW of 1 or 2.

```diff
diff --git a/etol_amd/_lib.py b/etol_amd/_lib.py
--- a/etol_amd/_lib.py
+++ b/etol_amd/_lib.py
@@ -202,6 +202,7 @@
     "emi_set_delays": (C.c_int, [_P, C.c_int, C.c_int, C.c_double]),
     "emi_get_delays": (C.c_int, [_P, _I, _I, _I]),
     "emi_delay_matrix": (C.c_int, [C.c_int, C.POINTER(C.c_double), C.POINTER(C.c_double), C.c_double, C.c_double, C.c_double, C.POINTER(C.c_double)]),
+    "emi_debug_operator_fragments": (C.c_int, [C.c_int, C.POINTER(C.c_double), C.POINTER(C.c_double)]),
     "emi_debug_tile_order2": (C.c_int, [C.c_int] * 7 + [C.POINTER(C.c_int), C.c_int, C.POINTER(C.c_int), C.POINTER(C.c_int), C.POINTER(C.c_int)]),
     "emi_comm_unique_id": (C.c_int, [_P]),
     "emi_comm_create": (C.c_int, [C.c_int, C.c_int, C.c_int, _P, C.POINTER(_P)]),
diff --git a/etol_amd/csrc/emi_api.hip b/etol_amd/csrc/emi_api.hip
--- a/etol_amd/csrc/emi_api.hip
+++ b/etol_amd/csrc/emi_api.hip
@@ -59,6 +59,23 @@
         if (o.bytes) HIP_TRY(c, hipMemcpyAsync(o.host, o.dev, o.bytes, hipMemcpyDeviceToHost, c->stream));
     HIP_TRY(c, hipStreamSynchronize(c->stream));
     return EMI_OK;
+}
+
+bool emi_api::even_odd_halves(int M, const double* D, std::vector<double>& De, std::vector<double>& Do) {
+    if (M % 2 != 0) return false;
+    const int N = M - 1, Hh = M / 2;
+    for (int i = 0; i < M; ++i)
+        for (int j = 0; j < M; ++j)
+            if (D[(size_t)i * M + j] != -D[(size_t)(N - i) * M + (N - j)]) return false;
+    De.assign((size_t)Hh * Hh, 0.0);
+    Do.assign((size_t)Hh * Hh, 0.0);
+    for (int i = 0; i < Hh; ++i)
+        for (int j = 0; j < Hh; ++j) {
+            const double p = D[(size_t)i * M + j], q = D[(size_t)i * M + (N - j)];
+            De[(size_t)i * Hh + j] = 0.5 * (p + q);
+            Do[(size_t)i * Hh + j] = 0.5 * (p - q);
+        }
+    return true;
 }
 
 namespace {
@@ -99,6 +116,7 @@
     {"sym_hs", &emi_ctx_s::sym_hs, within<0, 2>, as_given, "sym_hs must be 0 (by batch size), 1 or 2"},
     {"sym_ctc", &emi_ctx_s::sym_ctc, within<0, 2>, as_given, "sym_ctc must be 0 (by batch size), 1 or 2"},
     {"sym_bk", &emi_ctx_s::sym_bk, one_of<0, 8, 16>, as_given, "sym_bk must be 0 (by batch size), 8 or 16"},
+    {"sym_dop", &emi_ctx_s::sym_dop, within<0, 2>, as_given, "sym_dop must be 0 (by batch size), 1 (De / Do through the operand ring) or 2 (straight from L2)"},
     {"sym_cpart", &emi_ctx_s::sym_cpart, one_of<-1, 0, 1, 2, 4, 8>, as_given, "sym_cpart must be -1 (plain order), 0 (by mesh size), 1, 2, 4 or 8"},
     {"sym_gblk", &emi_ctx_s::sym_gblk, within<0, 64>, as_given, "sym_gblk must be 0 (off) .. 64 instance groups per super-block"},
     {"sym_cx", &emi_ctx_s::sym_cx, within<0, 64>, as_given, "sym_cx must be 0 (default) .. 64 column tiles per block"},
@@ -201,21 +219,17 @@
         return upload_bytes(c, c->d_D, Df.data(), Df.size() * 4);
     }
     EMI_TRY(upload_real(c, c->d_D, D, (size_t)M * M));
-    if (M % 2 != 0) return EMI_OK;
-    const int N = M - 1, Hh = M / 2;
-    for (int i = 0; i < M; ++i)
-        for (int j = 0; j < M; ++j)
-            if (D[(size_t)i * M + j] != -D[(size_t)(N - i) * M + (N - j)]) return EMI_OK;
-    std::vector<double> De((size_t)Hh * Hh), Do((size_t)Hh * Hh);
-    for (int i = 0; i < Hh; ++i)
-        for (int j = 0; j < Hh; ++j) {
-            const double p = D[(size_t)i * M + j], q = D[(size_t)i * M + (N - j)];
-            De[(size_t)i * Hh + j] = 0.5 * (p + q);
-            Do[(size_t)i * Hh + j] = 0.5 * (p - q);
-        }
+    std::vector<double> De, Do;
+    if (!even_odd_halves(M, D, De, Do)) return EMI_OK;
     EMI_TRY(upload_real(c, c->d_De, De.data(), De.size()));
     EMI_TRY(upload_real(c, c->d_Do, Do.data(), Do.size()));
     c->symmetric = true;
+    if (M % 128 == 0) {
+        std::vector<double> frag(De.size() + Do.size());
+        emi::operator_fragments(M, De.data(), Do.data(), frag.data());
+        EMI_TRY(upload_real(c, c->d_Dfrag, frag.data(), frag.size()));
+        c->has_dfrag = true;
+    }
     return EMI_OK;
 }
 
@@ -235,6 +249,7 @@
     EMI_TRY(upload_real(c, c->d_t, nt.data(), M));
     EMI_TRY(upload_real(c, c->d_Ddiag, dd.data(), M));
     c->symmetric = false;
+    c->has_dfrag = false;
     if (D) EMI_TRY(upload_operator(c, M, D));
     c->points_only = !D;
     c->h_tau.assign(tau, tau + M);
diff --git a/etol_amd/csrc/emi_api_pass.hip b/etol_amd/csrc/emi_api_pass.hip
--- a/etol_amd/csrc/emi_api_pass.hip
+++ b/etol_amd/csrc/emi_api_pass.hip
@@ -77,6 +77,10 @@
     if (hs_want == 2 && !c->rtc && plan.ks == 1 && plan.ct == 1 && (plan.sw == 1 || plan.sw == 2) && plan.nst == 3 &&
         ((c->M / 2) / plan.bk) % 4 == 0)
         plan.hs = 2;
+    const int dop_want = c->sym_dop ? c->sym_dop : ((deep_large && p.tiles16 >= 216) ? 2 : 1);
+    if (dop_want == 2 && !c->rtc && c->has_dfrag && plan.bk == 16 && plan.ks == 1 && plan.ct == 1 && plan.hs == 1 && plan.nst == 3 &&
+        plan.sw != c->ns && (plan.sw == 1 || plan.sw == 2))
+        plan.dop = true;
     p.sym = plan;
     p.mfma_first = c->pass_order >= 0 ? c->pass_order
                                       : (deep_band ? 150 : (p.tiles16 < 208 ? 1 : (p.tiles16 < 384 ? 125 : (p.tiles16 < 768 ? 110 : 0))));
@@ -248,7 +252,8 @@
 std::string name_pass_f64(const emi::SymPlan& plan) {
     return "emi_pass_f64_kernel<SW=" + std::to_string(plan.sw) + "> (MFMA + node roles, one launch" +
            (plan.ks > 1 ? ", " + std::to_string(plan.ks) + " K slices per tile" : "") + ")" +
-           (plan.bk == 16 ? " [K tiles of 16]" : "") + (plan.ct == 2 ? " [128-column tiles]" : "") + (plan.hs == 2 ? " [K range in two halves per workgroup]" : "");
+           (plan.bk == 16 ? " [K tiles of 16]" : "") + (plan.ct == 2 ? " [128-column tiles]" : "") + (plan.hs == 2 ? " [K range in two halves per workgroup]" : "") +
+           (plan.dop ? " [De/Do from L2]" : "");
 }
 std::string name_symdefect(emi_ctx_t c, const emi::SymPlan& plan, bool in_kernel_combine) {
     if (plan.ring1) return c->sym_ct == 1 || c->sym_ct == 2 ? "emi_symdefect_f64_kernel" : NAME_RING1_F64;
@@ -264,6 +269,7 @@
     sa.node_t = (const double*)c->d_t.p;
     sa.De = (const double*)c->d_De.p;
     sa.Do = (const double*)c->d_Do.p;
+    sa.Dfrag = c->has_dfrag ? (const double*)c->d_Dfrag.p : nullptr;
     sa.M = c->M;
     sa.B = L.B;
     sa.nres = nres_of(c);
@@ -671,6 +677,14 @@
     return EMI_OK;
 }
 
+int emi_debug_operator_fragments(int M, const double* D, double* out) {
+    if (M < 128 || M % 128 != 0 || !D || !out) return EMI_ERR_ARG;
+    std::vector<double> De, Do;
+    if (!even_odd_halves(M, D, De, Do)) return EMI_ERR_UNSUPPORTED;
+    emi::operator_fragments(M, De.data(), Do.data(), out);
+    return EMI_OK;
+}
+
 const char* emi_last_defect_kernel(emi_ctx_t c) {
     if (!c) return "";
     return c->last_defect_kernel.c_str();
diff --git a/etol_amd/csrc/emi_args.hpp b/etol_amd/csrc/emi_args.hpp
--- a/etol_amd/csrc/emi_args.hpp
+++ b/etol_amd/csrc/emi_args.hpp
@@ -101,6 +101,7 @@
     int cpart, cx;
     double h;
     ModelParams<double> P;
+    const double* Dfrag;
 };
 
 struct DefectArgs {
diff --git a/etol_amd/csrc/emi_ctx.hpp b/etol_amd/csrc/emi_ctx.hpp
--- a/etol_amd/csrc/emi_ctx.hpp
+++ b/etol_amd/csrc/emi_ctx.hpp
@@ -43,6 +43,8 @@
     double t0 = 0, tf = 0;
     DevBuf d_w, d_t, d_Ddiag, d_D, d_De, d_Do;
     bool symmetric = false;
+    DevBuf d_Dfrag;
+    bool has_dfrag = false;
     bool points_only = false;
     int allow_fused = 1;
     int sym_ct = 0;
@@ -81,6 +83,7 @@
     int sym_hs = 0;
     int sym_ctc = 0;
     int sym_bk = 0;
+    int sym_dop = 0;
     int xh = 0, uh = 0, nch = 0;
     double delay_dt = 0.0;
     bool delay_dirty = true;
@@ -189,6 +192,7 @@
 int upload_bytes(emi_ctx_t c, DevBuf& b, const void* src, size_t bytes);
 int upload_real(emi_ctx_t c, DevBuf& b, const double* src, size_t n);
 int download_real(emi_ctx_t c, double* dst, const void* dsrc, size_t n);
+bool even_odd_halves(int M, const double* D, std::vector<double>& De, std::vector<double>& Do);
 int ensure_vals_staging(emi_ctx_t c, size_t bytes);
 
 inline int np_total(emi_ctx_t c) { return c->np + c->np_model; }
diff --git a/etol_amd/csrc/emi_kernels.hpp b/etol_amd/csrc/emi_kernels.hpp
--- a/etol_amd/csrc/emi_kernels.hpp
+++ b/etol_amd/csrc/emi_kernels.hpp
@@ -37,12 +37,27 @@
     int bk = 8;
     int hs = 1;
     int ct = 1;
+    bool dop = false;
     size_t slab_bytes = 0;
     int cpart = 0, cx = 0;
     int tiles = 0;
 };
 SymPlan plan_symdefect(int ns, int B, int M, int ct, int ksplit_opt, int cpart_opt = 0, int gblk_opt = 0, int cx_opt = 0, int bk_opt = 8, int ct_cols = 1);
 hipError_t launch_symdefect(int model, const SymDefectArgs& a, hipStream_t s, bool set_attr, int ct, const SymPlan& plan);
+inline void operator_fragments(int M, const double* De, const double* Do, double* out) {
+    const int Hh = M / 2, nkt = Hh / 16;
+    for (int ct = 0; ct < Hh / 64; ++ct)
+        for (int w = 0; w < 4; ++w)
+            for (int kt = 0; kt < nkt; ++kt)
+                for (int q = 0; q < 4; ++q)
+                    for (int lane = 0; lane < 64; ++lane) {
+                        const double* row = ((q & 1) ? Do : De) + (size_t)(64 * ct + 16 * w + (lane & 15)) * Hh + 16 * kt + 8 * (q >> 1) + 2 * (lane >> 4);
+                        double* o = out + ((((size_t)(ct * 4 + w) * nkt + kt) * 4 + q) * 64 + lane) * 2;
+                        o[0] = row[0];
+                        o[1] = row[1];
+                    }
+}
+
 bool pass_supported(int model, int ns, int B, int M, const SymPlan& plan);
 hipError_t launch_pass(int model, const SymDefectArgs& sa, const NodeArgs<double>& na, hipStream_t s, const SymPlan& plan);
 
diff --git a/etol_amd/csrc/emi_symdefect.hip b/etol_amd/csrc/emi_symdefect.hip
--- a/etol_amd/csrc/emi_symdefect.hip
+++ b/etol_amd/csrc/emi_symdefect.hip
@@ -119,7 +119,7 @@
     return launch_ring2_model<Model, 1>(a, s);
 }
 
-template <class Model, int SW, int NST, int BK = 8, int CT = 1, int HS = 1>
+template <class Model, int SW, int NST, int BK = 8, int CT = 1, int HS = 1, bool DOP = false>
 static hipError_t launch_pass_model(const SymDefectArgs& sa, const NodeArgs<double>& na, hipStream_t s) {
     constexpr int NS = Model::NS;
     PassArgs a;
@@ -133,15 +133,17 @@
     a.nn = nn;
     a.nm8 = (nm + 7) / 8;
     a.nn8 = ((nn + HS - 1) / HS + 7) / 8;
-    const size_t lds = (size_t)HS * NST * ((2 * SW * FUSED_TI + 2 * 64 * CT + 63) / 64 * 64) * BK * sizeof(double);
+    const size_t lds = DOP ? (size_t)NST * (2 * SW * FUSED_TI) * BK * sizeof(double)
+                           : (size_t)HS * NST * ((2 * SW * FUSED_TI + 2 * 64 * CT + 63) / 64 * 64) * BK * sizeof(double);
+    if (DOP && (!sa.Dfrag || sa.ksplit > 1)) return hipErrorInvalidValue;
     const int st = (na.store_mode >= 0 && na.store_mode <= 3) ? na.store_mode : 0;
     constexpr bool HAS_KEEP = NST == 3 && HS == 1;
     const bool keep = HAS_KEEP && na.keep;
     auto pick = [&](auto keep_c) {
         constexpr bool K = decltype(keep_c)::value;
-        return st == 2 ? emi_pass_f64_kernel<Model, SW, 2, 2, NST, BK, CT, HS, K>
-             : (st == 1 ? emi_pass_f64_kernel<Model, SW, 2, 1, NST, BK, CT, HS, K>
-                        : (st == 3 ? emi_pass_f64_kernel<Model, SW, 2, 3, NST, BK, CT, HS, K> : emi_pass_f64_kernel<Model, SW, 2, 0, NST, BK, CT, HS, K>));
+        return st == 2 ? emi_pass_f64_kernel<Model, SW, 2, 2, NST, BK, CT, HS, K, DOP>
+             : (st == 1 ? emi_pass_f64_kernel<Model, SW, 2, 1, NST, BK, CT, HS, K, DOP>
+                        : (st == 3 ? emi_pass_f64_kernel<Model, SW, 2, 3, NST, BK, CT, HS, K, DOP> : emi_pass_f64_kernel<Model, SW, 2, 0, NST, BK, CT, HS, K, DOP>));
     };
     auto kern = pick(std::false_type{});
     if constexpr (HAS_KEEP) {
@@ -164,6 +166,7 @@
     if constexpr (NS > 2 && NS % 2 == 0) {
         if (p.sw == 2 && p.hs == 2 && p.ct == 1) return p.bk == 16 ? launch_pass_model<Model, 2, 3, 16, 1, 2>(sa, na, s) : launch_pass_model<Model, 2, 3, 8, 1, 2>(sa, na, s);
         if (p.sw == 2 && p.ct == 2) return p.bk == 16 ? launch_pass_model<Model, 2, 3, 16, 2>(sa, na, s) : launch_pass_model<Model, 2, 3, 8, 2>(sa, na, s);
+        if (p.sw == 2 && p.bk == 16 && p.dop) return launch_pass_model<Model, 2, 3, 16, 1, 1, true>(sa, na, s);
         if (p.sw == 2 && p.bk == 16) return launch_pass_model<Model, 2, 3, 16>(sa, na, s);
         if (p.sw == 2) return p.nst > 3 ? launch_pass_model<Model, 2, 4>(sa, na, s) : launch_pass_model<Model, 2, 3>(sa, na, s);
     }
@@ -171,6 +174,7 @@
         if (p.sw == 3) return launch_pass_model<Model, 3, 3>(sa, na, s);
     }
     if (p.hs == 2) return p.bk == 16 ? launch_pass_model<Model, 1, 3, 16, 1, 2>(sa, na, s) : launch_pass_model<Model, 1, 3, 8, 1, 2>(sa, na, s);
+    if (p.bk == 16 && p.dop) return launch_pass_model<Model, 1, 3, 16, 1, 1, true>(sa, na, s);
     if (p.bk == 16) return launch_pass_model<Model, 1, 3, 16>(sa, na, s);
     return p.nst > 3 ? launch_pass_model<Model, 1, 4>(sa, na, s) : launch_pass_model<Model, 1, 3>(sa, na, s);
 }
@@ -178,6 +182,7 @@
 bool pass_supported(int model, int ns, int B, int M, const SymPlan& p) {
     if (p.ring1 || p.sw < 1 || (model != EMI_MODEL_POINTMASS2D && model != EMI_MODEL_QUADROTOR2D)) return false;
     if (M % 128 != 0 || ns % p.sw != 0) return false;
+    if (p.dop && !(p.bk == 16 && p.ks == 1 && p.ct == 1 && p.hs == 1 && p.nst == 3 && p.sw != ns && (p.sw == 1 || p.sw == 2))) return false;
     return B >= 1;
 }
 
diff --git a/etol_amd/csrc/emi_symdefect_kernels.hpp b/etol_amd/csrc/emi_symdefect_kernels.hpp
--- a/etol_amd/csrc/emi_symdefect_kernels.hpp
+++ b/etol_amd/csrc/emi_symdefect_kernels.hpp
@@ -5,6 +5,9 @@
 namespace emi {
 
 typedef double d4 __attribute__((ext_vector_type(4)));
+typedef double d2 __attribute__((ext_vector_type(2)));
+template <bool C, class A, class B> struct emi_pick { typedef A type; };
+template <class A, class B> struct emi_pick<false, A, B> { typedef B type; };
 
 template <class Model, int CT>
 __global__ __launch_bounds__(256, CT == 1 ? 2 : 1) void emi_symdefect_f64_kernel(SymDefectArgs a) {
@@ -433,7 +436,7 @@
     ring_epilogue_pre<Model, SW, false>(a, acc_a, acc_b, inst0, i0, s0, wid, r16, kq, none);
 }
 
-template <class Model, int SW, int NST = 3, int BK = 8, int CT = 1, int HS = 1>
+template <class Model, int SW, int NST = 3, int BK = 8, int CT = 1, int HS = 1, bool DOP = false>
 EMI_DEV void emi_ring2_body(const SymDefectArgs& a, const int bid ) {
     constexpr int NS = Model::NS;
     constexpr int TI = FUSED_TI, TM = SW * TI, TN = 64 * CT, CH = BK / 2, NSG = NS / SW;
@@ -442,8 +445,9 @@
     constexpr int RPI = 64 / CH;
     static_assert(BK == 8 || BK == 16, "K tiles of 8 or 16");
     constexpr int LOOK = NST - 1;
-    constexpr int ROWS = 2 * TM + 2 * TN;
-    constexpr int ROWS_PAD = (ROWS + 63) / 64 * 64;
+    static_assert(!DOP || (SW <= 2 && NST == 3 && BK == 16 && CT == 1 && HS == 1), "De / Do from L2: the unsplit 16-deep form only");
+    constexpr int ROWS = 2 * TM + (DOP ? 0 : 2 * TN);
+    constexpr int ROWS_PAD = DOP ? (ROWS + 4 * RPI - 1) / (4 * RPI) * (4 * RPI) : (ROWS + 63) / 64 * 64;
     constexpr int STAGE = ROWS_PAD * BK;
     constexpr int L = ROWS_PAD * CH / 256;
     static_assert(NS % SW == 0, "states split evenly over workgroups");
@@ -455,7 +459,7 @@
 
     const int M = a.M, Hh = M >> 1, B = a.B;
     const int ntiles = Hh / TN;
-    const int KS = (HS == 1 && a.ksplit > 1) ? a.ksplit : 1;
+    const int KS = (HS == 1 && !DOP && a.ksplit > 1) ? a.ksplit : 1;
     const int kslice = bid % KS;
     const RingTile rt = ring_tile_of(bid / KS, ntiles, (B + TI - 1) / TI * NSG, a.cpart, a.cx, NSG);
     const int ntile = rt.ntile, grp = rt.grp;
@@ -517,6 +521,11 @@
 #pragma unroll
         for (int t = 0; t < L; ++t) issue_one(t);
     };
+    constexpr int ND = DOP ? 2 * KH : 0;
+    unsigned long long fnext = 0;
+    const unsigned foff = (unsigned)lane * 16u;
+    if constexpr (DOP)
+        fnext = (unsigned long long)(a.Dfrag + ((size_t)(((a.ablate & 64) ? 0 : ntile) * 4 + wid) * (Hh / BK) + kt0) * (ND * 64 * 2));
 
     d4 acc_a[SW][CT], acc_b[SW][CT];
 #pragma unroll
@@ -550,19 +559,42 @@
             off_m[s][h] = (TM + r) * BK + (((CH - 1 - kq - 4 * h) ^ ring_swz_k<BK>(r)) << 1);
         }
     }
+    typedef typename emi_pick<DOP, d2, double2>::type BFrag;
     struct Frag {
-        double2 be[CT][KH], bo[CT][KH], sp[SW][KH], dm[SW][KH];
+        BFrag be[CT][KH], bo[CT][KH];
+        double2 sp[SW][KH], dm[SW][KH];
     };
     double2 txf[SW][KH], txm[SW][KH];
-    constexpr int NRH = 2 * CT + 2 * SW;
+    constexpr int NB = DOP ? 0 : 2 * CT;
+    constexpr int NRH = NB + 2 * SW;
     constexpr int NR = NRH * KH, NM = 4 * SW * CT * KH;
     auto read_one = [&](Frag& f, const double* S, int r) {
         const int h = r / NRH, q = r % NRH;
-        if (q < 2 * CT) {
-            if (q & 1) f.bo[q >> 1][h] = *reinterpret_cast<const double2*>(S + (2 * TM + TN) * BK + off_b[q >> 1][h]);
-            else f.be[q >> 1][h] = *reinterpret_cast<const double2*>(S + 2 * TM * BK + off_b[q >> 1][h]);
-        } else if (q & 1) txm[(q - 2 * CT) >> 1][h] = *reinterpret_cast<const double2*>(S + off_m[(q - 2 * CT) >> 1][h]);
-        else txf[(q - 2 * CT) >> 1][h] = *reinterpret_cast<const double2*>(S + off_f[(q - 2 * CT) >> 1][h]);
+        if (q < NB) {
+            if constexpr (NB > 0) {
+                if (q & 1) f.bo[q >> 1][h] = *reinterpret_cast<const double2*>(S + (2 * TM + TN) * BK + off_b[q >> 1][h]);
+                else f.be[q >> 1][h] = *reinterpret_cast<const double2*>(S + 2 * TM * BK + off_b[q >> 1][h]);
+            }
+        } else if (q & 1) txm[(q - NB) >> 1][h] = *reinterpret_cast<const double2*>(S + off_m[(q - NB) >> 1][h]);
+        else txf[(q - NB) >> 1][h] = *reinterpret_cast<const double2*>(S + off_f[(q - NB) >> 1][h]);
+    };
+    auto dload_one = [&](Frag& f, int q) {
+        if constexpr (DOP) {
+            d2& dst = (q & 1) ? f.bo[0][q >> 1] : f.be[0][q >> 1];
+            if (q == 0) asm volatile("global_load_dwordx4 %0, %1, %2" : "=v"(dst) : "v"(foff), "s"(fnext) : "memory");
+            if (q == 1) asm volatile("global_load_dwordx4 %0, %1, %2 offset:1024" : "=v"(dst) : "v"(foff), "s"(fnext) : "memory");
+            if (q == 2) asm volatile("global_load_dwordx4 %0, %1, %2 offset:2048" : "=v"(dst) : "v"(foff), "s"(fnext) : "memory");
+            if (q == 3) asm volatile("global_load_dwordx4 %0, %1, %2 offset:3072" : "=v"(dst) : "v"(foff), "s"(fnext) : "memory");
+            if (q == ND - 1) fnext += (unsigned long long)(ND * 1024);
+        }
+    };
+    auto wait_counted = [&](Frag& f) {
+        if constexpr (DOP) asm volatile("s_waitcnt vmcnt(%4)" : "+v"(f.be[0][0]), "+v"(f.bo[0][0]), "+v"(f.be[0][1]), "+v"(f.bo[0][1]) : "n"(L * (LOOK - 1)) : "memory");
+        else asm volatile("s_waitcnt vmcnt(%0)" ::"n"(L * (LOOK - 1)) : "memory");
+    };
+    auto wait_all = [&](Frag& f) {
+        if constexpr (DOP) asm volatile("s_waitcnt vmcnt(0)" : "+v"(f.be[0][0]), "+v"(f.bo[0][0]), "+v"(f.be[0][1]), "+v"(f.bo[0][1]) :: "memory");
+        else asm volatile("s_waitcnt vmcnt(0)" ::: "memory");
     };
     auto sums_one = [&](Frag& f, int s) {
 #pragma unroll
@@ -595,12 +627,18 @@
         for (int i = 0; i < NM; ++i) mfma_one(f, i);
     };
     if constexpr (SW <= 3) {
-        constexpr int RPG = (NR + (NM - L) - 1) / (NM - L);
+        constexpr int RPG = DOP ? NR / ND : (NR + (NM - L) - 1) / (NM - L);
         constexpr int GR = (NR + RPG - 1) / RPG;
         static_assert(NM > L && GR + L <= NM, "a gap for every DMA instruction after the reads");
-        auto step = [&](const Frag& cur, Frag& nxt, int kt) {
-            if (kt + LOOK < nkt) asm volatile("s_waitcnt vmcnt(%0)" ::"n"(L * (LOOK - 1)) : "memory");
-            else                 asm volatile("s_waitcnt vmcnt(0)" ::: "memory");
+        static_assert(!DOP || GR == ND, "a direct load in every gap that takes reads");
+        struct Ahead { enum { drained = 0 }; };
+        struct Tail { enum { drained = 1 }; };
+        auto step = [&](Frag& cur, Frag& nxt, int kt, auto tail) {
+            if constexpr (DOP) {
+                if constexpr (decltype(tail)::drained) wait_all(cur);
+                else wait_counted(cur);
+            } else if (kt + LOOK < nkt) wait_counted(cur);
+            else wait_all(cur);
             __builtin_amdgcn_s_waitcnt(0xC07F);
             asm volatile("s_barrier" ::: "memory");
             const bool more = nd < nkt;
@@ -608,6 +646,7 @@
 #pragma unroll
             for (int i = 0; i < NM; ++i) {
                 mfma_one(cur, i);
+                if (DOP && i < ND) dload_one(nxt, i);
                 if (i < GR) {
 #pragma unroll
                     for (int r = i * RPG; r < (i + 1) * RPG && r < NR; ++r) read_one(nxt, S, r);
@@ -619,18 +658,23 @@
             }
         };
         Frag f0, f1;
-        if (nkt > LOOK - 1) asm volatile("s_waitcnt vmcnt(%0)" ::"n"(L * (LOOK - 1)) : "memory");
-        else                asm volatile("s_waitcnt vmcnt(0)" ::: "memory");
+        if constexpr (DOP) {
+#pragma unroll
+            for (int q = 0; q < ND; ++q) dload_one(f0, q);
+            wait_all(f0);
+        } else if (nkt > LOOK - 1) wait_counted(f0);
+        else wait_all(f0);
         asm volatile("s_barrier" ::: "memory");
         if (LOOK < nkt) issue();
         __builtin_amdgcn_s_waitcnt(0xC07F);
         read_frag(f0);
         int kt = 0;
         for (; kt + 2 < nkt; kt += 2) {
-            step(f0, f1, kt);
-            step(f1, f0, kt + 1);
-        }
-        step(f0, f1, kt);
+            step(f0, f1, kt, Ahead{});
+            step(f1, f0, kt + 1, Ahead{});
+        }
+        step(f0, f1, kt, Tail{});
+        if constexpr (DOP) wait_all(f1);
         multiply(f1);
     } else {
         for (int kt = 0; kt < nkt; ++kt) {
@@ -774,7 +818,7 @@
 #else
 #define EMI_PASS_OCC __attribute__((amdgpu_waves_per_eu(SW > 3 ? 1 : 2, 2)))
 #endif
-template <class Model, int SW, int VEC, int ST, int NST = 3, int BK = 8, int CT = 1, int HS = 1, bool KEEP = false>
+template <class Model, int SW, int VEC, int ST, int NST = 3, int BK = 8, int CT = 1, int HS = 1, bool KEEP = false, bool DOP = false>
 __global__ __launch_bounds__(256 * HS) EMI_PASS_OCC void emi_pass_f64_kernel(PassArgs a) {
 #ifdef EMI_ENTRY_PAD_NOPS
     asm volatile(".rept " EMI_STR(EMI_ENTRY_PAD_NOPS) "\n\ts_nop 0\n\t.endr" ::: "memory");
@@ -786,7 +830,7 @@
         const int tid = xcd * a.nm8 + role.index;
         if (tid >= a.nm) return;
         __builtin_amdgcn_s_setprio(3);
-        emi_ring2_body<Model, SW, NST, BK, CT, HS>(a.s, tid);
+        emi_ring2_body<Model, SW, NST, BK, CT, HS, DOP>(a.s, tid);
     } else {
         const int nid = (xcd * a.nn8 + role.index) * HS + (HS > 1 ? (int)(threadIdx.x >> 8) : 0);
         if (nid >= a.nn) return;
diff --git a/include/emi355x.h b/include/emi355x.h
--- a/include/emi355x.h
+++ b/include/emi355x.h
@@ -315,6 +315,7 @@
                          int* cpart, int* cx);
 int emi_debug_tile_order2(int ns, int B, int M, int sym_ct, int sym_cpart, int sym_gblk, int sym_cx, int* out_tile, int out_cap,
                           int* ntiles_total, int* cpart, int* cx);
+int emi_debug_operator_fragments(int M, const double* D, double* out);
 int emi_debug_pass_roles(int nm, int nn, int order, int* out_role, int out_cap);
 const char* emi_last_defect_kernel(emi_ctx_t ctx);
 
```

After: 5.792 billion (median of 6 runs). 1.03x the previous value.
